# Paleogenomics/IBDGem

Measured on NVIDIA B200. Metric: LD genotype-comparisons/s (site x target x bg x 4), higher is better.
Workload: dtype f64

## Files before the change

### ibdgem_b200/csrc/engine.cu

```cuda
#include <math.h>
#include <stdarg.h>
#include <stdio.h>
#include <string.h>

#include <algorithm>

#include "engine.h"
#include "site_math.cuh"

namespace ibdgem {

static thread_local char g_err[1024] = "";

void set_error(const char *fmt, ...) {
    va_list ap;
    va_start(ap, fmt);
    vsnprintf(g_err, sizeof g_err, fmt, ap);
    va_end(ap);
}

static const char *const kKernelNameList[] = {
    "site_table",     "scan_count",    "scan_offsets",  "scan_rank",    "window_nonld", "counters",
    "expand_sites",   "ld_general",    "ld_finalize",   "ld_compact",   "ld_c0",        "ld_transpose",
    "ld_stage",       "ld_expand_bg",  "ld_expand_tgt", "ld_windows",   "ld_ibd0",
    "ld_mma",         "viterbi",       "viterbi_back",  "viterbi_out",  "fill",
    "v_slots",        "v_wmap",        "v_tw",          "v_sort",       "v_expand_a",  "v_expand_b",   "ld_vmma",
    "window_linear",  "posterior_fwd", "posterior_bwd", "posterior_fwd_log", "posterior_bwd_log",
    "tract_count",    "tract_emit",    "posterior_bwd_moments",
};
static_assert(sizeof(kKernelNameList) / sizeof(kKernelNameList[0]) == K_COUNT, "one name per KernelId, in enum order");
const char *const *const kKernelNames = kKernelNameList;

LaunchScope::LaunchScope(ibdgem_engine *e_, int id_, cudaStream_t s_) : e(e_), id(id_), s(s_ ? s_ : e_->stream) {
    e->k_launches[id]++;
    if (!e->timing) return;
    auto get = [&]() {
        cudaEvent_t ev;
        if (!e->event_pool.empty()) {
            ev = e->event_pool.back();
            e->event_pool.pop_back();
        } else {
            cudaEventCreate(&ev);
        }
        return ev;
    };
    a = get();
    b = get();
    cudaEventRecord(a, s);
}
LaunchScope::~LaunchScope() {
    if (!a) return;
    cudaEventRecord(b, s);
    e->pending.push_back({id, a, b});
}
int settle_timers(ibdgem_engine *e) {
    if (e->t0_set || e->pending.size() > 4096) return resolve_timers(e);
    return 0;
}
int resolve_timers(ibdgem_engine *e) {
    FILE *tl = e->timeline_path && e->t0_set && !e->pending.empty() ? fopen(e->timeline_path, "a") : nullptr;
    for (auto &p : e->pending) {
        float ms = 0;
        cudaEventSynchronize(p.b);
        if (cudaEventElapsedTime(&ms, p.a, p.b) == cudaSuccess) e->k_ms[p.id] += ms;
        if (tl) {
            float t_a = 0, t_b = 0;
            cudaEventElapsedTime(&t_a, e->ev_t0, p.a);
            cudaEventElapsedTime(&t_b, e->ev_t0, p.b);
            fprintf(tl, "%s %.4f %.4f\n", kKernelNames[p.id], t_a, t_b);
        }
        e->event_pool.push_back(p.a);
        e->event_pool.push_back(p.b);
    }
    e->pending.clear();
    if (tl) fclose(tl);
    return 0;
}

int dev_alloc(ibdgem_engine *e, void **p, size_t bytes) {
    *p = nullptr;
    if (bytes == 0) bytes = 16;
    IBD_CUDA(cudaMalloc(p, bytes));
    e->device_bytes += (int64_t)bytes;
    return 0;
}
void dev_free(ibdgem_engine *e, void *p, size_t bytes) {
    if (!p) return;
    cudaFree(p);
    e->device_bytes -= (int64_t)(bytes ? bytes : 16);
}

int pinned_stage(ibdgem_engine *e, size_t bytes, void **out) {
    if (e->h_pin_cap < bytes) {
        if (e->h_pin) cudaFreeHost(e->h_pin);
        e->h_pin = nullptr;
        e->h_pin_cap = 0;
        const size_t want = bytes + bytes / 4 + 4096;
        IBD_CUDA(cudaMallocHost(&e->h_pin, want));
        e->h_pin_cap = want;
    }
    *out = e->h_pin;
    return 0;
}

int scratch(ibdgem_engine *e, int slot, size_t bytes, void **out) {
    if (e->scratch.empty()) e->scratch.assign(SC_SLOTS, nullptr);
    DeviceBuf *&b = e->scratch[slot];
    if (!b) b = new DeviceBuf();
    if (b->cap < bytes) {
        if (b->p) dev_free(e, b->p, b->cap);
        b->p = nullptr;
        b->cap = 0;
        size_t want = bytes + bytes / 8 + 256;
        if (dev_alloc(e, &b->p, want)) return 1;
        b->cap = want;
    }
    *out = b->p;
    return 0;
}

__device__ __forceinline__ int warp_sum_i(int v) {
#pragma unroll
    for (int o = 16; o > 0; o >>= 1) v += __shfl_xor_sync(0xffffffffu, v, o);
    return v;
}
__device__ __forceinline__ double warp_sum_d(double v) {
#pragma unroll
    for (int o = 16; o > 0; o >>= 1) v += __shfl_xor_sync(0xffffffffu, v, o);
    return v;
}
__device__ __forceinline__ double warp_max_d(double v) {
#pragma unroll
    for (int o = 16; o > 0; o >>= 1) v = fmax(v, __shfl_xor_sync(0xffffffffu, v, o));
    return v;
}

__global__ void fill_nan_kernel(double *p, int64_t n) {
    int64_t i = blockIdx.x * (int64_t)blockDim.x + threadIdx.x;
    const double nan = __longlong_as_double(0x7ff8000000000000LL);
    for (; i < n; i += (int64_t)gridDim.x * blockDim.x) p[i] = nan;
}

__global__ void __launch_bounds__(256)
site_table_kernel(int64_t s_begin, int64_t S, int32_t N, int64_t Wh, const uint32_t *__restrict__ bits,
                  const uint8_t *__restrict__ hostkeep, const uint8_t *__restrict__ nref,
                  const uint8_t *__restrict__ nalt, const double *__restrict__ afuser,
                  const double *__restrict__ Ptab, int C, double min_af, double max_af, int max_cov,
                  double *__restrict__ f_out, uint8_t *__restrict__ keep, uint8_t *__restrict__ status,
                  double *__restrict__ lik7, double *__restrict__ lnlik7, const double *__restrict__ lnPtab) {
    __shared__ double stage7[8][32 * 7];
    const int lane = threadIdx.x & 31;
    const int64_t warp0 = (blockIdx.x * (int64_t)blockDim.x + threadIdx.x) >> 5;
    const int64_t nwarps = ((int64_t)gridDim.x * blockDim.x) >> 5;
    const int H = 2 * N;
    const int nfull = H >> 5, rem = H & 31;
    const bool vec4 = ((Wh & 3) == 0);
    const int n4 = vec4 ? (nfull >> 2) : 0;
    for (int64_t s0 = s_begin + warp0 * 32; s0 < S; s0 += nwarps * 32) {
        const int rows = (int)min((int64_t)32, S - s0);
        int mycnt = 0;
        const int j = lane >> 2, q = lane & 3;
#pragma unroll
        for (int it = 0; it < 4; it++) {
            const int r = it * 8 + j;
            int cnt = 0;
            if (r < rows) {
                const uint32_t *row = bits + (s0 + r) * Wh;
                const uint4 *row4 = reinterpret_cast<const uint4 *>(row);
                for (int w = q; w < n4; w += 4) {
                    const uint4 x = __ldg(row4 + w);
                    cnt += __popc(x.x) + __popc(x.y) + __popc(x.z) + __popc(x.w);
                }
                for (int w = (n4 << 2) + q; w < nfull; w += 4) cnt += __popc(__ldg(row + w));
                if (q == 0 && rem) cnt += __popc(__ldg(row + nfull) & ((1u << rem) - 1u));
            }
            cnt += __shfl_xor_sync(0xffffffffu, cnt, 1);
            cnt += __shfl_xor_sync(0xffffffffu, cnt, 2);
            const int got = __shfl_sync(0xffffffffu, cnt, 4 * (lane & 7));
            if ((lane >> 3) == it) mycnt = got;
        }
        const int64_t s = s0 + lane;
        double v[7], lv[7];
        const double nan = __longlong_as_double(0x7ff8000000000000LL);
#pragma unroll
        for (int i = 0; i < 7; i++) v[i] = lv[i] = nan;
        if (lane < rows) {
            double f = __ddiv_rn((double)mycnt, (double)H);
            if (afuser) {
                const double u = afuser[s];
                if (u == u) f = u;
            }
            const int r = nref[s], a = nalt[s];
            const bool k = hostkeep[s] && !(f > max_af || f < min_af) && (r + a <= max_cov);
            if (k) {
                const double *P = Ptab + (size_t)(r * C + a) * 3;
                const double P0 = P[0], P1 = P[1], P2 = P[2];
                v[0] = lik_ibd0(f, P0, P1, P2);
                v[1] = lik_ibd1(0, f, P0, P1, P2);
                v[2] = lik_ibd1(1, f, P0, P1, P2);
                v[3] = lik_ibd1(2, f, P0, P1, P2);
                v[4] = P0; v[5] = P1; v[6] = P2;
            }
            const double *lP = lnPtab + (k ? (size_t)(r * C + a) * 3 : 0);
#pragma unroll
            for (int i = 0; i < 7; i++) lv[i] = k ? (i >= 4 ? lP[i - 4] : log(v[i])) : v[i];
            f_out[s] = f;
            keep[s] = k ? 1 : 0;
            status[s] = k ? ((r + a >= 1) ? 1 : 2) : 0;
        }
        double *stw = stage7[threadIdx.x >> 5];
#pragma unroll
        for (int pass = 0; pass < 2; pass++) {
            __syncwarp();
#pragma unroll
            for (int i = 0; i < 7; i++) stw[lane * 7 + i] = pass ? lv[i] : v[i];
            __syncwarp();
            double *dst = (pass ? lnlik7 : lik7) + s0 * 7;
            for (int i = lane; i < rows * 7; i += 32) dst[i] = stw[i];
        }
    }
}

__global__ void __launch_bounds__(256)
site_status_kernel(int64_t S, const uint8_t *__restrict__ hostkeep, const uint8_t *__restrict__ nref,
                   const uint8_t *__restrict__ nalt, int max_cov, uint8_t *__restrict__ keep, uint8_t *__restrict__ status,
                   int C, unsigned long long *__restrict__ cnt ) {
    extern __shared__ unsigned int shist[];
    for (int i = threadIdx.x; i < C + 3; i += blockDim.x) shist[i] = 0;
    __syncthreads();
    unsigned proc = 0, skip = 0, cov = 0;
    for (int64_t s = blockIdx.x * (int64_t)blockDim.x + threadIdx.x; s < S; s += (int64_t)gridDim.x * blockDim.x) {
        const int r = nref[s], a = nalt[s];
        const bool k = hostkeep[s] && (r + a <= max_cov);
        keep[s] = k ? 1 : 0;
        status[s] = k ? ((r + a >= 1) ? 1 : 2) : 0;
        if (k) {
            proc++;
            cov += (unsigned)(r + a);
            atomicAdd(&shist[3 + min(r + a, C - 1)], 1u);
        } else {
            skip++;
        }
    }
    proc = (unsigned)warp_sum_i((int)proc);
    skip = (unsigned)warp_sum_i((int)skip);
    cov = (unsigned)warp_sum_i((int)cov);
    if ((threadIdx.x & 31) == 0) {
        atomicAdd(&shist[0], proc);
        atomicAdd(&shist[1], skip);
        atomicAdd(&shist[2], cov);
    }
    __syncthreads();
    for (int i = threadIdx.x; i < C + 3; i += blockDim.x)
        if (shist[i]) atomicAdd(&cnt[i], (unsigned long long)shist[i]);
}

constexpr int SCAN_THREADS = 256;
constexpr int SCAN_ITERS = 8;
constexpr int SCAN_CHUNK = SCAN_THREADS * SCAN_ITERS;
constexpr int ROW_SLICE = 32768;

__global__ void __launch_bounds__(SCAN_THREADS)
scan_count_kernel(SiteView v, const int32_t *__restrict__ targets, uint32_t *__restrict__ blockcnt,
                  int nb) {
    const int t = blockIdx.y;
    const int indiv = targets ? targets[t] : 0;
    const int64_t base = (int64_t)blockIdx.x * SCAN_CHUNK;
    int c = 0;
    for (int it = 0; it < SCAN_ITERS; it++) {
        const int64_t s = base + it * SCAN_THREADS + threadIdx.x;
        int r, a, g;
        if (s < v.S && site_eval(v, t, indiv, s, r, a, g) == 1) c++;
    }
    c = warp_sum_i(c);
    __shared__ int ws[SCAN_THREADS / 32];
    if ((threadIdx.x & 31) == 0) ws[threadIdx.x >> 5] = c;
    __syncthreads();
    if (threadIdx.x == 0) {
        int tot = 0;
        for (int i = 0; i < SCAN_THREADS / 32; i++) tot += ws[i];
        blockcnt[(int64_t)t * nb + blockIdx.x] = tot;
    }
}

__global__ void __launch_bounds__(256)
scan_offsets_kernel(uint32_t *__restrict__ blockcnt, int nb, int window, int64_t *__restrict__ ktot,
                    int32_t *__restrict__ nwin) {
    const int t = blockIdx.x;
    uint32_t *row = blockcnt + (int64_t)t * nb;
    __shared__ uint32_t carry;
    __shared__ uint32_t ws[8];
    if (threadIdx.x == 0) carry = 0;
    __syncthreads();
    for (int b0 = 0; b0 < nb; b0 += 256) {
        const int i = b0 + threadIdx.x;
        const uint32_t v = (i < nb) ? row[i] : 0;
        uint32_t x = v;
#pragma unroll
        for (int o = 1; o < 32; o <<= 1) {
            const uint32_t y = __shfl_up_sync(0xffffffffu, x, o);
            if ((threadIdx.x & 31) >= o) x += y;
        }
        if ((threadIdx.x & 31) == 31) ws[threadIdx.x >> 5] = x;
        __syncthreads();
        uint32_t woff = 0;
        for (int w = 0; w < (int)(threadIdx.x >> 5); w++) woff += ws[w];
        const uint32_t excl = carry + woff + x - v;
        if (i < nb) row[i] = excl;
        __syncthreads();
        if (threadIdx.x == 255) carry = excl + v;
        __syncthreads();
    }
    if (threadIdx.x == 0) {
        ktot[t] = carry;
        nwin[t] = (int32_t)((carry + (uint32_t)window - 1) / (uint32_t)window);
    }
}

__global__ void __launch_bounds__(SCAN_THREADS)
scan_rank_kernel(SiteView v, const int32_t *__restrict__ targets, const uint32_t *__restrict__ blockoff,
                 int nb, int window, const int64_t *__restrict__ ktot, int64_t *__restrict__ wfirst,
                 int64_t *__restrict__ wlast, int maxW, uint32_t *__restrict__ rank_out) {
    const int t = blockIdx.y;
    const int indiv = targets ? targets[t] : 0;
    const int64_t base = (int64_t)blockIdx.x * SCAN_CHUNK;
    const int lane = threadIdx.x & 31, wid = threadIdx.x >> 5;
    __shared__ int ws[SCAN_THREADS / 32];
    uint32_t running = blockoff[(int64_t)t * nb + blockIdx.x];
    const int64_t K = ktot[t];
    for (int it = 0; it < SCAN_ITERS; it++) {
        const int64_t s = base + it * SCAN_THREADS + threadIdx.x;
        int r, a, g;
        const bool inf = (s < v.S) && site_eval(v, t, indiv, s, r, a, g) == 1;
        const uint32_t bal = __ballot_sync(0xffffffffu, inf);
        if (lane == 0) ws[wid] = __popc(bal);
        __syncthreads();
        uint32_t off = running;
        int tot = 0;
        for (int w = 0; w < SCAN_THREADS / 32; w++) {
            if (w < wid) off += ws[w];
            tot += ws[w];
        }
        const uint32_t rk = off + __popc(bal & ((1u << lane) - 1u));
        if (rank_out && s < v.S) rank_out[s] = rk;
        if (inf) {
            const uint32_t w = rk / (uint32_t)window, k = rk % (uint32_t)window;
            if ((int)w < maxW) {
                if (k == 0) wfirst[(int64_t)t * maxW + w] = s;
                if (k == (uint32_t)window - 1 || (int64_t)rk == K - 1) wlast[(int64_t)t * maxW + w] = s;
            }
        }
        running += tot;
        __syncthreads();
    }
}

struct WindowMapView {
    const int64_t *wfirst, *wlast;
    const int32_t *nwin;
    int rows;
    int maxW;
};

__global__ void __launch_bounds__(256)
window_nonld_kernel(SiteView v, WindowMapView m, const int32_t *__restrict__ targets, int T,
                    const uint64_t *__restrict__ pos, const double *__restrict__ f,
                    const double *__restrict__ lnlik7, const double *__restrict__ Ptab, int C,
                    int outW, double *__restrict__ wll, int32_t *__restrict__ wn,
                    uint64_t *__restrict__ ws, uint64_t *__restrict__ we, int32_t *__restrict__ nwin_out) {
    const int lane = threadIdx.x & 31;
    const int64_t gw = (blockIdx.x * (int64_t)blockDim.x + threadIdx.x) >> 5;
    const int64_t total = (int64_t)T * outW;
    if (gw >= total) return;
    const int t = (int)(gw / outW), w = (int)(gw % outW);
    const int row = (m.rows == 1) ? 0 : t;
    const int nw = m.nwin[row];
    if (w == 0 && lane == 0) nwin_out[t] = nw;
    if (w >= nw || w >= m.maxW) return;
    const int indiv = targets[t];
    const int64_t s0 = m.wfirst[(int64_t)row * m.maxW + w], s1 = m.wlast[(int64_t)row * m.maxW + w];
    double a0 = 0, a1 = 0, a2 = 0;
    int n = 0;
    for (int64_t s = s0 + lane; s <= s1; s += 32) {
        int r, a, g;
        if (site_eval(v, t, indiv, s, r, a, g) != 1) continue;
        n++;
        if (v.tgt_counts) {
            const double *P = Ptab + (size_t)(r * C + a) * 3;
            const double P0 = P[0], P1 = P[1], P2 = P[2], ff = f[s];
            a0 += log(lik_ibd0(ff, P0, P1, P2));
            a1 += log(lik_ibd1(g, ff, P0, P1, P2));
            a2 += log(P[g]);
        } else {
            const double *L = lnlik7 + s * 7;
            a0 += L[0];
            a1 += L[1 + g];
            a2 += L[4 + g];
        }
    }
    a0 = warp_sum_d(a0);
    a1 = warp_sum_d(a1);
    a2 = warp_sum_d(a2);
    n = warp_sum_i(n);
    if (lane == 0) {
        const int64_t o = (int64_t)t * outW + w;
        wll[o * 3 + 0] = a0;
        wll[o * 3 + 1] = a1;
        wll[o * 3 + 2] = a2;
        wn[o] = n;
        ws[o] = pos[s0];
        we[o] = pos[s1];
    }
}

constexpr int NONLD_TILE = 256;
template <int NONLD_BATCH>
__global__ void __launch_bounds__(128)
window_nonld_shared_kernel(SiteView v, WindowMapView m, const int32_t *__restrict__ targets, int T,
                           const uint64_t *__restrict__ pos, const uint8_t *__restrict__ status,
                           const double *__restrict__ lnlik7, int outW, double *__restrict__ wll,
                           int32_t *__restrict__ wn, uint64_t *__restrict__ ws, uint64_t *__restrict__ we,
                           int32_t *__restrict__ nwin_out) {
    __shared__ double2 sl12[NONLD_TILE][3];
    __shared__ int64_t srow[NONLD_TILE];
    __shared__ int32_t soff[NONLD_TILE];
    __shared__ int segcnt[NONLD_TILE / 32];
    __shared__ double sa0[4];
    constexpr int PASSES = NONLD_TILE / 128;
    const int w = blockIdx.x;
    const int nw = m.nwin[0];
    const int t = blockIdx.y * blockDim.x + threadIdx.x;
    if (w == 0 && t < T) nwin_out[t] = nw;
    if (w >= nw || w >= m.maxW) return;
    const int64_t s0 = m.wfirst[w], s1 = m.wlast[w];
    const int indiv = t < T ? targets[t] : 0;
    const uint32_t *tcol = v.bits + (indiv >> 4);
    const int tsh = (indiv & 15) * 2;
    const int lane = threadIdx.x & 31;
    double a0p = 0, a1 = 0, a2 = 0;
    int n = 0;
    for (int64_t sb = s0; sb <= s1; sb += NONLD_TILE) {
        __syncthreads();
        unsigned bal[PASSES];
#pragma unroll
        for (int q = 0; q < PASSES; q++) {
            const int64_t s = sb + q * 128 + threadIdx.x;
            bal[q] = __ballot_sync(0xffffffffu, s <= s1 && status[s] == 1);
            if (lane == 0) segcnt[(q * 128 + threadIdx.x) >> 5] = __popc(bal[q]);
        }
        __syncthreads();
        int cnt = 0;
#pragma unroll
        for (int q = 0; q < PASSES; q++) {
            const int seg = (q * 128 + (int)threadIdx.x) >> 5;
            int base = 0;
            for (int k = 0; k < seg; k++) base += segcnt[k];
            if ((bal[q] >> lane) & 1u) {
                const int slot = base + __popc(bal[q] & ((1u << lane) - 1u));
                const int64_t site = sb + q * 128 + threadIdx.x;
                srow[slot] = site * v.Wh;
                soff[slot] = (int32_t)(site - s0);
            }
        }
        for (int k = 0; k < NONLD_TILE / 32; k++) cnt += segcnt[k];
        __syncthreads();
        for (int i = threadIdx.x; i < cnt * 7; i += blockDim.x) {
            const int j = i / 7, c = i - j * 7;
            const double x = lnlik7[(s0 + soff[j]) * 7 + c];
            double *dst = reinterpret_cast<double *>(&sl12[j][0]);
            if (c == 0)
                a0p += x;
            else if (c <= 3)
                dst[(c - 1) * 2] = x;
            else
                dst[(c - 4) * 2 + 1] = x;
        }
        __syncthreads();
        if (t < T) {
            for (int j0 = 0; j0 < cnt; j0 += NONLD_BATCH) {
                uint32_t pr[NONLD_BATCH];
#pragma unroll
                for (int q = 0; q < NONLD_BATCH; q++) pr[q] = (j0 + q < cnt) ? __ldg(tcol + srow[j0 + q]) : 0u;
#pragma unroll
                for (int q = 0; q < NONLD_BATCH; q++) {
                    if (j0 + q < cnt) {
                        const int g = __popc((pr[q] >> tsh) & 3u);
                        const double2 l = sl12[j0 + q][g];
                        a1 += l.x;
                        a2 += l.y;
                    }
                }
            }
            n += cnt;
        }
    }
    a0p = warp_sum_d(a0p);
    if (lane == 0) sa0[threadIdx.x >> 5] = a0p;
    __syncthreads();
    if (t < T) {
        const double a0 = (sa0[0] + sa0[1]) + (sa0[2] + sa0[3]);
        const int64_t o = (int64_t)t * outW + w;
        wll[o * 3 + 0] = a0;
        wll[o * 3 + 1] = a1;
        wll[o * 3 + 2] = a2;
        wn[o] = n;
        ws[o] = pos[s0];
        we[o] = pos[s1];
    }
}

__global__ void __launch_bounds__(128)
window_linear_kernel(SiteView v, WindowMapView m, const int32_t *__restrict__ targets, int T, const double *__restrict__ f,
                     const double *__restrict__ lik7, const double *__restrict__ Ptab, int C, int outW, double *__restrict__ wlin) {
    const int64_t i = blockIdx.x * (int64_t)blockDim.x + threadIdx.x;
    if (i >= (int64_t)T * outW) return;
    const int t = (int)(i / outW), w = (int)(i % outW);
    const int row = (m.rows == 1) ? 0 : t;
    if (w >= m.nwin[row] || w >= m.maxW) return;
    const int indiv = targets[t];
    const int64_t s0 = m.wfirst[(int64_t)row * m.maxW + w], s1 = m.wlast[(int64_t)row * m.maxW + w];
    double p0 = 1.0, p1 = 1.0, p2 = 1.0;
    for (int64_t s = s0; s <= s1; s++) {
        int r, a, g;
        if (site_eval(v, t, indiv, s, r, a, g) != 1) continue;
        double l0, l1, l2;
        if (v.tgt_counts) {
            const double *P = Ptab + (size_t)(r * C + a) * 3;
            l0 = lik_ibd0(f[s], P[0], P[1], P[2]);
            l1 = lik_ibd1(g, f[s], P[0], P[1], P[2]);
            l2 = P[g];
        } else {
            const double *L = lik7 + s * 7;
            l0 = L[0];
            l1 = L[1 + g];
            l2 = L[4 + g];
        }
        p0 = __dmul_rn(p0, l0);
        p1 = __dmul_rn(p1, l1);
        p2 = __dmul_rn(p2, l2);
    }
    wlin[i * 3 + 0] = p0;
    wlin[i * 3 + 1] = p1;
    wlin[i * 3 + 2] = p2;
}

constexpr int COUNTERS_CHUNK = 8192;
__global__ void __launch_bounds__(256)
counters_kernel(SiteView v, const int32_t *__restrict__ targets, int C,
                unsigned long long *__restrict__ out ) {
    const int t = blockIdx.y;
    const int indiv = targets ? targets[t] : 0;
    extern __shared__ unsigned long long sh[];
    for (int i = threadIdx.x; i < C + 3; i += blockDim.x) sh[i] = 0;
    __syncthreads();
    unsigned long long proc = 0, skip = 0, cov = 0;
    const int64_t s_begin = (int64_t)blockIdx.x * COUNTERS_CHUNK;
    const int64_t s_end = min(v.S, s_begin + COUNTERS_CHUNK);
    for (int64_t s = s_begin + threadIdx.x; s < s_end; s += blockDim.x) {
        int r = 0, a = 0, g = 0;
        const int st = site_eval(v, t, indiv, s, r, a, g);
        if (st == 0) {
            skip++;
        } else {
            proc++;
            cov += (unsigned)(r + a);
            atomicAdd(&sh[3 + min(r + a, C - 1)], 1ULL);
        }
    }
    atomicAdd(&sh[0], proc);
    atomicAdd(&sh[1], skip);
    atomicAdd(&sh[2], cov);
    __syncthreads();
    for (int i = threadIdx.x; i < C + 3; i += blockDim.x)
        if (sh[i]) atomicAdd(&out[(int64_t)t * (C + 3) + i], sh[i]);
}

__global__ void __launch_bounds__(256)
expand_sites_kernel(SiteView v, const int32_t *__restrict__ targets, int T,
                    const double *__restrict__ f, const double *__restrict__ lik7,
                    const double *__restrict__ Ptab, int C, uint8_t *__restrict__ st_out,
                    double *__restrict__ lik_out) {
    const int64_t i = blockIdx.x * (int64_t)blockDim.x + threadIdx.x;
    if (i >= (int64_t)T * v.S) return;
    const int t = (int)(i / v.S);
    const int64_t s = i % v.S;
    int r = 0, a = 0, g = 0;
    const int st = site_eval(v, t, targets[t], s, r, a, g);
    const double nan = __longlong_as_double(0x7ff8000000000000LL);
    double l0 = nan, l1 = nan, l2 = nan;
    if (st != 0) {
        if (v.tgt_counts) {
            const double *P = Ptab + (size_t)(r * C + a) * 3;
            l0 = lik_ibd0(f[s], P[0], P[1], P[2]);
            l1 = lik_ibd1(g, f[s], P[0], P[1], P[2]);
            l2 = P[g];
        } else {
            const double *L = lik7 + s * 7;
            l0 = L[0];
            l1 = L[1 + g];
            l2 = L[4 + g];
        }
    }
    if (st_out) st_out[i] = (uint8_t)st;
    if (lik_out) {
        lik_out[i * 3 + 0] = l0;
        lik_out[i * 3 + 1] = l1;
        lik_out[i * 3 + 2] = l2;
    }
}

constexpr int LD_THREADS = 256;
constexpr int LD_PER = 2;

struct LdPartial {
    double m0, s0, m1, s1;
};

__global__ void __launch_bounds__(LD_THREADS)
ld_general_kernel(SiteView v, WindowMapView m, const int32_t *__restrict__ targets,
                  const int32_t *__restrict__ bg, int n_bg, int pu_idx,
                  const double *__restrict__ lnPtab, int C, int outW, int nz,
                  LdPartial *__restrict__ part ) {
    const int w = blockIdx.x, t = blockIdx.y, z = blockIdx.z;
    const int row = (m.rows == 1) ? 0 : t;
    if (w >= m.nwin[row] || w >= m.maxW || w >= outW) return;
    const int indiv = targets[t];
    const int64_t s0 = m.wfirst[(int64_t)row * m.maxW + w], s1 = m.wlast[(int64_t)row * m.maxW + w];

    __shared__ double sl[LD_THREADS][3];
    __shared__ int64_t ssite[LD_THREADS];
    __shared__ uint8_t sa[LD_THREADS];
    __shared__ int wcount[LD_THREADS / 32];
    __shared__ double red[LD_THREADS / 32];

    const int lane = threadIdx.x & 31, wid = threadIdx.x >> 5;
    int b[LD_PER];
    bool valid[LD_PER];
    double acc[LD_PER][5];
#pragma unroll
    for (int p = 0; p < LD_PER; p++) {
        const int n = (z * LD_PER + p) * LD_THREADS + threadIdx.x;
        b[p] = (n < n_bg) ? bg[n] : -1;
        valid[p] = (n < n_bg) && b[p] != indiv && b[p] != pu_idx;
        if (!valid[p]) b[p] = 0;
#pragma unroll
        for (int q = 0; q < 5; q++) acc[p][q] = 0.0;
    }

    for (int64_t sb = s0; sb <= s1; sb += LD_THREADS) {
        const int64_t s = sb + threadIdx.x;
        int r = 0, a = 0, g = 0;
        const bool inf = (s <= s1) && site_eval(v, t, indiv, s, r, a, g) == 1;
        const uint32_t bal = __ballot_sync(0xffffffffu, inf);
        if (lane == 0) wcount[wid] = __popc(bal);
        __syncthreads();
        int off = 0, cnt = 0;
        for (int k = 0; k < LD_THREADS / 32; k++) {
            if (k < wid) off += wcount[k];
            cnt += wcount[k];
        }
        if (inf) {
            const int j = off + __popc(bal & ((1u << lane) - 1u));
            const double *L = lnPtab + (size_t)(r * C + a) * 3;
            sl[j][0] = L[0];
            sl[j][1] = L[1];
            sl[j][2] = L[2];
            ssite[j] = s;
            sa[j] = (uint8_t)hap_pair(v.bits + s * v.Wh, indiv);
        }
        __syncthreads();
        for (int j = 0; j < cnt; j++) {
            const double l0 = sl[j][0], l1 = sl[j][1], l2 = sl[j][2];
            const uint32_t ta = sa[j];
            const double u0lo = (ta & 1u) ? l1 : l0, u0hi = (ta & 1u) ? l2 : l1;
            const double u1lo = (ta & 2u) ? l1 : l0, u1hi = (ta & 2u) ? l2 : l1;
            const uint32_t *rowp = v.bits + ssite[j] * v.Wh;
#pragma unroll
            for (int p = 0; p < LD_PER; p++) {
                const uint32_t pr = hap_pair(rowp, b[p]);
                const bool r0 = pr & 1u, r1 = pr & 2u;
                const int gg = (int)r0 + (int)r1;
                acc[p][0] += (gg == 0) ? l0 : (gg == 1 ? l1 : l2);
                acc[p][1] += r0 ? u0hi : u0lo;
                acc[p][2] += r1 ? u0hi : u0lo;
                acc[p][3] += r0 ? u1hi : u1lo;
                acc[p][4] += r1 ? u1hi : u1lo;
            }
        }
        __syncthreads();
    }

    const double NEG = -INFINITY;
    double m0 = NEG, m1 = NEG;
#pragma unroll
    for (int p = 0; p < LD_PER; p++)
        if (valid[p]) {
            m0 = fmax(m0, acc[p][0]);
            m1 = fmax(m1, fmax(fmax(acc[p][1], acc[p][2]), fmax(acc[p][3], acc[p][4])));
        }
    auto block_max = [&](double x) {
        x = warp_max_d(x);
        __syncthreads();
        if (lane == 0) red[wid] = x;
        __syncthreads();
        double y = red[0];
        for (int k = 1; k < LD_THREADS / 32; k++) y = fmax(y, red[k]);
        return y;
    };
    auto block_sum = [&](double x) {
        x = warp_sum_d(x);
        __syncthreads();
        if (lane == 0) red[wid] = x;
        __syncthreads();
        double y = 0;
        for (int k = 0; k < LD_THREADS / 32; k++) y += red[k];
        return y;
    };
    m0 = block_max(m0);
    m1 = block_max(m1);
    double e0 = 0, e1 = 0;
#pragma unroll
    for (int p = 0; p < LD_PER; p++)
        if (valid[p]) {
            e0 += exp(acc[p][0] - m0);
            e1 += exp(acc[p][1] - m1) + exp(acc[p][2] - m1) + exp(acc[p][3] - m1) + exp(acc[p][4] - m1);
        }
    e0 = block_sum(e0);
    e1 = block_sum(e1);
    if (threadIdx.x == 0) {
        LdPartial o;
        o.m0 = m0; o.s0 = e0; o.m1 = m1; o.s1 = e1;
        part[((int64_t)t * outW + w) * nz + z] = o;
    }
}

__global__ void ld_finalize_kernel(const LdPartial *__restrict__ part, int nz, WindowMapView m, int T,
                                   int outW, const int32_t *__restrict__ nrefpanel,
                                   double *__restrict__ wll) {
    const int64_t i = blockIdx.x * (int64_t)blockDim.x + threadIdx.x;
    if (i >= (int64_t)T * outW) return;
    const int t = (int)(i / outW), w = (int)(i % outW);
    const int row = (m.rows == 1) ? 0 : t;
    if (w >= m.nwin[row]) return;
    const double nan = __longlong_as_double(0x7ff8000000000000LL);
    const int nr = nrefpanel[t];
    if (nr <= 0) {
        wll[i * 3 + 0] = nan;
        wll[i * 3 + 1] = nan;
        return;
    }
    double M0 = -INFINITY, M1 = -INFINITY;
    for (int z = 0; z < nz; z++) {
        M0 = fmax(M0, part[i * nz + z].m0);
        M1 = fmax(M1, part[i * nz + z].m1);
    }
    double S0 = 0, S1 = 0;
    for (int z = 0; z < nz; z++) {
        const LdPartial p = part[i * nz + z];
        if (p.s0 > 0) S0 += p.s0 * exp(p.m0 - M0);
        if (p.s1 > 0) S1 += p.s1 * exp(p.m1 - M1);
    }
    wll[i * 3 + 0] = M0 + log(S0) - log((double)nr);
    wll[i * 3 + 1] = M1 + log(S1) - log(4.0 * (double)nr);
}

int wait_panel_upto(ibdgem_engine *e, int64_t s_end) {
    while (e->chunks_waited < (int)e->chunk_end.size() &&
           (e->chunks_waited == 0 || e->chunk_end[(size_t)e->chunks_waited - 1] < s_end)) {
        IBD_CUDA(cudaStreamWaitEvent(e->stream, e->chunk_ev[(size_t)e->chunks_waited], 0));
        e->chunks_waited++;
    }
    if (e->chunk_end.empty() || e->chunk_end.back() < s_end) {
        set_error("[::] ERROR: panel rows up to %lld are needed but only %lld were declared ready "
                  "(ibdgem_engine_panel_rows_ready).", (long long)s_end, (long long)(e->chunk_end.empty() ? 0 : e->chunk_end.back()));
        return 1;
    }
    return 0;
}

int ensure_table(ibdgem_engine *e, int64_t s_end) {
    if (wait_panel_upto(e, s_end)) return 1;
    if (e->table_upto >= s_end) return 0;
    {
        LaunchScope ls(e, K_SITE_TABLE);
        const int64_t n = s_end - e->table_upto;
        site_table_kernel<<<(unsigned)((n + 255) / 256), 256, 0, e->stream>>>(
            e->table_upto, s_end, e->N, e->Wh, e->d_bits, e->d_hostkeep, e->d_nref, e->d_nalt, e->d_afuser, e->d_P, e->C,
            e->prm.min_af, e->prm.max_af, (int)e->prm.max_cov, e->d_f, e->d_keep, e->d_status, e->d_lik7, e->d_lnlik7, e->d_lnP);
    }
    IBD_CUDA(cudaGetLastError());
    e->table_upto = s_end;
    return 0;
}

void window_shard_bounds(const ibdgem_engine *e, int32_t *w_begin, int32_t *w_end, int64_t *s_begin, int64_t *s_end) {
    const int64_t nW = e->nW_shared;
    const int32_t wb = (int32_t)(nW * e->shard_index / e->shard_count), we = (int32_t)(nW * (e->shard_index + 1) / e->shard_count);
    if (w_begin) *w_begin = wb;
    if (w_end) *w_end = we;
    if (s_begin) *s_begin = wb > 0 && wb <= (int32_t)e->h_wlast.size() ? e->h_wlast[(size_t)wb - 1] + 1 : 0;
    if (s_end) *s_end = (e->shard_index + 1 >= e->shard_count || we <= 0 || we > (int32_t)e->h_wlast.size()) ? e->S : e->h_wlast[(size_t)we - 1] + 1;
}

}

using namespace ibdgem;

extern "C" {

const char *ibdgem_last_error(void) { return g_err; }
int ibdgem_abi_version(void) { return IBDGEM_B200_ABI_VERSION; }

static unsigned long host_binom(unsigned int n, unsigned int k) {
    unsigned long v = 1;
    const unsigned int base = n - k;
    for (unsigned int j = 1; j <= k; j++) v = ((unsigned int)(base + j) * v) / j;
    return v;
}

static void host_pdg(double eps, unsigned r, unsigned a, double out[3]) {
    if (r == 0 && a == 0) {
        out[0] = out[1] = out[2] = 1.0;
        return;
    }
    volatile double coef = (double)host_binom(r + a, r);
    volatile double p0 = coef * pow(1 - eps, (double)r);
    p0 = p0 * pow(eps, (double)a);
    volatile double p1 = coef * pow(0.5, (double)r);
    p1 = p1 * pow(0.5, (double)a);
    volatile double p2 = coef * pow(1 - eps, (double)a);
    p2 = p2 * pow(eps, (double)r);
    out[0] = p0 == 0.0 ? DBL_MIN : (double)p0;
    out[1] = p1 == 0.0 ? DBL_MIN : (double)p1;
    out[2] = p2 == 0.0 ? DBL_MIN : (double)p2;
}

int ibdgem_engine_create(const ibdgem_params *params, ibdgem_engine **out) {
    if (!params || !out) {
        set_error("[::] ERROR in ibdgem_engine_create(): NULL argument.");
        return 1;
    }
    *out = nullptr;
    if (params->max_cov < 1 || params->max_cov > IBDGEM_MAX_COV_LIMIT) {
        set_error("[::] ERROR: Invalid maximum estimated coverage (-M) of %u (must be 1..%d).",
                  params->max_cov, IBDGEM_MAX_COV_LIMIT);
        return 1;
    }
    if (params->window_size < 2) {
        set_error("[::] ERROR: Invalid window size (-w) of %d (must be >= 2).", params->window_size);
        return 1;
    }
    int ndev = 0;
    cudaError_t ce = cudaGetDeviceCount(&ndev);
    if (ce != cudaSuccess || ndev <= 0) {
        set_error("[::] ERROR: no usable CUDA device (%s); the engine has no CPU fallback.",
                  ce == cudaSuccess ? "device count is 0" : cudaGetErrorString(ce));
        return 1;
    }
    if (params->device < 0 || params->device >= ndev) {
        set_error("[::] ERROR: CUDA device %d out of range (0..%d).", params->device, ndev - 1);
        return 1;
    }
    IBD_CUDA(cudaSetDevice(params->device));
    ibdgem_engine *e = new ibdgem_engine();
    e->prm = *params;
    e->device = params->device;
    e->C = (int)params->max_cov + 1;
    cudaDeviceProp prop;
    if (cudaGetDeviceProperties(&prop, e->device) == cudaSuccess) e->sm_count = prop.multiProcessorCount;

    const int C = e->C;
    e->h_P.assign((size_t)C * C * 3, 1.0);
    e->h_lnP.assign((size_t)C * C * 3, 0.0);
    for (int r = 0; r < C; r++)
        for (int a = 0; a + r < C; a++) {
            double P[3];
            host_pdg(params->epsilon, (unsigned)r, (unsigned)a, P);
            for (int g = 0; g < 3; g++) {
                e->h_P[((size_t)r * C + a) * 3 + g] = P[g];
                e->h_lnP[((size_t)r * C + a) * 3 + g] = (double)logl((long double)P[g]);
            }
        }
    {
        const long double eps = params->epsilon;
        bool ok = eps > 0 && eps < 1;
        long double kap = 0, al = 0, be = 0;
        if (ok) {
            kap = logl(4 * eps * (1 - eps));
            al = logl(0.5L / (1 - eps));
            be = logl(0.5L / eps);
            for (int r = 0; r < C && ok; r++)
                for (int a = 0; a + r < C && ok; a++) {
                    const double *L = &e->h_lnP[((size_t)r * C + a) * 3];
                    const long double c = (long double)L[2] - 2 * (long double)L[1] + L[0];
                    const long double d = (long double)L[1] - L[0];
                    const long double tol = 1e-12L * (1 + fabsl((long double)L[0]) + fabsl((long double)L[2]));
                    if (fabsl(c - (r + a) * kap) > tol || fabsl(d - (r * al + a * be)) > tol) ok = false;
                }
        }
        e->depth_linear = ok;
        e->kappa = (double)kap;
        e->alpha = (double)al;
        e->beta = (double)be;
    }
    if (dev_alloc(e, (void **)&e->d_P, e->h_P.size() * 8) || dev_alloc(e, (void **)&e->d_lnP, e->h_lnP.size() * 8)) {
        delete e;
        return 1;
    }
    IBD_CUDA(cudaMemcpy(e->d_P, e->h_P.data(), e->h_P.size() * 8, cudaMemcpyHostToDevice));
    IBD_CUDA(cudaMemcpy(e->d_lnP, e->h_lnP.data(), e->h_lnP.size() * 8, cudaMemcpyHostToDevice));
    *out = e;
    return 0;
}

static void free_sites(ibdgem_engine *e) {
    dev_free(e, e->d_pos, (size_t)e->S * 8);
    dev_free(e, e->d_nref, (size_t)e->S);
    dev_free(e, e->d_nalt, (size_t)e->S);
    dev_free(e, e->d_hostkeep, (size_t)e->S);
    if (e->d_afuser) dev_free(e, e->d_afuser, (size_t)e->S * 8);
    e->d_pos = nullptr;
    e->d_nref = e->d_nalt = e->d_hostkeep = nullptr;
    e->d_afuser = nullptr;
    e->have_sites = false;
}
static void free_panel(ibdgem_engine *e, int64_t S) {
    if (e->d_bits && e->owns_bits) dev_free(e, e->d_bits, (size_t)S * e->Wh * 4);
    e->d_bits = nullptr;
    e->owns_bits = true;
    e->have_panel = false;
}
static void free_prepared(ibdgem_engine *e, int64_t S) {
    if (e->d_f) {
        dev_free(e, e->d_f, (size_t)S * 8);
        dev_free(e, e->d_keep, (size_t)S);
        dev_free(e, e->d_status, (size_t)S);
        dev_free(e, e->d_lik7, (size_t)S * 56);
        dev_free(e, e->d_lnlik7, (size_t)S * 56);
        dev_free(e, e->d_rank, (size_t)S * 4);
    }
    if (e->d_wfirst) {
        const size_t cap = (size_t)(S / std::max(e->prm.window_size, 1) + 2) * 8;
        dev_free(e, e->d_wfirst, cap);
        dev_free(e, e->d_wlast, cap);
        dev_free(e, e->d_nwin_shared, 4);
        dev_free(e, e->d_ktot_shared, 8);
    }
    e->d_f = e->d_lik7 = e->d_lnlik7 = nullptr;
    e->d_keep = e->d_status = nullptr;
    e->d_rank = nullptr;
    e->d_wfirst = e->d_wlast = nullptr;
    e->d_nwin_shared = nullptr;
    e->d_ktot_shared = nullptr;
    e->prepared = false;
    ld_tensor_release(e);
    ld_vtensor_release(e);
}

int ibdgem_engine_destroy(ibdgem_engine *e) {
    if (!e) return 0;
    cudaSetDevice(e->device);
    cudaStreamSynchronize(e->stream);
    resolve_timers(e);
    const int64_t S = e->S;
    free_prepared(e, S);
    free_panel(e, S);
    if (e->have_sites) free_sites(e);
    dev_free(e, e->d_P, e->h_P.size() * 8);
    dev_free(e, e->d_lnP, e->h_lnP.size() * 8);
    dev_free(e, e->d_shared_cnt, (size_t)(e->C + 3) * 8);
    for (auto *b : e->scratch)
        if (b) {
            if (b->p) cudaFree(b->p);
            delete b;
        }
    for (auto ev : e->event_pool) cudaEventDestroy(ev);
    for (auto ev : e->chunk_ev) cudaEventDestroy(ev);
    if (e->ev_order) cudaEventDestroy(e->ev_order);
    if (e->ev_book) cudaEventDestroy(e->ev_book);
    if (e->copy_stream) cudaStreamDestroy(e->copy_stream);
    for (auto ev : e->range_ev) cudaEventDestroy(ev);
    if (e->d2h_stream) cudaStreamDestroy(e->d2h_stream);
    if (e->h_pin) cudaFreeHost(e->h_pin);
    delete e;
    return 0;
}

int ibdgem_engine_set_stream(ibdgem_engine *e, void *cuda_stream) {
    if (!e) return 1;
    e->stream = (cudaStream_t)cuda_stream;
    return 0;
}

int ibdgem_engine_upload_sites(ibdgem_engine *e, int64_t n_sites, const uint64_t *pos,
                               const uint8_t *n_ref, const uint8_t *n_alt, const uint8_t *host_keep,
                               const double *af_user) {
    if (!e || n_sites <= 0 || !pos || !n_ref || !n_alt || !host_keep) {
        set_error("[::] ERROR in ibdgem_engine_upload_sites(): bad arguments.");
        return 1;
    }
    IBD_CUDA(cudaSetDevice(e->device));
    if (!e->timeline_path) e->timeline_path = getenv("IBDGEM_TIMELINE");
    if (e->timeline_path && e->timing) {
        if (!e->ev_t0) {
            IBD_CUDA(cudaEventCreate(&e->ev_t0));
            IBD_CUDA(cudaEventCreate(&e->ev_wll));
            IBD_CUDA(cudaEventCreate(&e->ev_bookdone));
        }
        IBD_CUDA(cudaEventRecord(e->ev_t0, e->stream));
        e->t0_set = true;
    }
    if (e->have_panel && e->S != n_sites) {
        set_error("[::] ERROR: site count %lld does not match the uploaded panel (%lld rows).",
                  (long long)n_sites, (long long)e->S);
        return 1;
    }
    if (e->have_sites && (e->S != n_sites || (af_user != nullptr) != (e->d_afuser != nullptr))) {
        const int64_t S_old = e->S;
        free_prepared(e, S_old);
        free_sites(e);
    }
    if (!e->have_sites) {
        if (!e->have_panel) e->S = n_sites;
        if (dev_alloc(e, (void **)&e->d_pos, (size_t)n_sites * 8) || dev_alloc(e, (void **)&e->d_nref, (size_t)n_sites) ||
            dev_alloc(e, (void **)&e->d_nalt, (size_t)n_sites) || dev_alloc(e, (void **)&e->d_hostkeep, (size_t)n_sites))
            return 1;
        if (af_user && dev_alloc(e, (void **)&e->d_afuser, (size_t)n_sites * 8)) return 1;
    }
    IBD_CUDA(cudaMemcpyAsync(e->d_pos, pos, (size_t)n_sites * 8, cudaMemcpyHostToDevice, e->stream));
    IBD_CUDA(cudaMemcpyAsync(e->d_nref, n_ref, (size_t)n_sites, cudaMemcpyHostToDevice, e->stream));
    IBD_CUDA(cudaMemcpyAsync(e->d_nalt, n_alt, (size_t)n_sites, cudaMemcpyHostToDevice, e->stream));
    IBD_CUDA(cudaMemcpyAsync(e->d_hostkeep, host_keep, (size_t)n_sites, cudaMemcpyHostToDevice, e->stream));
    if (af_user)
        IBD_CUDA(cudaMemcpyAsync(e->d_afuser, af_user, (size_t)n_sites * 8, cudaMemcpyHostToDevice, e->stream));
    e->have_sites = true;
    e->prepared = false;
    return 0;
}

int ibdgem_engine_upload_panel(ibdgem_engine *e, int64_t n_sites, int32_t n_indiv,
                               const uint32_t *bits, int64_t words_per_site) {
    if (!e || n_sites <= 0 || n_indiv <= 0 || !bits || words_per_site * 32 < 2 * (int64_t)n_indiv) {
        set_error("[::] ERROR in ibdgem_engine_upload_panel(): bad arguments.");
        return 1;
    }
    IBD_CUDA(cudaSetDevice(e->device));
    if (e->have_sites && e->S != n_sites) {
        set_error("[::] ERROR: panel has %lld rows but %lld sites were uploaded.", (long long)n_sites,
                  (long long)e->S);
        return 1;
    }
    if (e->have_panel && (e->S != n_sites || e->Wh != words_per_site)) {
        free_prepared(e, e->S);
        free_panel(e, e->S);
    }
    if (e->have_panel && !e->owns_bits) free_panel(e, e->S);
    if (!e->have_panel) {
        e->S = n_sites;
        e->Wh = words_per_site;
        if (dev_alloc(e, (void **)&e->d_bits, (size_t)n_sites * words_per_site * 4)) return 1;
    }
    e->N = n_indiv;
    if (!e->copy_stream) {
        IBD_CUDA(cudaStreamCreateWithFlags(&e->copy_stream, cudaStreamNonBlocking));
        IBD_CUDA(cudaEventCreateWithFlags(&e->ev_order, cudaEventDisableTiming));
    }
    static const int want_chunks = [] {
        const char *sc = getenv("IBDGEM_PANEL_CHUNKS");
        return sc ? std::max(1, atoi(sc)) : PANEL_CHUNKS;
    }();
    static const double taper = [] {
        const char *st = getenv("IBDGEM_PANEL_TAPER");
        const double t = st ? atof(st) : PANEL_TAPER;
        return (t > 0.1 && t <= 1.0) ? t : 1.0;
    }();
    const size_t panel_bytes = (size_t)n_sites * (size_t)words_per_site * 4;
    const int nchunk = (int)std::max<size_t>(1, std::min<size_t>((size_t)want_chunks, panel_bytes / PANEL_CHUNK_MIN_BYTES));
    while ((int)e->chunk_ev.size() < nchunk) {
        cudaEvent_t ev;
        IBD_CUDA(cudaEventCreateWithFlags(&ev, e->t0_set ? cudaEventDefault : cudaEventDisableTiming));
        e->chunk_ev.push_back(ev);
    }
    IBD_CUDA(cudaEventRecord(e->ev_order, e->stream));
    IBD_CUDA(cudaStreamWaitEvent(e->copy_stream, e->ev_order, 0));
    e->chunk_end.assign((size_t)nchunk, 0);
    double wsum = 0, wk = 1;
    for (int k = 0; k < nchunk; k++, wk *= taper) wsum += wk;
    int64_t s0 = 0;
    double acc = 0;
    wk = 1;
    for (int k = 0; k < nchunk; k++, wk *= taper) {
        acc += wk / wsum;
        const int64_t s1 = k + 1 == nchunk ? n_sites : std::min<int64_t>(n_sites, std::max<int64_t>(s0 + 1, (int64_t)(acc * (double)n_sites)));
        IBD_CUDA(cudaMemcpyAsync(e->d_bits + (size_t)s0 * words_per_site, bits + (size_t)s0 * words_per_site,
                                 (size_t)(s1 - s0) * words_per_site * 4, cudaMemcpyHostToDevice, e->copy_stream));
        IBD_CUDA(cudaEventRecord(e->chunk_ev[(size_t)k], e->copy_stream));
        e->chunk_end[(size_t)k] = s1;
        s0 = s1;
    }
    e->chunks_waited = 0;
    e->have_panel = true;
    e->prepared = false;
    e->table_from = e->table_upto = 0;
    ld_tensor_invalidate(e);
    ld_vtensor_invalidate(e);
    return 0;
}

int ibdgem_engine_set_panel_device(ibdgem_engine *e, int64_t n_sites, int32_t n_indiv, const uint32_t *d_bits,
                                   int64_t words_per_site) {
    if (!e || n_sites <= 0 || n_indiv <= 0 || !d_bits || words_per_site * 32 < 2 * (int64_t)n_indiv) {
        set_error("[::] ERROR in ibdgem_engine_set_panel_device(): bad arguments.");
        return 1;
    }
    IBD_CUDA(cudaSetDevice(e->device));
    cudaPointerAttributes attr;
    if (cudaPointerGetAttributes(&attr, d_bits) != cudaSuccess || attr.type != cudaMemoryTypeDevice || attr.device != e->device) {
        cudaGetLastError();
        set_error("[::] ERROR in ibdgem_engine_set_panel_device(): d_bits is not device memory of GPU %d.", e->device);
        return 1;
    }
    if (e->have_sites && e->S != n_sites) {
        set_error("[::] ERROR: panel has %lld rows but %lld sites were uploaded.", (long long)n_sites, (long long)e->S);
        return 1;
    }
    IBD_CUDA(cudaStreamSynchronize(e->stream));
    if (e->have_panel && (e->S != n_sites || e->Wh != words_per_site)) free_prepared(e, e->S);
    if (e->have_panel) free_panel(e, e->S);
    e->S = n_sites;
    e->Wh = words_per_site;
    e->N = n_indiv;
    e->d_bits = const_cast<uint32_t *>(d_bits);
    e->owns_bits = false;
    e->chunk_end.clear();
    e->chunks_waited = 0;
    e->have_panel = true;
    e->prepared = false;
    e->table_from = e->table_upto = 0;
    ld_tensor_invalidate(e);
    ld_vtensor_invalidate(e);
    return 0;
}

int ibdgem_engine_clone_panel(ibdgem_engine *e, ibdgem_engine *src) {
    if (!e || !src || e == src || !src->have_panel) {
        set_error("[::] ERROR in ibdgem_engine_clone_panel(): the source engine has no panel.");
        return 1;
    }
    if (e->have_sites && e->S != src->S) {
        set_error("[::] ERROR: panel has %lld rows but %lld sites were uploaded.", (long long)src->S, (long long)e->S);
        return 1;
    }
    IBD_CUDA(cudaSetDevice(e->device));
    if (e->have_panel && (e->S != src->S || e->Wh != src->Wh || !e->owns_bits)) {
        free_prepared(e, e->S);
        free_panel(e, e->S);
    }
    if (!e->have_panel) {
        e->S = src->S;
        e->Wh = src->Wh;
        if (dev_alloc(e, (void **)&e->d_bits, (size_t)e->S * e->Wh * 4)) return 1;
    }
    e->N = src->N;
    if (!e->copy_stream) {
        IBD_CUDA(cudaStreamCreateWithFlags(&e->copy_stream, cudaStreamNonBlocking));
        IBD_CUDA(cudaEventCreateWithFlags(&e->ev_order, cudaEventDisableTiming));
    }
    if (e->device != src->device) {
        int can = 0;
        cudaDeviceCanAccessPeer(&can, e->device, src->device);
        if (can && cudaDeviceEnablePeerAccess(src->device, 0) == cudaErrorPeerAccessAlreadyEnabled) cudaGetLastError();
    }
    IBD_CUDA(cudaEventRecord(e->ev_order, e->stream));
    IBD_CUDA(cudaStreamWaitEvent(e->copy_stream, e->ev_order, 0));
    const size_t nchunk = std::max<size_t>(1, src->chunk_end.size());
    while (e->chunk_ev.size() < nchunk) {
        cudaEvent_t ev;
        IBD_CUDA(cudaEventCreateWithFlags(&ev, e->t0_set ? cudaEventDefault : cudaEventDisableTiming));
        e->chunk_ev.push_back(ev);
    }
    e->chunk_end.assign(nchunk, 0);
    int64_t s0 = 0;
    for (size_t k = 0; k < nchunk; k++) {
        const int64_t s1 = src->chunk_end.empty() ? src->S : src->chunk_end[k];
        if (!src->chunk_end.empty()) IBD_CUDA(cudaStreamWaitEvent(e->copy_stream, src->chunk_ev[k], 0));
        IBD_CUDA(cudaMemcpyPeerAsync(e->d_bits + (size_t)s0 * e->Wh, e->device, src->d_bits + (size_t)s0 * e->Wh, src->device,
                                     (size_t)(s1 - s0) * e->Wh * 4, e->copy_stream));
        IBD_CUDA(cudaEventRecord(e->chunk_ev[k], e->copy_stream));
        e->chunk_end[k] = s1;
        s0 = s1;
    }
    e->chunks_waited = 0;
    e->have_panel = true;
    e->owns_bits = true;
    e->prepared = false;
    e->table_from = e->table_upto = 0;
    ld_tensor_invalidate(e);
    ld_vtensor_invalidate(e);
    return 0;
}

int ibdgem_engine_panel_rows_ready(ibdgem_engine *e, int64_t row_end, void *stream) {
    if (!e || !e->have_panel || e->owns_bits) {
        set_error("[::] ERROR in ibdgem_engine_panel_rows_ready(): no caller-owned device panel is set.");
        return 1;
    }
    if (row_end <= 0 || row_end > e->S || (!e->chunk_end.empty() && row_end < e->chunk_end.back())) {
        set_error("[::] ERROR in ibdgem_engine_panel_rows_ready(): row_end %lld out of order or range.", (long long)row_end);
        return 1;
    }
    IBD_CUDA(cudaSetDevice(e->device));
    const size_t k = e->chunk_end.size();
    while (e->chunk_ev.size() <= k) {
        cudaEvent_t ev;
        IBD_CUDA(cudaEventCreateWithFlags(&ev, e->t0_set ? cudaEventDefault : cudaEventDisableTiming));
        e->chunk_ev.push_back(ev);
    }
    IBD_CUDA(cudaEventRecord(e->chunk_ev[k], stream ? static_cast<cudaStream_t>(stream) : e->stream));
    e->chunk_end.push_back(row_end);
    return 0;
}

int ibdgem_engine_sync_uploads(ibdgem_engine *e) {
    if (!e) return 1;
    IBD_CUDA(cudaSetDevice(e->device));
    if (e->copy_stream) IBD_CUDA(cudaStreamSynchronize(e->copy_stream));
    IBD_CUDA(cudaStreamSynchronize(e->stream));
    return 0;
}

static SiteView make_view(ibdgem_engine *e, const uint8_t *d_tgt_counts, int vflag) {
    SiteView v;
    v.keep = e->d_keep;
    v.nref = e->d_nref;
    v.nalt = e->d_nalt;
    v.bits = e->d_bits;
    v.Wh = e->Wh;
    v.S = e->S;
    v.tgt_counts = d_tgt_counts;
    v.vflag = vflag;
    return v;
}

extern "C++" {
namespace ibdgem {
int build_window_map(ibdgem_engine *e, const SiteView &v, const int32_t *d_targets, int rows,
                     int maxW, int64_t *d_wfirst, int64_t *d_wlast, int32_t *d_nwin,
                     int64_t *d_ktot, uint32_t *d_rank) {
    const int nb = (int)((e->S + SCAN_CHUNK - 1) / SCAN_CHUNK);
    uint32_t *d_cnt;
    if (scratch(e, SC_BLOCKCNT, (size_t)rows * nb * 4, (void **)&d_cnt)) return 1;
    for (int r0 = 0; r0 < rows; r0 += ROW_SLICE) {
        const int rc = std::min(ROW_SLICE, rows - r0);
        SiteView vv = v;
        if (vv.tgt_counts) vv.tgt_counts += (size_t)r0 * e->S * 2;
        const int32_t *tg = d_targets ? d_targets + r0 : nullptr;
        uint32_t *cnt = d_cnt + (size_t)r0 * nb;
        {
            LaunchScope ls(e, K_SCAN_COUNT);
            scan_count_kernel<<<dim3(nb, rc), SCAN_THREADS, 0, e->stream>>>(vv, tg, cnt, nb);
        }
        {
            LaunchScope ls(e, K_SCAN_OFFSETS);
            scan_offsets_kernel<<<rc, 256, 0, e->stream>>>(cnt, nb, e->prm.window_size, d_ktot + r0, d_nwin + r0);
        }
        {
            LaunchScope ls(e, K_SCAN_RANK);
            scan_rank_kernel<<<dim3(nb, rc), SCAN_THREADS, 0, e->stream>>>(
                vv, tg, cnt, nb, e->prm.window_size, d_ktot + r0, d_wfirst + (size_t)r0 * maxW, d_wlast + (size_t)r0 * maxW, maxW,
                d_rank);
        }
    }
    IBD_CUDA(cudaGetLastError());
    return 0;
}
}
}

int ibdgem_engine_prepare(ibdgem_engine *e) {
    if (!e) return 1;
    if (e->prepared) return 0;
    if (!e->have_sites || !e->have_panel) {
        set_error("[::] ERROR in ibdgem_engine_prepare(): sites and panel must both be uploaded.");
        return 1;
    }
    IBD_CUDA(cudaSetDevice(e->device));
    const int64_t S = e->S;
    const int maxW = (int)(S / e->prm.window_size + 2);
    if (!e->d_f) {
        if (dev_alloc(e, (void **)&e->d_f, (size_t)S * 8) || dev_alloc(e, (void **)&e->d_keep, (size_t)S) ||
            dev_alloc(e, (void **)&e->d_status, (size_t)S) || dev_alloc(e, (void **)&e->d_lik7, (size_t)S * 56) ||
            dev_alloc(e, (void **)&e->d_lnlik7, (size_t)S * 56) || dev_alloc(e, (void **)&e->d_rank, (size_t)S * 4) ||
            dev_alloc(e, (void **)&e->d_wfirst, (size_t)maxW * 8) || dev_alloc(e, (void **)&e->d_wlast, (size_t)maxW * 8) ||
            dev_alloc(e, (void **)&e->d_nwin_shared, 4) || dev_alloc(e, (void **)&e->d_ktot_shared, 8))
            return 1;
    }
    e->table_from = e->table_upto = 0;
    e->lazy_table = !e->d_afuser && e->prm.min_af <= 0.0 && e->prm.max_af >= 1.0;
    e->shared_cnt_valid = false;
    if (e->lazy_table) {
        if (!e->d_shared_cnt && dev_alloc(e, (void **)&e->d_shared_cnt, (size_t)(e->C + 3) * 8)) return 1;
        IBD_CUDA(cudaMemsetAsync(e->d_shared_cnt, 0, (size_t)(e->C + 3) * 8, e->stream));
        LaunchScope ls(e, K_SITE_TABLE);
        const unsigned nblk = (unsigned)std::min<int64_t>((S + 255) / 256, (int64_t)e->sm_count * 8);
        site_status_kernel<<<nblk, 256, (size_t)(e->C + 3) * 4, e->stream>>>(S, e->d_hostkeep, e->d_nref, e->d_nalt, (int)e->prm.max_cov,
                                                                           e->d_keep, e->d_status, e->C, e->d_shared_cnt);
        e->shared_cnt_valid = true;
    } else if (ensure_table(e, S)) {
        return 1;
    }
    IBD_CUDA(cudaGetLastError());
    int32_t *d_nwin = e->d_nwin_shared;
    int64_t *d_ktot = e->d_ktot_shared;
    SiteView v = make_view(e, nullptr, 0);
    v.bits = nullptr;
    if (build_window_map(e, v, nullptr, 1, maxW, e->d_wfirst, e->d_wlast, d_nwin, d_ktot, e->d_rank)) return 1;
    int64_t *h_map;
    if (pinned_stage(e, (size_t)(maxW + 2) * 8, (void **)&h_map)) return 1;
    IBD_CUDA(cudaMemcpyAsync(h_map, d_nwin, 4, cudaMemcpyDeviceToHost, e->stream));
    IBD_CUDA(cudaMemcpyAsync(h_map + 1, d_ktot, 8, cudaMemcpyDeviceToHost, e->stream));
    IBD_CUDA(cudaMemcpyAsync(h_map + 2, e->d_wlast, (size_t)maxW * 8, cudaMemcpyDeviceToHost, e->stream));
    IBD_CUDA(cudaStreamSynchronize(e->stream));
    const int32_t nwin = *reinterpret_cast<const int32_t *>(h_map);
    const int64_t ktot = h_map[1];
    e->nW_shared = nwin;
    e->K_shared = ktot;
    e->h_wlast.assign(h_map + 2, h_map + 2 + std::max(nwin, 0));
    e->table_from = 0;
    if (e->shard_count > 1 && e->lazy_table) {
        int64_t sb = 0;
        window_shard_bounds(e, nullptr, nullptr, &sb, nullptr);
        e->table_from = e->table_upto = sb;
    }
    e->prepared = true;
    ld_tensor_invalidate(e);
    ld_vtensor_invalidate(e);
    settle_timers(e);
    return 0;
}

int ibdgem_engine_invalidate(ibdgem_engine *e) {
    if (!e) return 1;
    e->prepared = false;
    e->table_from = e->table_upto = 0;
    ld_tensor_invalidate(e);
    ld_vtensor_invalidate(e);
    return 0;
}

int ibdgem_engine_get_site_table(ibdgem_engine *e, double *f, uint8_t *status, double *lik7) {
    if (!e) return 1;
    if (ibdgem_engine_prepare(e)) return 1;
    if (e->table_from > 0) {
        e->table_from = 0;
        e->table_from = e->table_upto = 0;
    }
    if (ensure_table(e, e->S)) return 1;
    IBD_CUDA(cudaSetDevice(e->device));
    if (f) IBD_CUDA(cudaMemcpyAsync(f, e->d_f, (size_t)e->S * 8, cudaMemcpyDeviceToHost, e->stream));
    if (status) IBD_CUDA(cudaMemcpyAsync(status, e->d_status, (size_t)e->S, cudaMemcpyDeviceToHost, e->stream));
    if (lik7) IBD_CUDA(cudaMemcpyAsync(lik7, e->d_lik7, (size_t)e->S * 56, cudaMemcpyDeviceToHost, e->stream));
    IBD_CUDA(cudaStreamSynchronize(e->stream));
    return 0;
}

static int score_common(ibdgem_engine *e, int32_t T, const int32_t *targets, int32_t n_bg,
                        const int32_t *bg, int32_t pu_idx, const uint8_t *tgt_counts,
                        ibdgem_scores *out, bool ld) {
    if (!e || T <= 0 || !targets || !out || (ld && (n_bg < 0 || (n_bg > 0 && !bg)))) {
        set_error("[::] ERROR in ibdgem_engine_score_%s(): bad arguments.", ld ? "ld" : "nonld");
        return 1;
    }
    if (ibdgem_engine_prepare(e)) return 1;
    IBD_CUDA(cudaSetDevice(e->device));
    for (int t = 0; t < T; t++)
        if (targets[t] < 0 || targets[t] >= e->N) {
            set_error("[::] ERROR: target ordinal %d out of range (panel has %d individuals).", targets[t], e->N);
            return 1;
        }
    for (int n = 0; ld && n < n_bg; n++)
        if (bg[n] < 0 || bg[n] >= e->N) {
            set_error("[::] ERROR: background ordinal %d out of range (panel has %d individuals).", bg[n], e->N);
            return 1;
        }
    const int64_t S = e->S;
    const int C = e->C;
    const int vflag = e->prm.variable_sites_only ? 1 : 0;
    const bool shared = !vflag && !tgt_counts;
    const int mapW = shared ? std::max(e->nW_shared, 1) : (int)(S / e->prm.window_size + 2);
    const bool want_windows = out->n_windows || out->w_start || out->w_end || out->w_nsites || out->w_loglik ||
                              out->w_loglik_device || out->w_lik_linear;
    const int outW = want_windows ? out->max_windows : mapW;
    if (want_windows && outW <= 0) {
        set_error("[::] ERROR: ibdgem_scores.max_windows must be positive.");
        return 1;
    }
    if (shared && want_windows && e->nW_shared > outW) {
        set_error("[::] ERROR: %d windows do not fit max_windows = %d.", e->nW_shared, outW);
        return 1;
    }

    int32_t *d_targets;
    if (scratch(e, SC_TARGETS, (size_t)T * 4, (void **)&d_targets)) return 1;
    IBD_CUDA(cudaMemcpyAsync(d_targets, targets, (size_t)T * 4, cudaMemcpyHostToDevice, e->stream));
    uint8_t *d_tc = nullptr;
    if (tgt_counts) {
        if (scratch(e, SC_TGT_COUNTS, (size_t)T * S * 2, (void **)&d_tc)) return 1;
        IBD_CUDA(cudaMemcpyAsync(d_tc, tgt_counts, (size_t)T * S * 2, cudaMemcpyHostToDevice, e->stream));
    }
    SiteView v = make_view(e, d_tc, vflag);

    bool vtensor = false;
    WindowMapView m;
    int32_t *d_nwin;
    int64_t *d_ktot;
    if (shared) {
        d_nwin = e->d_nwin_shared;
        m.wfirst = e->d_wfirst;
        m.wlast = e->d_wlast;
        m.nwin = d_nwin;
        m.rows = 1;
        m.maxW = (int)(S / e->prm.window_size + 2);
    } else if (ld && !e->force_general && ld_vtensor_eligible(e, T, n_bg)) {
        vtensor = true;
        d_nwin = nullptr;
        m.wfirst = m.wlast = nullptr;
        m.nwin = nullptr;
        m.rows = T;
        m.maxW = mapW;
    } else {
        int64_t *d_wf, *d_wl;
        if (scratch(e, SC_WFIRST, (size_t)T * mapW * 8, (void **)&d_wf) ||
            scratch(e, SC_WLAST, (size_t)T * mapW * 8, (void **)&d_wl) ||
            scratch(e, SC_NWIN, (size_t)std::max(T, 1) * 4, (void **)&d_nwin) ||
            scratch(e, SC_KTOT, (size_t)std::max(T, 1) * 8, (void **)&d_ktot))
            return 1;
        if (ensure_table(e, S)) return 1;
        if (build_window_map(e, v, d_targets, T, mapW, d_wf, d_wl, d_nwin, d_ktot, nullptr)) return 1;
        m.wfirst = d_wf;
        m.wlast = d_wl;
        m.nwin = d_nwin;
        m.rows = T;
        m.maxW = mapW;
    }

    double *d_wll;
    int32_t *d_wn, *d_nwout;
    uint64_t *d_ws, *d_we;
    const size_t nWT = (size_t)T * outW;
    if (scratch(e, SC_WLL, nWT * 24, (void **)&d_wll) || scratch(e, SC_WN, nWT * 4 + (size_t)T * 4, (void **)&d_wn) ||
        scratch(e, SC_WS, nWT * 8, (void **)&d_ws) || scratch(e, SC_WE, nWT * 8, (void **)&d_we))
        return 1;
    d_nwout = d_wn + nWT;
    {
        LaunchScope ls(e, K_FILL);
        fill_nan_kernel<<<(unsigned)std::min<int64_t>((int64_t)(nWT * 3 + 255) / 256, 4096), 256, 0, e->stream>>>(d_wll, (int64_t)nWT * 3);
    }
    IBD_CUDA(cudaMemsetAsync(d_wn, 0, nWT * 4 + (size_t)T * 4, e->stream));
    IBD_CUDA(cudaMemsetAsync(d_ws, 0, nWT * 8, e->stream));
    IBD_CUDA(cudaMemsetAsync(d_we, 0, nWT * 8, e->stream));
    const bool tensor = ld && !e->force_general && shared && ld_tensor_eligible(e, T, n_bg, tgt_counts);
    e->book_ready = false;
    if ((tensor || vtensor) && !e->copy_stream) {
        IBD_CUDA(cudaStreamCreateWithFlags(&e->copy_stream, cudaStreamNonBlocking));
        IBD_CUDA(cudaEventCreateWithFlags(&e->ev_order, cudaEventDisableTiming));
    }
    if ((tensor || vtensor) && !e->ev_book) IBD_CUDA(cudaEventCreateWithFlags(&e->ev_book, cudaEventDisableTiming));
    if (!tensor) {
        if (e->shard_count > 1) {
            set_error("[::] ERROR: a window shard (ibdgem_engine_set_window_shard) needs the shared-window tensor --LD path; "
                      "shard the target list instead for non-LD, -v and -D runs.");
            return 1;
        }
        if (ensure_table(e, S)) return 1;
    }
    e->wll_streamed = false;
    e->wll_dev_streamed = false;
    e->h_wll_out = out->w_loglik;
    e->d_wll_out_device = static_cast<double *>(out->w_loglik_device);
    if (vtensor) {
        const int rc = ld_vtensor_score(e, T, targets, d_targets, n_bg, bg, pu_idx, d_tc, outW, d_wll, d_wn, d_ws, d_we, d_nwout);
        if (rc == 1) return 1;
        if (rc == 2) {
            vtensor = false;
            int64_t *d_wf, *d_wl;
            if (scratch(e, SC_WFIRST, (size_t)T * mapW * 8, (void **)&d_wf) ||
                scratch(e, SC_WLAST, (size_t)T * mapW * 8, (void **)&d_wl) ||
                scratch(e, SC_NWIN, (size_t)std::max(T, 1) * 4, (void **)&d_nwin) ||
                scratch(e, SC_KTOT, (size_t)std::max(T, 1) * 8, (void **)&d_ktot))
                return 1;
            if (build_window_map(e, v, d_targets, T, mapW, d_wf, d_wl, d_nwin, d_ktot, nullptr)) return 1;
            m.wfirst = d_wf;
            m.wlast = d_wl;
            m.nwin = d_nwin;
        } else {
            e->last_ld_path = 2;
        }
    }
    if (vtensor) {
    } else if (tensor) {
        if (ld_tensor_score(e, T, targets, d_targets, n_bg, bg, pu_idx, outW, d_wll, d_wn, d_ws, d_we, d_nwout)) return 1;
        e->last_ld_path = 1;
    } else {
        {
            LaunchScope ls(e, K_WINDOW_NONLD);
            if (shared) {
                static const int batch = [] { const char *sb = getenv("IBDGEM_NONLD_BATCH"); return sb ? atoi(sb) : 8; }();
                const dim3 grid((unsigned)std::max(e->nW_shared, 1), (unsigned)((T + 127) / 128));
                auto kern = batch >= 32 ? window_nonld_shared_kernel<32> : (batch >= 16 ? window_nonld_shared_kernel<16> : window_nonld_shared_kernel<8>);
                kern<<<grid, 128, 0, e->stream>>>(v, m, d_targets, T, e->d_pos, e->d_status, e->d_lnlik7, outW, d_wll, d_wn, d_ws, d_we, d_nwout);
            } else {
                const int64_t warps = (int64_t)nWT;
                window_nonld_kernel<<<(unsigned)((warps * 32 + 255) / 256), 256, 0, e->stream>>>(
                    v, m, d_targets, T, e->d_pos, e->d_f, e->d_lnlik7, e->d_P, C, outW, d_wll, d_wn, d_ws, d_we, d_nwout);
            }
        }
        IBD_CUDA(cudaGetLastError());
    }

    if (ld && !tensor && !vtensor) {
        std::vector<int32_t> h_nref(T);
        for (int t = 0; t < T; t++) {
            int c = 0;
            for (int n = 0; n < n_bg; n++)
                if (bg[n] != targets[t] && bg[n] != pu_idx) c++;
            h_nref[t] = c;
        }
        {
            int32_t *d_bg, *d_nrp;
            LdPartial *d_part;
            const int nz = std::max(1, (n_bg + LD_THREADS * LD_PER - 1) / (LD_THREADS * LD_PER));
            if (scratch(e, SC_BG, (size_t)std::max(n_bg, 1) * 4, (void **)&d_bg) ||
                scratch(e, SC_NREFPANEL, (size_t)T * 4, (void **)&d_nrp) ||
                scratch(e, SC_LD_PART, nWT * nz * sizeof(LdPartial), (void **)&d_part))
                return 1;
            if (n_bg > 0) IBD_CUDA(cudaMemcpyAsync(d_bg, bg, (size_t)n_bg * 4, cudaMemcpyHostToDevice, e->stream));
            IBD_CUDA(cudaMemcpyAsync(d_nrp, h_nref.data(), (size_t)T * 4, cudaMemcpyHostToDevice, e->stream));
            for (int t0 = 0; t0 < T; t0 += 32768) {
                const int tc = std::min(32768, T - t0);
                SiteView vv = v;
                if (vv.tgt_counts) vv.tgt_counts += (size_t)t0 * S * 2;
                WindowMapView mm = m;
                if (mm.rows != 1) {
                    mm.wfirst += (size_t)t0 * m.maxW;
                    mm.wlast += (size_t)t0 * m.maxW;
                    mm.nwin += t0;
                }
                LaunchScope ls(e, K_LD_GENERAL);
                ld_general_kernel<<<dim3(outW, tc, nz), LD_THREADS, 0, e->stream>>>(
                    vv, mm, d_targets + t0, d_bg, n_bg, pu_idx, e->d_lnP, C, outW, nz, d_part + (size_t)t0 * outW * nz);
            }
            {
                LaunchScope ls(e, K_LD_FINALIZE);
                ld_finalize_kernel<<<(unsigned)((nWT + 255) / 256), 256, 0, e->stream>>>(d_part, nz, m, T, outW, d_nrp, d_wll);
            }
            IBD_CUDA(cudaGetLastError());
            e->last_ld_path = 0;
        }
    }

    if (e->shard_count == 1 && ensure_table(e, S)) return 1;
    double *d_wlin = nullptr;
    if (out->w_lik_linear && e->shard_count == 1) {
        if (scratch(e, SC_WLIN, nWT * 24, (void **)&d_wlin)) return 1;
        {
            LaunchScope ls(e, K_FILL);
            fill_nan_kernel<<<(unsigned)std::min<int64_t>((int64_t)(nWT * 3 + 255) / 256, 4096), 256, 0, e->stream>>>(d_wlin, (int64_t)nWT * 3);
        }
        if (!vtensor) {
            LaunchScope ls(e, K_WINDOW_LINEAR);
            window_linear_kernel<<<(unsigned)((nWT + 127) / 128), 128, 0, e->stream>>>(v, m, d_targets, T, e->d_f, e->d_lik7, e->d_P, C, outW, d_wlin);
        }
        IBD_CUDA(cudaGetLastError());
    }
    const bool want_counters = out->processed || out->skipped || out->final_total_cov || out->final_dist;
    unsigned long long *d_cnt = nullptr;
    const int crow = C + 3;
    const int crows = shared ? 1 : T;
    if (want_counters && shared && e->shared_cnt_valid) {
        d_cnt = e->d_shared_cnt;
    } else if (want_counters) {
        if (scratch(e, SC_COUNTERS, (size_t)crows * crow * 8, (void **)&d_cnt)) return 1;
        IBD_CUDA(cudaMemsetAsync(d_cnt, 0, (size_t)crows * crow * 8, e->stream));
        LaunchScope ls(e, K_COUNTERS);
        for (int r0 = 0; r0 < crows; r0 += ROW_SLICE) {
            const int rc = std::min(ROW_SLICE, crows - r0);
            SiteView vv = v;
            if (vv.tgt_counts) vv.tgt_counts += (size_t)r0 * S * 2;
            counters_kernel<<<dim3((unsigned)((S + COUNTERS_CHUNK - 1) / COUNTERS_CHUNK), rc), 256, (size_t)crow * 8, e->stream>>>(
                vv, shared ? nullptr : d_targets + r0, C, d_cnt + (size_t)r0 * crow);
        }
    }
    uint8_t *d_st = nullptr;
    double *d_sl = nullptr;
    if (out->site_status || out->site_lik) {
        if (out->site_status && scratch(e, SC_SITE_STATUS, (size_t)T * S, (void **)&d_st)) return 1;
        if (out->site_lik && scratch(e, SC_SITE_LIK, (size_t)T * S * 24, (void **)&d_sl)) return 1;
        LaunchScope ls(e, K_EXPAND_SITES);
        const int64_t n = (int64_t)T * S;
        expand_sites_kernel<<<(unsigned)((n + 255) / 256), 256, 0, e->stream>>>(v, d_targets, T, e->d_f, e->d_lik7, e->d_P, C, d_st, d_sl);
    }
    IBD_CUDA(cudaGetLastError());

    if (out->w_loglik_device && !e->wll_dev_streamed)
        IBD_CUDA(cudaMemcpyAsync(out->w_loglik_device, d_wll, nWT * 24, cudaMemcpyDefault, e->stream));
    if (out->w_loglik && !e->wll_streamed)
        IBD_CUDA(cudaMemcpyAsync(out->w_loglik, d_wll, nWT * 24, cudaMemcpyDeviceToHost, e->stream));
    if (d_wlin) IBD_CUDA(cudaMemcpyAsync(out->w_lik_linear, d_wlin, nWT * 24, cudaMemcpyDeviceToHost, e->stream));
    if (e->t0_set) IBD_CUDA(cudaEventRecord(e->ev_wll, e->wll_streamed ? e->d2h_stream : e->stream));
    cudaStream_t bs = e->stream;
    if (e->book_ready) {
        IBD_CUDA(cudaStreamWaitEvent(e->copy_stream, e->ev_book, 0));
        bs = e->copy_stream;
    }
    if (out->w_nsites) IBD_CUDA(cudaMemcpyAsync(out->w_nsites, d_wn, nWT * 4, cudaMemcpyDeviceToHost, bs));
    if (out->w_start) IBD_CUDA(cudaMemcpyAsync(out->w_start, d_ws, nWT * 8, cudaMemcpyDeviceToHost, bs));
    if (out->w_end) IBD_CUDA(cudaMemcpyAsync(out->w_end, d_we, nWT * 8, cudaMemcpyDeviceToHost, bs));
    if (e->t0_set) IBD_CUDA(cudaEventRecord(e->ev_bookdone, bs));
    std::vector<int32_t> h_nw(T);
    IBD_CUDA(cudaMemcpyAsync(h_nw.data(), d_nwout, (size_t)T * 4, cudaMemcpyDeviceToHost, e->stream));
    std::vector<unsigned long long> h_cnt;
    if (want_counters) {
        h_cnt.resize((size_t)crows * crow);
        IBD_CUDA(cudaMemcpyAsync(h_cnt.data(), d_cnt, h_cnt.size() * 8, cudaMemcpyDeviceToHost, e->stream));
    }
    if (out->site_status) IBD_CUDA(cudaMemcpyAsync(out->site_status, d_st, (size_t)T * S, cudaMemcpyDeviceToHost, e->stream));
    if (out->site_lik) IBD_CUDA(cudaMemcpyAsync(out->site_lik, d_sl, (size_t)T * S * 24, cudaMemcpyDeviceToHost, e->stream));
    IBD_CUDA(cudaStreamSynchronize(e->stream));
    if (e->book_ready) IBD_CUDA(cudaStreamSynchronize(e->copy_stream));
    if (e->wll_streamed || e->wll_dev_streamed) IBD_CUDA(cudaStreamSynchronize(e->d2h_stream));
    e->book_ready = false;
    settle_timers(e);
    if (e->t0_set) {
        if (FILE *tl = fopen(e->timeline_path, "a")) {
            float ms = 0;
            for (size_t k = 0; k < e->chunk_end.size(); k++)
                if (cudaEventElapsedTime(&ms, e->ev_t0, e->chunk_ev[k]) == cudaSuccess) fprintf(tl, "chunk%d_arrived %.4f %.4f\n", (int)k, ms, ms);
            if (cudaEventElapsedTime(&ms, e->ev_t0, e->ev_wll) == cudaSuccess) fprintf(tl, "wll_on_host %.4f %.4f\n", ms, ms);
            if (cudaEventElapsedTime(&ms, e->ev_t0, e->ev_bookdone) == cudaSuccess) fprintf(tl, "bookkeeping_on_host %.4f %.4f\n", ms, ms);
            fprintf(tl, "---\n");
            fclose(tl);
            cudaGetLastError();
        }
    }

    for (int t = 0; t < T; t++) {
        if (want_windows && h_nw[t] > outW) {
            set_error("[::] ERROR: target %d has %d windows but max_windows = %d.", t, h_nw[t], outW);
            return 1;
        }
        if (out->n_windows) out->n_windows[t] = h_nw[t];
        if (want_counters) {
            const unsigned long long *c = &h_cnt[(size_t)(shared ? 0 : t) * crow];
            if (out->processed) out->processed[t] = c[0];
            if (out->skipped) out->skipped[t] = c[1];
            if (out->final_total_cov) out->final_total_cov[t] = c[2];
            if (out->final_dist)
                for (int k = 0; k < C; k++) out->final_dist[(size_t)t * C + k] = c[3 + k];
        }
    }
    return 0;
}

int ibdgem_engine_score_nonld(ibdgem_engine *e, int32_t n_targets, const int32_t *targets,
                              const uint8_t *tgt_counts, ibdgem_scores *out) {
    return score_common(e, n_targets, targets, 0, nullptr, -1, tgt_counts, out, false);
}

int ibdgem_engine_score_ld(ibdgem_engine *e, int32_t n_targets, const int32_t *targets, int32_t n_bg,
                           const int32_t *bg, int32_t pu_idx, const uint8_t *tgt_counts,
                           ibdgem_scores *out) {
    return score_common(e, n_targets, targets, n_bg, bg, pu_idx, tgt_counts, out, true);
}

int ibdgem_engine_set_window_shard(ibdgem_engine *e, int32_t index, int32_t count) {
    if (!e || count < 1 || index < 0 || index >= count) {
        set_error("[::] ERROR in ibdgem_engine_set_window_shard(): need 0 <= index < count.");
        return 1;
    }
    if (e->shard_index != index || e->shard_count != count) {
        e->shard_index = index;
        e->shard_count = count;
        e->prepared = false;
        e->table_from = e->table_upto = 0;
        ld_tensor_invalidate(e);
        ld_vtensor_invalidate(e);
    }
    return 0;
}

int ibdgem_engine_set_shard_compact_output(ibdgem_engine *e, int32_t on) {
    if (!e) return 1;
    e->shard_compact = on != 0;
    return 0;
}

int ibdgem_engine_window_shard(ibdgem_engine *e, int32_t *w_begin, int32_t *w_end, int64_t *site_begin, int64_t *site_end) {
    if (!e) return 1;
    if (ibdgem_engine_prepare(e)) return 1;
    window_shard_bounds(e, w_begin, w_end, site_begin, site_end);
    return 0;
}

int ibdgem_peer_alloc(int32_t device, int64_t bytes, void **dptr, unsigned char *handle64) {
    if (!dptr || !handle64 || bytes <= 0) {
        set_error("[::] ERROR in ibdgem_peer_alloc(): bad arguments.");
        return 1;
    }
    static_assert(sizeof(cudaIpcMemHandle_t) == 64, "the ABI passes IPC handles as 64 opaque bytes");
    IBD_CUDA(cudaSetDevice(device));
    IBD_CUDA(cudaMalloc(dptr, (size_t)bytes));
    cudaIpcMemHandle_t h;
    const cudaError_t ce = cudaIpcGetMemHandle(&h, *dptr);
    if (ce != cudaSuccess) {
        cudaFree(*dptr);
        *dptr = nullptr;
        set_error("[::] ERROR in ibdgem_peer_alloc(): cudaIpcGetMemHandle: %s", cudaGetErrorString(ce));
        return 1;
    }
    memcpy(handle64, &h, 64);
    return 0;
}
int ibdgem_peer_open(int32_t device, const unsigned char *handle64, void **dptr) {
    if (!dptr || !handle64) {
        set_error("[::] ERROR in ibdgem_peer_open(): bad arguments.");
        return 1;
    }
    IBD_CUDA(cudaSetDevice(device));
    cudaIpcMemHandle_t h;
    memcpy(&h, handle64, 64);
    IBD_CUDA(cudaIpcOpenMemHandle(dptr, h, cudaIpcMemLazyEnablePeerAccess));
    return 0;
}
int ibdgem_peer_close(int32_t device, void *dptr, int32_t owner) {
    if (!dptr) return 0;
    IBD_CUDA(cudaSetDevice(device));
    if (owner)
        IBD_CUDA(cudaFree(dptr));
    else
        IBD_CUDA(cudaIpcCloseMemHandle(dptr));
    return 0;
}

int ibdgem_engine_last_ld_path(ibdgem_engine *e) { return e ? e->last_ld_path : -1; }
int ibdgem_engine_force_general_ld(ibdgem_engine *e, int on) {
    if (!e) return 1;
    e->force_general = on;
    return 0;
}

int ibdgem_engine_enable_timing(ibdgem_engine *e, int on) {
    if (!e) return 1;
    e->timing = on != 0;
    return 0;
}
int ibdgem_engine_reset_stats(ibdgem_engine *e) {
    if (!e) return 1;
    resolve_timers(e);
    for (int k = 0; k < K_COUNT; k++) {
        e->k_ms[k] = 0;
        e->k_launches[k] = 0;
    }
    return 0;
}
int ibdgem_engine_num_kernels(ibdgem_engine *e) { return e ? (int)K_COUNT : 0; }
int ibdgem_engine_kernel_stats(ibdgem_engine *e, int32_t k, char *name_out, int32_t name_cap,
                               double *ms_total, int64_t *launches) {
    if (!e || k < 0 || k >= K_COUNT) return 1;
    resolve_timers(e);
    if (name_out && name_cap > 0) {
        strncpy(name_out, kKernelNames[k], (size_t)name_cap - 1);
        name_out[name_cap - 1] = 0;
    }
    if (ms_total) *ms_total = e->k_ms[k];
    if (launches) *launches = e->k_launches[k];
    return 0;
}
int64_t ibdgem_engine_device_bytes(ibdgem_engine *e) { return e ? e->device_bytes : 0; }

}
```

### ibdgem_b200/csrc/engine.h

```cpp
#pragma once

#include <cuda_runtime.h>
#include <stdint.h>

#include <functional>
#include <string>
#include <vector>

#include "../../include/ibdgem_b200.h"

namespace ibdgem {

void set_error(const char *fmt, ...);

#define IBD_CUDA(expr)                                                                          \
    do {                                                                                        \
        cudaError_t _e = (expr);                                                                \
        if (_e != cudaSuccess) {                                                                \
            ::ibdgem::set_error("[::] ERROR in %s (%s:%d): %s", #expr, __FILE__, __LINE__,      \
                                cudaGetErrorString(_e));                                        \
            return 1;                                                                           \
        }                                                                                       \
    } while (0)

enum KernelId {
    K_SITE_TABLE = 0,
    K_SCAN_COUNT,
    K_SCAN_OFFSETS,
    K_SCAN_RANK,
    K_WINDOW_NONLD,
    K_COUNTERS,
    K_EXPAND_SITES,
    K_LD_GENERAL,
    K_LD_FINALIZE,
    K_LD_COMPACT,
    K_LD_C0,
    K_LD_TRANSPOSE,
    K_LD_STAGE,
    K_LD_EXPAND_BG,
    K_LD_EXPAND_TGT,
    K_LD_WINDOWS,
    K_LD_IBD0,
    K_LD_MMA,
    K_VITERBI,
    K_VITERBI_BACK,
    K_VITERBI_OUT,
    K_FILL,
    K_V_SLOTS,
    K_V_WMAP,
    K_V_TW,
    K_V_SORT,
    K_V_EXPAND_A,
    K_V_EXPAND_B,
    K_LD_VMMA,
    K_WINDOW_LINEAR,
    K_POSTERIOR_FWD,
    K_POSTERIOR_BWD,
    K_POSTERIOR_FWD_LOG,
    K_POSTERIOR_BWD_LOG,
    K_TRACT_COUNT,
    K_TRACT_EMIT,
    K_POSTERIOR_BWD_MOMENTS,
    K_COUNT
};

extern const char *const *const kKernelNames;

struct LdCache;
struct VCache;
struct SiteView;

struct PendingTimer {
    int id;
    cudaEvent_t a, b;
};

struct DeviceBuf {
    void *p = nullptr;
    size_t cap = 0;
};

}

struct ibdgem_engine {
    ibdgem_params prm{};
    int device = 0;
    int sm_count = 148;
    cudaStream_t stream = nullptr;
    int C = 21;

    std::vector<double> h_P;
    std::vector<double> h_lnP;
    double *d_P = nullptr, *d_lnP = nullptr;
    bool depth_linear = false;
    double kappa = 0, alpha = 0, beta = 0;

    int64_t S = 0;
    int32_t N = 0;
    int64_t Wh = 0;
    uint64_t *d_pos = nullptr;
    uint8_t *d_nref = nullptr, *d_nalt = nullptr, *d_hostkeep = nullptr;
    double *d_afuser = nullptr;
    uint32_t *d_bits = nullptr;
    bool owns_bits = true;
    bool have_sites = false, have_panel = false, prepared = false;

    cudaStream_t copy_stream = nullptr;
    cudaEvent_t ev_order = nullptr;
    cudaEvent_t ev_book = nullptr;
    bool book_ready = false;
    cudaStream_t d2h_stream = nullptr;
    std::vector<cudaEvent_t> range_ev;
    double *h_wll_out = nullptr;
    bool wll_streamed = false;
    std::vector<cudaEvent_t> chunk_ev;
    std::vector<int64_t> chunk_end;
    int chunks_waited = 0;
    int64_t table_from = 0, table_upto = 0;
    int32_t shard_index = 0, shard_count = 1;
    bool shard_compact = false;
    double *d_wll_out_device = nullptr;
    bool wll_dev_streamed = false;
    bool lazy_table = false;
    std::vector<int64_t> h_wlast;

    double *d_f = nullptr;
    uint8_t *d_keep = nullptr;
    uint8_t *d_status = nullptr;
    double *d_lik7 = nullptr, *d_lnlik7 = nullptr;
    uint32_t *d_rank = nullptr;
    int64_t *d_wfirst = nullptr, *d_wlast = nullptr;
    int32_t *d_nwin_shared = nullptr;
    int64_t *d_ktot_shared = nullptr;
    int32_t nW_shared = 0;
    int64_t K_shared = 0;
    unsigned long long *d_shared_cnt = nullptr;
    bool shared_cnt_valid = false;

    ibdgem::LdCache *ld = nullptr;
    ibdgem::VCache *vc = nullptr;

    void *h_pin = nullptr;
    size_t h_pin_cap = 0;
    std::vector<ibdgem::DeviceBuf *> scratch;
    int64_t device_bytes = 0;

    bool timing = false;
    double k_ms[ibdgem::K_COUNT] = {0};
    int64_t k_launches[ibdgem::K_COUNT] = {0};
    std::vector<ibdgem::PendingTimer> pending;
    std::vector<cudaEvent_t> event_pool;
    const char *timeline_path = nullptr;
    cudaEvent_t ev_t0 = nullptr, ev_wll = nullptr, ev_bookdone = nullptr;
    bool t0_set = false;

    int64_t hg_flagged = 0;
    int64_t hg_tracts = -1;
    int last_ld_path = -1;
    int force_general = 0;
};

namespace ibdgem {

struct LaunchScope {
    ibdgem_engine *e;
    int id;
    cudaEvent_t a = nullptr, b = nullptr;
    cudaStream_t s = nullptr;
    LaunchScope(ibdgem_engine *e_, int id_, cudaStream_t s_ = nullptr);
    ~LaunchScope();
};
int resolve_timers(ibdgem_engine *e);
int settle_timers(ibdgem_engine *e);
int pinned_stage(ibdgem_engine *e, size_t bytes, void **out);

enum ScratchSlot {
    SC_TARGETS = 0, SC_BG, SC_TGT_COUNTS, SC_BLOCKCNT, SC_WFIRST, SC_WLAST, SC_NWIN, SC_KTOT, SC_WLL,
    SC_WN, SC_WS, SC_WE, SC_COUNTERS, SC_SITE_STATUS, SC_SITE_LIK, SC_LD_PART, SC_NREFPANEL,
    SC_HG_LIK, SC_HG_OFF, SC_HG_STATE, SC_HG_SCORE, SC_HG_COUNTS, SC_HG_FROMT, SC_HG_LAST,
    SC_MMA_TGT, SC_MMA_BG, SC_MMA_ROWLSE, SC_MMA_BGIDX, SC_MMA_MISC, SC_MMA_UNIT,
    SC_WLIN, SC_WLL_PACK, SC_V_KS, SC_V_KE, SC_V_TWBASE, SC_V_TWI, SC_V_TWD, SC_V_ORDER, SC_V_HIST, SC_V_TILES, SC_V_MISC, SC_HG_CKPT,
    SC_HG_TRACTS,
    SC_HG_TOFF, SC_SLOTS
};
int scratch(ibdgem_engine *e, int slot, size_t bytes, void **out);
int table_layout(const char *fn, int n_tables, const int64_t *bin_offsets, int64_t table_stride, std::vector<int64_t> *sl, int64_t *maxbins,
                 int64_t *total);
int viterbi_on_device(ibdgem_engine *e, int n_tables, int64_t maxbins, int64_t total_bins, const int64_t *d_start, const int64_t *d_len,
                      const double *d_lik, int is_log, double p01, double p02, double p12, uint8_t *d_state, double *d_score,
                      long long *d_counts, uint8_t *d_flag);
void viterbi_redo_flagged(const std::vector<int> &flagged, const int64_t *bin_offsets, const double *lik, int is_log, double p01,
                          double p02, double p12,
                          const std::function<void(size_t, int, const uint8_t *, const double *, const int64_t *)> &sink);
bool bad_penalties(const char *fn, double p01, double p02, double p12);
int posterior_on_device(ibdgem_engine *e, int n_tables, int64_t maxbins, const int64_t *d_start, const int64_t *d_len, const double *d_lik,
                        int is_log, double p01, double p02, double p12, double *d_post, double *d_expected, double *d_cov = nullptr);

int wait_panel_upto(ibdgem_engine *e, int64_t s_end);
int ensure_table(ibdgem_engine *e, int64_t s_end);

int dev_alloc(ibdgem_engine *e, void **p, size_t bytes);
void dev_free(ibdgem_engine *e, void *p, size_t bytes);

bool ld_tensor_eligible(ibdgem_engine *e, int32_t n_targets, int32_t n_bg, const uint8_t *tgt_counts);
int ld_tensor_prepare(ibdgem_engine *e);
int ld_tensor_score(ibdgem_engine *e, int32_t T, const int32_t *h_targets, const int32_t *d_targets, int32_t n_bg,
                    const int32_t *h_bg, int32_t pu_idx, int32_t outW, double *d_wll , int32_t *d_wn,
                    uint64_t *d_ws, uint64_t *d_we, int32_t *d_nwout);
void ld_tensor_release(ibdgem_engine *e);
constexpr int PANEL_CHUNKS = 16;
constexpr double PANEL_TAPER = 1.0;
constexpr size_t PANEL_CHUNK_MIN_BYTES = (size_t)16 << 20;
void ld_tensor_invalidate(ibdgem_engine *e);
int ld_transpose_launch(ibdgem_engine *e, int w_begin, int w_end, const int32_t *infsite, int Wpad, int WP32, int H, uint32_t *tbits);
bool ld_vtensor_eligible(ibdgem_engine *e, int32_t n_targets, int32_t n_bg);
int ld_vtensor_score(ibdgem_engine *e, int32_t T, const int32_t *h_targets, const int32_t *d_targets, int32_t n_bg, const int32_t *h_bg,
                     int32_t pu_idx, const uint8_t *d_tgt_counts, int32_t outW, double *d_wll, int32_t *d_wn, uint64_t *d_ws,
                     uint64_t *d_we, int32_t *d_nwout);
void ld_vtensor_release(ibdgem_engine *e);
void ld_vtensor_invalidate(ibdgem_engine *e);
int build_window_map(ibdgem_engine *e, const SiteView &v, const int32_t *d_targets, int rows, int maxW, int64_t *d_wfirst,
                     int64_t *d_wlast, int32_t *d_nwin, int64_t *d_ktot, uint32_t *d_rank);
void window_shard_bounds(const ibdgem_engine *e, int32_t *w_begin, int32_t *w_end, int64_t *s_begin, int64_t *s_end);

}
```

### ibdgem_b200/csrc/ld_mma.cu

```cuda
#include <cuda.h>
#include <math.h>
#include <stdio.h>
#include <stdlib.h>
#include <string.h>

#include <algorithm>
#include <vector>

#include "engine.h"
#include "tc_common.cuh"

namespace ibdgem {

struct LdCache {
    bool valid = false;
    int tw_upto = 0;
    int32_t nW = 0;
    int64_t K = 0;
    int W = 0, Wpad = 0, WP32 = 0, KB = 0;
    int H = 0, N = 0;
    int32_t *d_infsite = nullptr;
    uint8_t *d_nk = nullptr;
    uint8_t *d_nr = nullptr;
    double *d_l0 = nullptr;
    double *d_C0 = nullptr;
    uint32_t *d_tbits = nullptr;
    size_t b_infsite = 0, b_nk = 0, b_nr = 0, b_l0 = 0, b_C0 = 0, b_tbits = 0;
};

constexpr int KEY_PAD = -(1 << 30);
constexpr int KEY_INIT = -(1 << 29);
constexpr double SCREEN_NATS = 32.0;
constexpr int MAX_GRID_Y = 65535;
constexpr size_t LD_OPERAND_BUDGET = (size_t)12 << 30;


__global__ void __launch_bounds__(256)
ld_compact_kernel(int64_t S, const uint8_t *__restrict__ status, const uint32_t *__restrict__ rank,
                  const uint8_t *__restrict__ nref, const uint8_t *__restrict__ nalt,
                  const double *__restrict__ lnP, int C, int W, int Wpad, int32_t *__restrict__ infsite,
                  uint8_t *__restrict__ nk, uint8_t *__restrict__ nr, double *__restrict__ l0) {
    const int64_t s = blockIdx.x * (int64_t)blockDim.x + threadIdx.x;
    if (s >= S || status[s] != 1) return;
    const uint32_t r = rank[s];
    const int64_t slot = (int64_t)(r / (uint32_t)W) * Wpad + (r % (uint32_t)W);
    const int a = nref[s], b = nalt[s];
    infsite[slot] = (int32_t)s;
    nk[slot] = (uint8_t)(a + b);
    nr[slot] = (uint8_t)a;
    l0[slot] = lnP[(size_t)(a * C + b) * 3];
}

__global__ void __launch_bounds__(256) ld_c0_kernel(const double *__restrict__ l0, int Wpad, double *__restrict__ C0) {
    __shared__ double sh[256];
    const double *p = l0 + (size_t)blockIdx.x * Wpad;
    double a = 0;
    for (int k = threadIdx.x; k < Wpad; k += 256) a += p[k];
    sh[threadIdx.x] = a;
    __syncthreads();
    for (int o = 128; o > 0; o >>= 1) {
        if ((int)threadIdx.x < o) sh[threadIdx.x] += sh[threadIdx.x + o];
        __syncthreads();
    }
    if (threadIdx.x == 0) C0[blockIdx.x] = sh[0];
}

__device__ __forceinline__ uint32_t transpose32(uint32_t x, int lane) {
#pragma unroll
    for (int k = 0; k < 5; k++) {
        const int j = 16 >> k;
        const uint32_t m = k == 0 ? 0x0000FFFFu : k == 1 ? 0x00FF00FFu : k == 2 ? 0x0F0F0F0Fu : k == 3 ? 0x33333333u : 0x55555555u;
        const bool hi = (lane & j) != 0;
        const uint32_t keep = hi ? ~m : m;
        const uint32_t y = __shfl_xor_sync(0xffffffffu, x, j);
        const uint32_t t = __funnelshift_l(y, y, hi ? 32 - j : j);
        x = (x & keep) | (t & ~keep);
    }
    return x;
}

__global__ void __launch_bounds__(1024)
ld_transpose_kernel(int w_off, const uint32_t *__restrict__ bits, int64_t Wh, int H, const int32_t *__restrict__ infsite,
                    int Wpad, int WP32, uint32_t *__restrict__ tbits) {
    __shared__ uint32_t tile[256 * 33];
    const int w = w_off + blockIdx.y, j0 = blockIdx.x * 8;
    const int lane = threadIdx.x & 31, g = threadIdx.x >> 5;
    if (g < WP32) {
        const int32_t s = infsite[(size_t)w * Wpad + g * 32 + lane];
        const uint32_t *row = bits + (size_t)(s < 0 ? 0 : s) * Wh;
        uint32_t word[8];
        if ((Wh & 3) == 0) {
            uint4 lo = make_uint4(0u, 0u, 0u, 0u), hi = lo;
            if (s >= 0 && j0 < Wh) lo = __ldg(reinterpret_cast<const uint4 *>(row + j0));
            if (s >= 0 && j0 + 4 < Wh) hi = __ldg(reinterpret_cast<const uint4 *>(row + j0 + 4));
            word[0] = lo.x; word[1] = lo.y; word[2] = lo.z; word[3] = lo.w;
            word[4] = hi.x; word[5] = hi.y; word[6] = hi.z; word[7] = hi.w;
        } else {
#pragma unroll
            for (int jj = 0; jj < 8; jj++) word[jj] = (s >= 0 && j0 + jj < Wh) ? __ldg(row + j0 + jj) : 0u;
        }
#pragma unroll
        for (int jj = 0; jj < 8; jj++) tile[(jj * 32 + lane) * 33 + g] = transpose32(word[jj], lane);
    }
    __syncthreads();
    if (lane < WP32)
        for (int hl = g; hl < 256; hl += 32) {
            const int hap = j0 * 32 + hl;
            if (hap < H) tbits[((size_t)w * H + hap) * WP32 + lane] = tile[hl * 33 + lane];
        }
}


__device__ __forceinline__ uint32_t spread4(uint32_t nib) { return (nib * 0x00204081u) & 0x01010101u; }
__device__ __forceinline__ void spread32(uint32_t x, uint32_t (&e)[8]) {
#pragma unroll
    for (int k = 0; k < 8; k++) e[k] = spread4((x >> (4 * k)) & 15u);
}
__device__ __forceinline__ unsigned warp_sum(unsigned v) {
#pragma unroll
    for (int o = 16; o > 0; o >>= 1) v += __shfl_xor_sync(0xffffffffu, v, o);
    return v;
}

__global__ void __launch_bounds__(256) ld_stage_kernel(uint32_t *__restrict__ dst, const uint32_t *__restrict__ src, int n) {
    const int i = blockIdx.x * blockDim.x + threadIdx.x;
    if (i < n) dst[i] = src[i];
}

__global__ void __launch_bounds__(256)
ld_expand_bg_kernel(int w0, int nU, int npadU, int ncols, int ncolpad, int H, int Wpad, int WP32,
                    const int32_t *__restrict__ bgU, const double *__restrict__ lnc, const uint32_t *__restrict__ tbits,
                    const uint8_t *__restrict__ nr, const uint8_t *__restrict__ nk, const double *__restrict__ C0,
                    double alpha, double beta, double kappa, double inv_abs_kappa, unsigned char *__restrict__ out,
                    int32_t *__restrict__ akey, double *__restrict__ Rp, double *__restrict__ Qp, double *__restrict__ Fp) {
    const int lane = threadIdx.x & 31;
    const int u = blockIdx.x * 8 + (threadIdx.x >> 5);
    const int wl = blockIdx.y, w = w0 + wl;
    if (u >= npadU) return;
    if (u >= nU) {
        if (lane < 2 && 2 * u + lane < ncolpad) {
            akey[(size_t)w * ncolpad + 2 * u + lane] = KEY_PAD;
            Rp[(size_t)w * ncolpad + 2 * u + lane] = -INFINITY;
            Fp[(size_t)w * ncolpad + 2 * u + lane] = 0.0;
        }
        return;
    }
    const int ind = __ldg(bgU + u);
    unsigned A0 = 0, N0 = 0, A1 = 0, N1 = 0, M = 0;
    if (lane < WP32) {
        const uint32_t x0 = __ldg(tbits + ((size_t)w * H + 2 * ind) * WP32 + lane);
        const uint32_t x1 = __ldg(tbits + ((size_t)w * H + 2 * ind + 1) * WP32 + lane);
        const uint4 *cr = reinterpret_cast<const uint4 *>(nr + (size_t)w * Wpad + lane * 32);
        const uint4 *cn = reinterpret_cast<const uint4 *>(nk + (size_t)w * Wpad + lane * 32);
        const uint4 r0 = __ldg(cr), r1 = __ldg(cr + 1), n0 = __ldg(cn), n1 = __ldg(cn + 1);
        const uint32_t rr[8] = {r0.x, r0.y, r0.z, r0.w, r1.x, r1.y, r1.z, r1.w};
        const uint32_t nn[8] = {n0.x, n0.y, n0.z, n0.w, n1.x, n1.y, n1.z, n1.w};
        uint32_t e0[8], e1[8];
        spread32(x0, e0);
        spread32(x1, e1);
#pragma unroll
        for (int k = 0; k < 8; k++) {
            A0 = __dp4a(e0[k], rr[k], A0);
            N0 = __dp4a(e0[k], nn[k], N0);
            A1 = __dp4a(e1[k], rr[k], A1);
            N1 = __dp4a(e1[k], nn[k], N1);
            M = __dp4a(e0[k] & e1[k], nn[k], M);
        }
        uint4 *o0 = reinterpret_cast<uint4 *>(out + ((size_t)wl * ncols + 2 * u) * Wpad) + lane * 2;
        uint4 *o1 = reinterpret_cast<uint4 *>(out + ((size_t)wl * ncols + 2 * u + 1) * Wpad) + lane * 2;
        __stcs(o0, make_uint4(e0[0], e0[1], e0[2], e0[3]));
        __stcs(o0 + 1, make_uint4(e0[4], e0[5], e0[6], e0[7]));
        __stcs(o1, make_uint4(e1[0], e1[1], e1[2], e1[3]));
        __stcs(o1 + 1, make_uint4(e1[4], e1[5], e1[6], e1[7]));
    }
    A0 = warp_sum(A0); N0 = warp_sum(N0); A1 = warp_sum(A1); N1 = warp_sum(N1); M = warp_sum(M);
    if (lane == 0) {
        const double R0 = fma(alpha, (double)A0, beta * (double)(N0 - A0));
        const double R1 = fma(alpha, (double)A1, beta * (double)(N1 - A1));
        const double lc = lnc[u];
        const double p0 = R0 + lc, p1 = R1 + lc;
        Rp[(size_t)w * ncolpad + 2 * u] = p0;
        Rp[(size_t)w * ncolpad + 2 * u + 1] = p1;
        const double k0 = rint(p0 * inv_abs_kappa), k1 = rint(p1 * inv_abs_kappa);
        akey[(size_t)w * ncolpad + 2 * u] = (int32_t)k0;
        akey[(size_t)w * ncolpad + 2 * u + 1] = (int32_t)k1;
        Fp[(size_t)w * ncolpad + 2 * u] = p0 == -INFINITY ? 0.0 : exp(fma(k0, kappa, p0));
        Fp[(size_t)w * ncolpad + 2 * u + 1] = p1 == -INFINITY ? 0.0 : exp(fma(k1, kappa, p1));
        Qp[(size_t)w * nU + u] = (((C0[w] + R0) + R1) + kappa * (double)M) + lc;
    }
}

__global__ void __launch_bounds__(256)
ld_expand_tgt_kernel(int w0, int T, int H, int Wpad, int WP32, int outW, const int32_t *__restrict__ targets,
                     const uint32_t *__restrict__ tbits, const uint8_t *__restrict__ nr, const uint8_t *__restrict__ nk,
                     const double *__restrict__ C0, double alpha, double beta, double kappa,
                     unsigned char *__restrict__ out, double *__restrict__ Rt, double *__restrict__ wll) {
    const int lane = threadIdx.x & 31;
    const int t = blockIdx.x * 8 + (threadIdx.x >> 5);
    const int wl = blockIdx.y, w = w0 + wl;
    if (t >= T) return;
    const int ind = __ldg(targets + t);
    unsigned A0 = 0, N0 = 0, A1 = 0, N1 = 0, M = 0;
    if (lane < WP32) {
        const uint32_t x0 = __ldg(tbits + ((size_t)w * H + 2 * ind) * WP32 + lane);
        const uint32_t x1 = __ldg(tbits + ((size_t)w * H + 2 * ind + 1) * WP32 + lane);
        const uint4 *cr = reinterpret_cast<const uint4 *>(nr + (size_t)w * Wpad + lane * 32);
        const uint4 *cn = reinterpret_cast<const uint4 *>(nk + (size_t)w * Wpad + lane * 32);
        const uint4 r0 = __ldg(cr), r1 = __ldg(cr + 1), n0 = __ldg(cn), n1 = __ldg(cn + 1);
        const uint32_t rr[8] = {r0.x, r0.y, r0.z, r0.w, r1.x, r1.y, r1.z, r1.w};
        const uint32_t nn[8] = {n0.x, n0.y, n0.z, n0.w, n1.x, n1.y, n1.z, n1.w};
        uint32_t e0[8], e1[8];
        spread32(x0, e0);
        spread32(x1, e1);
#pragma unroll
        for (int k = 0; k < 8; k++) {
            A0 = __dp4a(e0[k], rr[k], A0);
            N0 = __dp4a(e0[k], nn[k], N0);
            A1 = __dp4a(e1[k], rr[k], A1);
            N1 = __dp4a(e1[k], nn[k], N1);
            M = __dp4a(e0[k] & e1[k], nn[k], M);
        }
        if (out) {
#pragma unroll
            for (int k = 0; k < 8; k++) {
                e0[k] = (e0[k] * 0xFFu) & nn[k];
                e1[k] = (e1[k] * 0xFFu) & nn[k];
            }
            uint4 *o0 = reinterpret_cast<uint4 *>(out + ((size_t)wl * 2 * T + 2 * t) * Wpad) + lane * 2;
            uint4 *o1 = reinterpret_cast<uint4 *>(out + ((size_t)wl * 2 * T + 2 * t + 1) * Wpad) + lane * 2;
            __stcs(o0, make_uint4(e0[0], e0[1], e0[2], e0[3]));
            __stcs(o0 + 1, make_uint4(e0[4], e0[5], e0[6], e0[7]));
            __stcs(o1, make_uint4(e1[0], e1[1], e1[2], e1[3]));
            __stcs(o1 + 1, make_uint4(e1[4], e1[5], e1[6], e1[7]));
        }
    }
    A0 = warp_sum(A0); N0 = warp_sum(N0); A1 = warp_sum(A1); N1 = warp_sum(N1); M = warp_sum(M);
    if (lane == 0) {
        const double R0 = fma(alpha, (double)A0, beta * (double)(N0 - A0));
        const double R1 = fma(alpha, (double)A1, beta * (double)(N1 - A1));
        Rt[((size_t)w * T + t) * 2] = R0;
        Rt[((size_t)w * T + t) * 2 + 1] = R1;
        wll[((size_t)t * outW + w) * 3 + 2] = ((C0[w] + R0) + R1) + kappa * (double)M;
    }
}

__global__ void __launch_bounds__(256)
ld_store_cols_kernel(const double *__restrict__ src, double *__restrict__ dst, int T, int outW, int w_lo, int ncols) {
    const int64_t per = (int64_t)ncols * 3;
    const int64_t i = blockIdx.x * (int64_t)blockDim.x + threadIdx.x;
    if (i >= (int64_t)T * per) return;
    const int64_t t = i / per, c = i % per;
    const int64_t o = (t * outW + w_lo) * 3 + c;
    dst[o] = src[o];
}

__global__ void __launch_bounds__(256)
ld_pack_cols_kernel(const double *__restrict__ src, double *__restrict__ dst, int T, int outW, int w_lo, int ncols) {
    const int64_t i = blockIdx.x * (int64_t)blockDim.x + threadIdx.x;
    if (i >= (int64_t)T * ncols * 3) return;
    const int64_t c = i % 3, t = (i / 3) % T, w = i / ((int64_t)3 * T);
    dst[i] = src[(t * outW + w_lo + w) * 3 + c];
}

__global__ void __launch_bounds__(256)
ld_windows_kernel(int w_lo, int w_hi, int T, int nW, int outW, int W, int64_t K, const int64_t *__restrict__ wfirst,
                  const int64_t *__restrict__ wlast, const uint64_t *__restrict__ pos, int32_t *__restrict__ wn,
                  uint64_t *__restrict__ ws, uint64_t *__restrict__ we, int32_t *__restrict__ nwout) {
    const int64_t j = blockIdx.x * (int64_t)blockDim.x + threadIdx.x;
    const int span = w_hi - w_lo;
    if (j >= (int64_t)T * span) return;
    const int t = (int)(j / span), w = w_lo + (int)(j % span);
    const int64_t i = (int64_t)t * outW + w;
    if (w == w_lo) nwout[t] = nW;
    if (w >= nW) return;
    const int64_t left = K - (int64_t)w * W;
    wn[i] = (int32_t)(left < W ? left : W);
    ws[i] = pos[wfirst[w]];
    we[i] = pos[wlast[w]];
}

constexpr int IBD0_CHUNKS = 64;
__global__ void __launch_bounds__(256, 4)
ld_ibd0_kernel(int w_off, int T, int nU, int outW, const double *__restrict__ Qp, const int32_t *__restrict__ ownU,
               const double *__restrict__ lognb, double *__restrict__ wll, int stage) {
    extern __shared__ double qs[];
    __shared__ double cm[IBD0_CHUNKS], cs[IBD0_CHUNKS];
    __shared__ double tot_m, tot_s;
    const int w = w_off + blockIdx.x;
    const double *q = Qp + (size_t)w * nU;
    if (stage) {
        for (int u = threadIdx.x; u < nU; u += blockDim.x) qs[u] = __ldg(q + u);
        __syncthreads();
        q = qs;
    }
    const int clen = (nU + IBD0_CHUNKS - 1) / IBD0_CHUNKS;
    const int lane = threadIdx.x & 31, wid = threadIdx.x >> 5;
    for (int c = wid; c < IBD0_CHUNKS; c += 8) {
        const int u0 = c * clen, u1 = min(nU, u0 + clen);
        double m = -INFINITY;
        for (int u = u0 + lane; u < u1; u += 32) m = fmax(m, q[u]);
        for (int o = 16; o > 0; o >>= 1) m = fmax(m, __shfl_xor_sync(0xffffffffu, m, o));
        double s = 0;
        if (m > -INFINITY)
            for (int u = u0 + lane; u < u1; u += 32) s += exp_nonpos(q[u] - m);
        for (int o = 16; o > 0; o >>= 1) s += __shfl_xor_sync(0xffffffffu, s, o);
        if (lane == 0) { cm[c] = m; cs[c] = s; }
    }
    __syncthreads();
    if (wid == 0) {
        double m = fmax(cm[lane], cm[lane + 32]);
        for (int o = 16; o > 0; o >>= 1) m = fmax(m, __shfl_xor_sync(0xffffffffu, m, o));
        double s = 0;
        if (cs[lane] > 0) s += cs[lane] * exp_nonpos(cm[lane] - m);
        if (cs[lane + 32] > 0) s += cs[lane + 32] * exp_nonpos(cm[lane + 32] - m);
        for (int o = 16; o > 0; o >>= 1) s += __shfl_xor_sync(0xffffffffu, s, o);
        if (lane == 0) { tot_m = m; tot_s = s; }
    }
    __syncthreads();
    const double nan = __longlong_as_double(0x7ff8000000000000LL);
    for (int t = threadIdx.x; t < T; t += blockDim.x) {
        const double lnb = lognb[t];
        double r;
        if (!(lnb == lnb)) {
            r = nan;
        } else {
            const int own = ownU[t];
            double x = 0;
            if (own >= 0 && q[own] >= tot_m - 60.0) x = exp_nonpos(q[own] - tot_m);
            if (x + x <= tot_s) {
                r = tot_m + log(tot_s - x) - lnb;
            } else {
                const int oc = own / clen;
                double m = -INFINITY;
                for (int c = 0; c < IBD0_CHUNKS; c++)
                    if (c != oc) m = fmax(m, cm[c]);
                const int u0 = oc * clen, u1 = min(nU, u0 + clen);
                for (int u = u0; u < u1; u++)
                    if (u != own) m = fmax(m, q[u]);
                double s = 0;
                for (int c = 0; c < IBD0_CHUNKS; c++)
                    if (c != oc && cs[c] > 0) s += cs[c] * exp_nonpos(cm[c] - m);
                for (int u = u0; u < u1; u++)
                    if (u != own) s += exp_nonpos(q[u] - m);
                r = m + log(s) - lnb;
            }
        }
        wll[((size_t)t * outW + w) * 3 + 0] = r;
    }
}

namespace mma {
using namespace tcx;
constexpr int BM = 128, BN = 128, KBYTES = 128, UK = 32;
constexpr int MAXKB = 8;
constexpr int A_SLAB = BM * KBYTES;
constexpr int B_SLAB = BN * KBYTES;
constexpr int EPI_WARP0 = 4;
constexpr int NSETS = 4;
constexpr int ETAB_N = 512;

template <int CG_, int NSTAGE_>
struct Cfg {
    static constexpr int CG = CG_, NSTAGE = NSTAGE_;
    static constexpr int TILE_N = BN * CG;
    static constexpr int NACC = 512 / TILE_N;
    static constexpr int SETCOLS = TILE_N / NSETS;
    static constexpr int THREADS = 128 + NSETS * 128;
    static constexpr int OFF_A = 0;
    static constexpr int OFF_B = OFF_A + MAXKB * A_SLAB;
    static constexpr int OFF_KEYS = OFF_B + NSTAGE * B_SLAB;
    static constexpr int OFF_MERGE = OFF_KEYS + NSETS * 4 * SETCOLS * 4;
    static constexpr int OFF_KMAX = OFF_MERGE + NSETS * BM * 16;
    static constexpr int OFF_BAR = OFF_KMAX + 2 * BM * 4;
    static constexpr int NBAR = 2 * MAXKB + 2 * NSTAGE + 2 * NACC + URING;
    static constexpr int OFF_TMEM = OFF_BAR + NBAR * 8;
    static constexpr int OFF_URING = OFF_TMEM + 16;
    static constexpr int OFF_ETAB = OFF_URING + URING * 4;
    static constexpr int SMEM_BYTES = OFF_ETAB + ETAB_N * 8 + 1024;
    static constexpr uint32_t IDESC = (2u << 4)  | (0u << 7)  | (0u << 10)  |
                                      ((uint32_t)(TILE_N >> 3) << 17) | ((uint32_t)((BM * CG) >> 4) << 24);
    static_assert(SMEM_BYTES <= 232448, "over the 227 KB shared memory limit");
    static_assert(SETCOLS % 32 == 0 && SETCOLS <= BN, "epilogue sets split the tile into 32-column chunks");
};

struct Params {
    int w0;
    int nW, MB, NT, KB;
    int n_units;
    int nrows, ncolpad;
    int H, outW;
    int delta;
    double kappa;
    const int32_t *akey;
    const double *Rp;
    const double *Fp;
    int tab_n, dpos;
    const double *Rt;
    const int32_t *row_own;
    const double *C0;
    const double *lognb4;
    double *wll;
    double *wll_host;
    int debug;
    int warm_tiles;
    int *unit_counter;
    int pf_tiles;
    unsigned long long *trace;
};
#define IBD_TRACE(role, ev, tile)                                                                          \
    do {                                                                                                   \
        if (p.trace && blockIdx.x == 0 && lane == 0 && tr_n < 1024 && (p.debug != 9 || (ev) == 5))        \
            p.trace[(role) * 1024 + tr_n++] = ((unsigned long long)clock64() << 16) | ((ev) << 12) | ((tile) & 0xfff); \
    } while (0)

template <class CF>
__global__ void __launch_bounds__(CF::THREADS, 1)
ld_mma_kernel(const __grid_constant__ CUtensorMap tmapA, const __grid_constant__ CUtensorMap tmapB, const Params p) {
    constexpr int CG = CF::CG, NSTAGE = CF::NSTAGE, NACC = CF::NACC, TILE_N = CF::TILE_N;
    constexpr int OFF_A = CF::OFF_A, OFF_B = CF::OFF_B, OFF_KEYS = CF::OFF_KEYS, OFF_MERGE = CF::OFF_MERGE;
    constexpr int OFF_BAR = CF::OFF_BAR, OFF_TMEM = CF::OFF_TMEM, OFF_KMAX = CF::OFF_KMAX;
    extern __shared__ unsigned char smem_raw[];
    unsigned char *smem = reinterpret_cast<unsigned char *>((reinterpret_cast<uintptr_t>(smem_raw) + 1023) & ~(uintptr_t)1023);
    uint64_t *bars = reinterpret_cast<uint64_t *>(smem + OFF_BAR);
    uint64_t *a_full = bars, *a_empty = bars + MAXKB;
    uint64_t *b_full = bars + 2 * MAXKB, *b_empty = b_full + NSTAGE;
    uint64_t *acc_full = b_empty + NSTAGE, *acc_empty = acc_full + NACC;
    uint64_t *ufull = acc_empty + NACC;
    int *uring = reinterpret_cast<int *>(smem + CF::OFF_URING);
    uint32_t *tmem_slot = reinterpret_cast<uint32_t *>(smem + OFF_TMEM);

    const int warp = threadIdx.x >> 5, lane = threadIdx.x & 31;
    uint32_t rank = 0;
    if constexpr (CG == 2) asm volatile("mov.u32 %0, %%cluster_ctarank;" : "=r"(rank));

    if (p.trace && warp == 1 && lane == 0 && blockIdx.x < 256) {
        unsigned long long t;
        asm volatile("mov.u64 %0, %%globaltimer;" : "=l"(t));
        p.trace[3 * 1024 + blockIdx.x * 4] = t;
        unsigned smid;
        asm volatile("mov.u32 %0, %%smid;" : "=r"(smid));
        p.trace[3 * 1024 + blockIdx.x * 4 + 2] = smid;
    }
    if (warp == 0 && lane == 0) {
        asm volatile("prefetch.tensormap [%0];" ::"l"(&tmapA) : "memory");
        asm volatile("prefetch.tensormap [%0];" ::"l"(&tmapB) : "memory");
    }
    if (warp == 1 && lane == 0) {
        for (int i = 0; i < MAXKB; i++) { mbar_init(a_full + i, 1); mbar_init(a_empty + i, 1); }
        for (int i = 0; i < URING; i++) mbar_init(ufull + i, 1);
        for (int i = 0; i < NSTAGE; i++) { mbar_init(b_full + i, 1); mbar_init(b_empty + i, 1); }
        for (int i = 0; i < NACC; i++) { mbar_init(acc_full + i, 1); mbar_init(acc_empty + i, 4 * NSETS * CG); }
        asm volatile("fence.mbarrier_init.release.cluster;" ::: "memory");
    }
    if (warp == 3)
        for (int i = lane; i < 2 * BM; i += 32) reinterpret_cast<int *>(smem + OFF_KMAX)[i] = KEY_INIT;
    for (int i = threadIdx.x; i < p.tab_n; i += CF::THREADS)
        reinterpret_cast<double *>(smem + CF::OFF_ETAB)[i] = exp(-p.kappa * (double)(i - p.delta));
    if (warp == 2) {
        if constexpr (CG == 1) {
            asm volatile("tcgen05.alloc.cta_group::1.sync.aligned.shared::cta.b32 [%0], %1;" ::"r"(smem_u32(tmem_slot)), "r"(512u) : "memory");
            asm volatile("tcgen05.relinquish_alloc_permit.cta_group::1.sync.aligned;" ::: "memory");
        } else {
            asm volatile("tcgen05.alloc.cta_group::2.sync.aligned.shared::cta.b32 [%0], %1;" ::"r"(smem_u32(tmem_slot)), "r"(512u) : "memory");
            asm volatile("tcgen05.relinquish_alloc_permit.cta_group::2.sync.aligned;" ::: "memory");
        }
    }
    tc_fence_before();
    __syncthreads();
    if constexpr (CG == 2) cluster_sync_all();
    tc_fence_after();
    const uint32_t tmem_base = *tmem_slot;

    if (warp < EPI_WARP0) {
    if (warp == 0) {
        if (lane == 0) {
            int st = 0;
            uint32_t ph = 0;
            int u_next = -1;
            auto fetch_unit = [&]() {
                const int v = atomicAdd(p.unit_counter, 1);
                return v < p.n_units ? v : -1;
            };
            int pending = -1;
            if (rank == 0) {
                u_next = fetch_unit();
                unit_publish<CG>(uring, ufull, 0, u_next);
                pending = atomicAdd(p.unit_counter, 1);
            }
            for (int it = 0;; it++) {
                int u;
                if (rank == 0) {
                    u = u_next;
                    if (u < 0) break;
                } else {
                    u = unit_of(uring, ufull, it);
                    if (u < 0) break;
                }
                const int w = u / p.MB, mb = u % p.MB;
                auto load_a = [&](int kb) {
                    mbar_wait(a_empty + kb, (uint32_t)((it & 1) ^ 1));
                    if (rank == 0) mbar_expect_tx(a_full + kb, (uint32_t)(CG * A_SLAB));
                    tma_load_3d_cg<CG>(smem + OFF_A + kb * A_SLAB, &tmapA, a_full + kb, kb * KBYTES, (mb * CG + (int)rank) * BM, w);
                };
                for (int n = 0; n < p.NT; n++)
                    for (int kb = 0; kb < p.KB; kb++) {
                        if (n == 0) load_a(kb);
                        if (n + p.pf_tiles < p.NT)
                            tma_prefetch_3d(&tmapB, kb * KBYTES, ((n + p.pf_tiles) * CG + (int)rank) * BN, w);
                        mbar_wait(b_empty + st, ph ^ 1u);
                        if (rank == 0) mbar_expect_tx(b_full + st, (uint32_t)(CG * B_SLAB));
                        tma_load_3d_cg<CG>(smem + OFF_B + st * B_SLAB, &tmapB, b_full + st, kb * KBYTES,
                                           (n * CG + (int)rank) * BN, w);
                        if (++st == NSTAGE) { st = 0; ph ^= 1u; }
                    }
                if (rank == 0) {
                    u_next = pending < p.n_units ? pending : -1;
                    unit_publish<CG>(uring, ufull, it + 1, u_next);
                    if (u_next >= 0) pending = atomicAdd(p.unit_counter, 1);
                }
            }
        }
    } else if (warp == 1) {
        if (rank == 0) {
            int st = 0;
            uint32_t ph = 0;
            int it = 0;
            uint32_t g = 0;
            int tr_n = 0;
            const uint64_t adesc0 = umma_desc_sw128(smem_u32(smem + OFF_A));
            const uint64_t bdesc0 = umma_desc_sw128(smem_u32(smem + OFF_B));
            for (;; it++) {
                const int u_cur = unit_of(uring, ufull, it);
                if (u_cur < 0) break;
                for (int n = 0; n < p.NT; n++, g++) {
                    const bool first = n == 0, last = n == p.NT - 1;
                    const uint32_t acc = g % NACC, use = g / NACC;
                    IBD_TRACE(0, 1, g);
                    mbar_wait(acc_empty + acc, (use & 1u) ^ 1u);
                    IBD_TRACE(0, 2, g);
                    const uint32_t d_tmem = tmem_base + acc * TILE_N;
                    for (int kb = 0; kb < p.KB; kb += 2) {
                        const bool two = kb + 1 < p.KB;
                        int st2 = st + 1;
                        uint32_t ph2 = ph;
                        if (st2 == NSTAGE) { st2 = 0; ph2 ^= 1u; }
                        const bool r1 = mbar_test(b_full + st, ph);
                        const bool r2 = two ? mbar_test(b_full + st2, ph2) : true;
                        if (!r1 || !r2) IBD_TRACE(0, 3, g);
                        if (!r1) mbar_wait(b_full + st, ph);
                        if (!r2) mbar_wait(b_full + st2, ph2);
                        if (!r1 || !r2) IBD_TRACE(0, 4, g);
                        if (first) {
                            IBD_TRACE(0, 6, kb);
                            mbar_wait(a_full + kb, (uint32_t)(it & 1));
                            if (two) mbar_wait(a_full + kb + 1, (uint32_t)(it & 1));
                            IBD_TRACE(0, 7, kb);
                        }
                        tc_fence_after();
                        if (elect_one()) {
                            const uint64_t ad = adesc0 + (uint64_t)((kb * A_SLAB) >> 4);
                            const uint64_t bd = bdesc0 + (uint64_t)((st * B_SLAB) >> 4);
#pragma unroll
                            for (int k = 0; k < KBYTES / UK; k++)
                                umma_i8_cg<CG>(d_tmem, ad + (uint64_t)(k * (UK >> 4)), bd + (uint64_t)(k * (UK >> 4)), CF::IDESC,
                                               (uint32_t)((kb | k) != 0));
                            tc_commit_cg<CG>(b_empty + st);
                            if (last) tc_commit_cg<CG>(a_empty + kb);
                            if (two) {
                                const uint64_t ad2 = ad + (uint64_t)(A_SLAB >> 4);
                                const uint64_t bd2 = bdesc0 + (uint64_t)((st2 * B_SLAB) >> 4);
#pragma unroll
                                for (int k = 0; k < KBYTES / UK; k++)
                                    umma_i8_cg<CG>(d_tmem, ad2 + (uint64_t)(k * (UK >> 4)), bd2 + (uint64_t)(k * (UK >> 4)), CF::IDESC, 1u);
                                tc_commit_cg<CG>(b_empty + st2);
                                if (last) tc_commit_cg<CG>(a_empty + kb + 1);
                            }
                            if (kb + 2 >= p.KB) tc_commit_cg<CG>(acc_full + acc);
                        }
                        __syncwarp();
                        if (two) { st = st2; ph = ph2; }
                        if (++st == NSTAGE) { st = 0; ph ^= 1u; }
                    }
                }
                IBD_TRACE(0, 5, (u_cur % p.MB) | (((u_cur / p.MB) & 0x1ff) << 3));
            }
            if (p.trace && lane == 0 && blockIdx.x < 256) p.trace[3 * 1024 + blockIdx.x * 4 + 3] = (unsigned long long)it;
        }
    } else {
        const double2 *mb_buf = reinterpret_cast<const double2 *>(smem + OFF_MERGE);
        const int r0 = (warp - 2) * 64 + lane * 2;
        asm volatile("bar.arrive 2, %0;" ::"n"(NSETS * 128 + 64) : "memory");
        for (int it = 0;; it++) {
            const int u = unit_of(uring, ufull, it);
            if (u < 0) break;
            const int w = p.w0 + u / p.MB, mb = u % p.MB;
            const int row = (mb * CG + (int)rank) * BM + r0;
            const bool ok = row < p.nrows;
            double rw0 = 0.0, rw1 = 0.0, lnb = 0.0;
            if (ok) {
                rw0 = __ldg(p.Rt + (size_t)w * p.nrows + row);
                rw1 = __ldg(p.Rt + (size_t)w * p.nrows + row + 1);
                lnb = __ldg(p.lognb4 + (row >> 1));
            }
            const double c0w = __ldg(p.C0 + w);
            asm volatile("bar.sync 1, %0;" ::"n"(NSETS * 128 + 64) : "memory");
            double A[2], S[2];
#pragma unroll
            for (int h = 0; h < 2; h++) {
                double2 o[NSETS];
#pragma unroll
                for (int q = 0; q < NSETS; q++) o[q] = mb_buf[q * BM + r0 + h];
                double M2 = o[0].x;
#pragma unroll
                for (int q = 1; q < NSETS; q++) M2 = fmax(M2, o[q].x);
                double S2 = 0.0;
#pragma unroll
                for (int q = 0; q < NSETS; q++) S2 = fma(o[q].y, exp_nonpos(o[q].x - M2), S2);
                S[h] = S2;
                A[h] = (S2 > 0.0) ? M2 + (h ? rw1 : rw0) : -INFINITY;
            }
            asm volatile("bar.arrive 2, %0;" ::"n"(NSETS * 128 + 64) : "memory");
            const double mm = fmax(A[0], A[1]);
            double r = mm + log(fma(S[0], exp_nonpos(A[0] - mm), S[1] * exp_nonpos(A[1] - mm)));
            if (mm == -INFINITY) r = -INFINITY;
            r = (c0w + r) - lnb;
            if (!(lnb == lnb)) r = __longlong_as_double(0x7ff8000000000000LL);
            if (ok) {
                double *o = p.wll + ((size_t)(row >> 1) * p.outW + w) * 3;
                o[1] = r;
                if (p.wll_host) {
                    double *h = p.wll_host + ((size_t)(row >> 1) * p.outW + w) * 3;
                    const double l0 = o[0], l2 = o[2];
                    h[0] = l0;
                    h[1] = r;
                    h[2] = l2;
                }
            }
        }
    }
    } else {
        constexpr int SETCOLS = CF::SETCOLS;
        const int ew = warp - EPI_WARP0, set = ew >> 2, quarter = warp & 3;
        const int rloc = quarter * 32 + lane;
        int *skeys = reinterpret_cast<int *>(smem + OFF_KEYS) + ew * SETCOLS;
        double2 *merge = reinterpret_cast<double2 *>(smem + OFF_MERGE);
        int *skmax_all = reinterpret_cast<int *>(smem + OFF_KMAX);
        uint32_t g0 = 0;
        int it = 0;
        int tr_n = 0;
        const int tr_role = ew == 0 ? 1 : (ew == 15 ? 2 : 3);
        for (;; it++, g0 += (uint32_t)p.NT) {
            const int u = unit_of(uring, ufull, it);
            if (u < 0) break;
            const int w = p.w0 + u / p.MB, mb = u % p.MB;
            const int row = (mb * CG + (int)rank) * BM + rloc;
            const bool row_ok = row < p.nrows;
            const int own0 = row_ok ? p.row_own[row] : -1;
            const int32_t *akw = p.akey + (size_t)w * p.ncolpad;
            const bool tab = p.tab_n > 0;
            const double *etab = reinterpret_cast<const double *>(smem + CF::OFF_ETAB);
            const double *rpw = (tab ? p.Fp : p.Rp) + (size_t)w * p.ncolpad;
            int vref = KEY_INIT;
            int kmax = row_ok ? KEY_INIT : (1 << 30);
            int *skmax = skmax_all + (it & 1) * BM + rloc;
            double m = -INFINITY, s = 0.0;
            constexpr int NCH = SETCOLS / 32;
            int4 kv_next = make_int4(0, 0, 0, 0);
            double rp_next[NCH];
            auto fetch = [&](int n) {
                const int col = n * TILE_N + set * SETCOLS;
                if (lane < SETCOLS / 4) kv_next = __ldg(reinterpret_cast<const int4 *>(akw + col) + lane);
#pragma unroll
                for (int c = 0; c < NCH; c++) rp_next[c] = __ldg(rpw + col + c * 32 + lane);
            };
            fetch(0);
            for (int n = 0; n < p.NT; n++) {
                const uint32_t g = g0 + (uint32_t)n;
                const int slot = (int)(g % NACC);
                const uint32_t use = g / NACC;
                const int col0 = n * TILE_N + set * SETCOLS;
                double rp_cur[NCH];
#pragma unroll
                for (int c = 0; c < NCH; c++) rp_cur[c] = rp_next[c];
                __syncwarp();
                if (lane < SETCOLS / 4) reinterpret_cast<int4 *>(skeys)[lane] = kv_next;
                __syncwarp();
                if (n + 1 < p.NT) fetch(n + 1);
                const bool own_here = own0 >= col0 && own0 < col0 + SETCOLS;
                const bool any_own = __any_sync(0xffffffffu, own_here);
                kmax = max(kmax, *skmax);
                if (tr_role < 3) IBD_TRACE(tr_role, 1, g);
                mbar_wait_relaxed(acc_full + slot, use & 1u);
                if (tr_role < 3) IBD_TRACE(tr_role, 2, g);
                tc_fence_after();
                const uint32_t taddr = tmem_base + slot * TILE_N + set * SETCOLS + ((uint32_t)(quarter * 32) << 16);
                auto load_chunk = [&](int c, int (&v)[32]) -> int {
                    __syncwarp();
                    tmem_ld32(taddr + c * 32, v);
                    tmem_ld_wait();
#pragma unroll
                    for (int j = 0; j < 32; j += 4) {
                        const int4 a4 = *reinterpret_cast<const int4 *>(skeys + c * 32 + j);
                        v[j] = a4.x - v[j];
                        v[j + 1] = a4.y - v[j + 1];
                        v[j + 2] = a4.z - v[j + 2];
                        v[j + 3] = a4.w - v[j + 3];
                    }
                    if (any_own) {
                        const int jo = own0 - (col0 + c * 32);
#pragma unroll
                        for (int j = 0; j < 32; j++)
                            if ((j & ~1) == jo) v[j] = KEY_PAD;
                    }
                    int c0 = __vimax3_s32(v[0], v[1], v[2]), c1 = __vimax3_s32(v[8], v[9], v[10]);
                    int c2 = __vimax3_s32(v[16], v[17], v[18]), c3 = __vimax3_s32(v[24], v[25], v[26]);
                    c0 = __vimax3_s32(c0, v[3], v[4]); c1 = __vimax3_s32(c1, v[11], v[12]);
                    c2 = __vimax3_s32(c2, v[19], v[20]); c3 = __vimax3_s32(c3, v[27], v[28]);
                    c0 = __vimax3_s32(c0, v[5], v[6]); c1 = __vimax3_s32(c1, v[13], v[14]);
                    c2 = __vimax3_s32(c2, v[21], v[22]); c3 = __vimax3_s32(c3, v[29], v[30]);
                    c0 = __vimax3_s32(c0, v[7], c1); c2 = __vimax3_s32(c2, v[15], c3);
                    return __vimax3_s32(c0, c2, max(v[23], v[31]));
                };
                if (n < p.warm_tiles && p.debug != 1) {
                    int tm = KEY_PAD;
#pragma unroll
                    for (int c = 0; c < NCH; c++) {
                        int v[32];
                        tm = max(tm, load_chunk(c, v));
                    }
                    if (tm > kmax) {
                        kmax = tm;
                        if (row_ok) atomicMax(skmax, tm);
                    }
                    asm volatile("bar.sync 3, %0;" ::"n"(NSETS * 128) : "memory");
                    kmax = max(kmax, *skmax);
                }
#pragma unroll
                for (int c = 0; c < NCH; c++) {
                    if (p.debug == 1) break;
                    int v[32];
                    const int cm = load_chunk(c, v);
                    if (cm > kmax) {
                        kmax = cm;
                        if (row_ok) atomicMax(skmax, cm);
                    }
                    const int thr = kmax - p.delta;
                    if (tab && row_ok && cm > vref + p.dpos) {
                        s *= exp(p.kappa * (double)(kmax - vref));
                        vref = kmax;
                    }
                    uint32_t mask = 0;
                    if (__any_sync(0xffffffffu, cm > thr)) {
#pragma unroll
                        for (int j = 0; j < 32; j++)
                            if (v[j] > thr) mask |= 1u << j;
                    }
                    uint32_t mk = mask;
                    const int trips = __reduce_max_sync(0xffffffffu, (unsigned)__popc(mk));
                    for (int q = 0; q < trips; q++) {
                        const bool act = mk != 0u;
                        const int j = act ? __ffs((int)mk) - 1 : 0;
                        mk &= mk - 1u;
                        const int vj = pick32(v, j);
                        const double rp = __shfl_sync(0xffffffffu, rp_cur[c], j);
                        if (tab) {
                            if (act) s = fma(etab[vj - vref + p.delta], rp, s);
                        } else {
                            const int M = skeys[c * 32 + j] - vj;
                            if (act) lse_add_fast(m, s, fma(p.kappa, (double)M, rp));
                        }
                    }
                }
                tc_fence_before();
                __syncwarp();
                if (lane == 0) mbar_arrive_leader<CG>(acc_empty + slot);
                if (tr_role < 3) IBD_TRACE(tr_role, 3, g);
            }
            if (set == 0) skmax_all[((it + 1) & 1) * BM + rloc] = KEY_INIT;
            if (tr_role < 3) IBD_TRACE(tr_role, 4, g0);
            asm volatile("bar.sync 2, %0;" ::"n"(NSETS * 128 + 64) : "memory");
            merge[set * BM + rloc] = tab ? make_double2(-p.kappa * (double)vref, s) : make_double2(m, s);
            asm volatile("bar.arrive 1, %0;" ::"n"(NSETS * 128 + 64) : "memory");
            if (tr_role < 3) IBD_TRACE(tr_role, 7, g0);
        }
    }

    tc_fence_before();
    __syncthreads();
    if (p.trace && warp == 1 && lane == 0 && blockIdx.x < 256) {
        unsigned long long t;
        asm volatile("mov.u64 %0, %%globaltimer;" : "=l"(t));
        p.trace[3 * 1024 + blockIdx.x * 4 + 1] = t;
    }
    if constexpr (CG == 2) cluster_sync_all();
    if (warp == 2) {
        tc_fence_after();
        if constexpr (CG == 1)
            asm volatile("tcgen05.dealloc.cta_group::1.sync.aligned.b32 %0, %1;" ::"r"(tmem_base), "r"(512u) : "memory");
        else
            asm volatile("tcgen05.dealloc.cta_group::2.sync.aligned.b32 %0, %1;" ::"r"(tmem_base), "r"(512u) : "memory");
    }
}
}

typedef CUresult (*EncodeTiledFn)(CUtensorMap *, CUtensorMapDataType, cuuint32_t, void *, const cuuint64_t *,
                                  const cuuint64_t *, const cuuint32_t *, const cuuint32_t *, CUtensorMapInterleave,
                                  CUtensorMapSwizzle, CUtensorMapL2promotion, CUtensorMapFloatOOBfill);

static EncodeTiledFn get_encode_fn() {
    static const EncodeTiledFn fn = [] {
        void *p = nullptr;
        cudaDriverEntryPointQueryResult q;
        if (cudaGetDriverEntryPoint("cuTensorMapEncodeTiled", &p, cudaEnableDefault, &q) != cudaSuccess || !p)
            return (EncodeTiledFn) nullptr;
        return reinterpret_cast<EncodeTiledFn>(p);
    }();
    return fn;
}

static int make_operand_map(CUtensorMap *m, void *base, int Wpad, int rows, int nW) {
    EncodeTiledFn fn = get_encode_fn();
    if (!fn) {
        set_error("[::] ERROR: cuTensorMapEncodeTiled is not available from the CUDA driver.");
        return 1;
    }
    const cuuint64_t dims[3] = {(cuuint64_t)Wpad, (cuuint64_t)rows, (cuuint64_t)nW};
    const cuuint64_t strides[2] = {(cuuint64_t)Wpad, (cuuint64_t)Wpad * (cuuint64_t)rows};
    const cuuint32_t box[3] = {(cuuint32_t)mma::KBYTES, (cuuint32_t)mma::BM, 1};
    const cuuint32_t estr[3] = {1, 1, 1};
    const CUresult r = fn(m, CU_TENSOR_MAP_DATA_TYPE_UINT8, 3, base, dims, strides, box, estr, CU_TENSOR_MAP_INTERLEAVE_NONE,
                          CU_TENSOR_MAP_SWIZZLE_128B, CU_TENSOR_MAP_L2_PROMOTION_L2_256B, CU_TENSOR_MAP_FLOAT_OOB_FILL_NONE);
    if (r != CUDA_SUCCESS) {
        set_error("[::] ERROR: cuTensorMapEncodeTiled failed (%d) for a %d x %d x %d operand.", (int)r, Wpad, rows, nW);
        return 1;
    }
    return 0;
}

template <class CF>
static int launch_mma_cfg(int n_units, int sm_count, cudaStream_t st, const CUtensorMap &a, const CUtensorMap &b,
                          const mma::Params &p) {
    IBD_CUDA(cudaFuncSetAttribute(mma::ld_mma_kernel<CF>, cudaFuncAttributeMaxDynamicSharedMemorySize, CF::SMEM_BYTES));
    const int groups = std::max(1, std::min(n_units, sm_count / CF::CG));
    cudaLaunchConfig_t cfg = {};
    cfg.gridDim = dim3((unsigned)(groups * CF::CG));
    cfg.blockDim = dim3((unsigned)CF::THREADS);
    cfg.dynamicSmemBytes = CF::SMEM_BYTES;
    cfg.stream = st;
    cudaLaunchAttribute at[1];
    at[0].id = cudaLaunchAttributeClusterDimension;
    at[0].val.clusterDim.x = CF::CG;
    at[0].val.clusterDim.y = 1;
    at[0].val.clusterDim.z = 1;
    cfg.attrs = at;
    cfg.numAttrs = 1;
    IBD_CUDA(cudaLaunchKernelEx(&cfg, mma::ld_mma_kernel<CF>, a, b, p));
    return 0;
}
static int mma_variant() {
    static const int v = [] {
        const char *s = getenv("IBDGEM_MMA_VARIANT");
        return s ? atoi(s) : 2;
    }();
    return v;
}
static int mma_cg(int variant) { return variant == 1 ? 1 : 2; }
static int launch_mma(int variant, int n_units, int sm_count, cudaStream_t st, const CUtensorMap &a, const CUtensorMap &b,
                      const mma::Params &p) {
    if (variant == 1) return launch_mma_cfg<mma::Cfg<1, 5>>(n_units, sm_count, st, a, b, p);
    return launch_mma_cfg<mma::Cfg<2, 5>>(n_units, sm_count, st, a, b, p);
}
static double screen_nats(int ncols) {
    static const double forced = [] {
        const char *s = getenv("IBDGEM_SCREEN_NATS");
        const double f = s ? atof(s) : 0.0;
        return (f >= 8.0 && f <= 700.0) ? f : 0.0;
    }();
    if (forced > 0.0) return forced;
    return std::min(SCREEN_NATS, log((double)std::max(ncols, 2)) + 16.2);
}

bool ld_tensor_eligible(ibdgem_engine *e, int32_t n_targets, int32_t n_bg, const uint8_t *tgt_counts) {
    if (tgt_counts || e->prm.variable_sites_only) return false;
    if (!e->depth_linear || !(e->kappa < -1e-3)) return false;
    if (e->nW_shared <= 0 || e->K_shared <= 0) return false;
    const int Wpad = (e->prm.window_size + 127) / 128 * 128;
    if (Wpad > mma::MAXKB * mma::KBYTES) return false;
    if ((int64_t)e->prm.max_cov * Wpad >= (1 << 24)) return false;
    if (n_targets <= 0 || n_bg <= 0) return false;
    if (ceil(SCREEN_NATS / -e->kappa) > 1e6) return false;
    return true;
}

void ld_tensor_release(ibdgem_engine *e) {
    LdCache *c = e->ld;
    if (!c) return;
    dev_free(e, c->d_infsite, c->b_infsite);
    dev_free(e, c->d_nk, c->b_nk);
    dev_free(e, c->d_nr, c->b_nr);
    dev_free(e, c->d_l0, c->b_l0);
    dev_free(e, c->d_C0, c->b_C0);
    dev_free(e, c->d_tbits, c->b_tbits);
    delete c;
    e->ld = nullptr;
}

void ld_tensor_invalidate(ibdgem_engine *e) {
    if (e->ld) e->ld->valid = false;
}

static int build_cache(ibdgem_engine *e) {
    if (e->ld && e->ld->valid) return 0;
    const int Wpad = (e->prm.window_size + 127) / 128 * 128;
    if (e->ld && (e->ld->nW != e->nW_shared || e->ld->N != e->N || e->ld->Wpad != Wpad)) ld_tensor_release(e);
    LdCache *c = e->ld;
    if (!c) {
        c = new LdCache();
        e->ld = c;
        c->nW = e->nW_shared;
        c->W = e->prm.window_size;
        c->Wpad = Wpad;
        c->WP32 = c->Wpad / 32;
        c->KB = c->Wpad / 128;
        c->N = e->N;
        c->H = 2 * e->N;
        const size_t slots = (size_t)c->nW * c->Wpad;
        c->b_infsite = slots * 4; c->b_nk = slots; c->b_nr = slots; c->b_l0 = slots * 8; c->b_C0 = (size_t)c->nW * 8;
        c->b_tbits = (size_t)c->nW * c->H * c->WP32 * 4;
        if (dev_alloc(e, (void **)&c->d_infsite, c->b_infsite) || dev_alloc(e, (void **)&c->d_nk, c->b_nk) ||
            dev_alloc(e, (void **)&c->d_nr, c->b_nr) || dev_alloc(e, (void **)&c->d_l0, c->b_l0) ||
            dev_alloc(e, (void **)&c->d_C0, c->b_C0) || dev_alloc(e, (void **)&c->d_tbits, c->b_tbits))
            return 1;
    }
    c->K = e->K_shared;
    IBD_CUDA(cudaMemsetAsync(c->d_infsite, 0xFF, c->b_infsite, e->stream));
    IBD_CUDA(cudaMemsetAsync(c->d_nk, 0, c->b_nk, e->stream));
    IBD_CUDA(cudaMemsetAsync(c->d_nr, 0, c->b_nr, e->stream));
    IBD_CUDA(cudaMemsetAsync(c->d_l0, 0, c->b_l0, e->stream));
    {
        LaunchScope ls(e, K_LD_COMPACT);
        ld_compact_kernel<<<(unsigned)((e->S + 255) / 256), 256, 0, e->stream>>>(
            e->S, e->d_status, e->d_rank, e->d_nref, e->d_nalt, e->d_lnP, e->C, c->W, c->Wpad, c->d_infsite, c->d_nk,
            c->d_nr, c->d_l0);
    }
    {
        LaunchScope ls(e, K_LD_C0);
        ld_c0_kernel<<<c->nW, 256, 0, e->stream>>>(c->d_l0, c->Wpad, c->d_C0);
    }
    IBD_CUDA(cudaGetLastError());
    c->valid = true;
    c->tw_upto = 0;
    return 0;
}

int ld_transpose_launch(ibdgem_engine *e, int w_begin, int w_end, const int32_t *infsite, int Wpad, int WP32, int H, uint32_t *tbits) {
    LaunchScope ls(e, K_LD_TRANSPOSE);
    const int words = (H + 31) / 32;
    for (int w0 = w_begin; w0 < w_end; w0 += MAX_GRID_Y)
        ld_transpose_kernel<<<dim3((words + 7) / 8, std::min(MAX_GRID_Y, w_end - w0)), 1024, 0, e->stream>>>(
            w0, e->d_bits, e->Wh, H, infsite, Wpad, WP32, tbits);
    IBD_CUDA(cudaGetLastError());
    return 0;
}

static int cache_windows(ibdgem_engine *e, int w_hi) {
    LdCache *c = e->ld;
    if (e->shard_count > 1 && c->tw_upto == 0) {
        int32_t wb = 0;
        window_shard_bounds(e, &wb, nullptr, nullptr, nullptr);
        c->tw_upto = wb;
    }
    if (c->tw_upto >= w_hi) return 0;
    if (ld_transpose_launch(e, c->tw_upto, w_hi, c->d_infsite, c->Wpad, c->WP32, c->H, c->d_tbits)) return 1;
    c->tw_upto = w_hi;
    return 0;
}

int ld_tensor_prepare(ibdgem_engine *e) {
    if (build_cache(e) || ensure_table(e, e->S)) return 1;
    return cache_windows(e, e->ld->nW);
}

int ld_tensor_score(ibdgem_engine *e, int32_t T, const int32_t *h_targets, const int32_t *d_targets, int32_t n_bg,
                    const int32_t *h_bg, int32_t pu_idx, int32_t outW, double *d_wll, int32_t *d_wn, uint64_t *d_ws,
                    uint64_t *d_we, int32_t *d_nwout) {
    if (build_cache(e)) return 1;
    LdCache *c = e->ld;
    std::vector<int32_t> mult((size_t)c->N, 0), where((size_t)c->N, -1);
    int64_t total_bg = 0;
    for (int n = 0; n < n_bg; n++)
        if (h_bg[n] != pu_idx) { mult[h_bg[n]]++; total_bg++; }
    std::vector<int32_t> bgU;
    std::vector<double> lnc;
    bgU.reserve((size_t)c->N);
    lnc.reserve((size_t)c->N);
    for (int32_t b = 0; b < c->N; b++)
        if (mult[b]) {
            where[b] = (int32_t)bgU.size();
            bgU.push_back(b);
            lnc.push_back(mult[b] == 1 ? 0.0 : log((double)mult[b]));
        }
    const int nU = (int)bgU.size();
    const double nan = (double)NAN;
    std::vector<int32_t> ownU(T), row_own(2 * (size_t)T);
    std::vector<double> lognb(T), lognb4(T);
    for (int t = 0; t < T; t++) {
        const int own = where[h_targets[t]];
        const int64_t nb = total_bg - (own >= 0 ? mult[h_targets[t]] : 0);
        ownU[t] = own;
        lognb[t] = nb > 0 ? log((double)nb) : nan;
        lognb4[t] = nb > 0 ? log(4.0 * (double)nb) : nan;
        row_own[2 * t] = row_own[2 * t + 1] = own >= 0 ? 2 * own : -1;
    }
    const int nW = c->nW;
    std::vector<int> range_end;
    const bool in_flight = e->chunks_waited < (int)e->chunk_end.size() && e->chunk_end.size() > 1 &&
                           cudaEventQuery(e->chunk_ev[e->chunk_end.size() - 1]) == cudaErrorNotReady;
    if (in_flight && c->tw_upto == 0) {
        int w = 0;
        for (size_t k = 0; k < e->chunk_end.size(); k++) {
            while (w < nW && e->h_wlast[(size_t)w] < e->chunk_end[k]) w++;
            range_end.push_back(k + 1 == e->chunk_end.size() ? nW : w);
        }
    } else {
        static const int tail_div = [] { const char *st = getenv("IBDGEM_LD_TAIL_DIV"); return st ? atoi(st) : 0; }();
        if (e->h_wll_out && tail_div > 1 && nW >= 8 * tail_div) range_end.push_back(nW - nW / tail_div);
        range_end.push_back(nW);
    }
    bool by_chunk = in_flight && c->tw_upto == 0;
    int32_t shard_wb = 0, shard_we = nW;
    int64_t shard_se = e->S;
    const bool sharded = e->shard_count > 1;
    if (sharded) {
        window_shard_bounds(e, &shard_wb, &shard_we, nullptr, &shard_se);
        range_end.clear();
        const int span = shard_we - shard_wb;
        static const int parts_env = [] { const char *sp = getenv("IBDGEM_SHARD_PARTS"); return sp ? atoi(sp) : 3; }();
        const int64_t units = (int64_t)span * ((2 * T + 255) / 256);
        int parts = 1;
        if (parts_env < 0) parts = std::min(span, -parts_env);
        else if (e->h_wll_out && parts_env > 1 && (size_t)T * span * 24 >= ((size_t)20 << 20))
            parts = (int)std::max<int64_t>(1, std::min<int64_t>(parts_env, units / (8 * std::max(1, e->sm_count / 2))));
        const int64_t wsum = (int64_t)parts * (parts + 1) / 2;
        int64_t acc = 0;
        for (int k = 0; k < parts; k++) {
            acc += parts - k;
            range_end.push_back(shard_wb + (int)((int64_t)span * acc / wsum));
        }
        by_chunk = false;
    }
    auto range_sites = [&](size_t k) { return by_chunk ? e->chunk_end[k] : shard_se; };
    const int nrows = 2 * T;
    if (nU == 0) {
        double *d_Rt;
        if (ensure_table(e, e->S) || cache_windows(e, nW) || scratch(e, SC_MMA_ROWLSE, (size_t)nW * nrows * 8, (void **)&d_Rt))
            return 1;
        {
            LaunchScope ls(e, K_LD_WINDOWS);
            const int64_t n = (int64_t)T * nW;
            ld_windows_kernel<<<(unsigned)((n + 255) / 256), 256, 0, e->stream>>>(
                0, nW, T, nW, outW, c->W, c->K, e->d_wfirst, e->d_wlast, e->d_pos, d_wn, d_ws, d_we, d_nwout);
        }
        {
            LaunchScope ls(e, K_LD_EXPAND_TGT);
            for (int w0 = 0; w0 < nW; w0 += MAX_GRID_Y)
                ld_expand_tgt_kernel<<<dim3((unsigned)((T + 7) / 8), (unsigned)std::min(MAX_GRID_Y, nW - w0)), 256, 0, e->stream>>>(
                    w0, T, c->H, c->Wpad, c->WP32, outW, d_targets, c->d_tbits, c->d_nr, c->d_nk, c->d_C0, e->alpha, e->beta,
                    e->kappa, nullptr, d_Rt, d_wll);
        }
        IBD_CUDA(cudaGetLastError());
        return 0;
    }
    const int ncols = 2 * nU;
    const int variant = mma_variant();
    const int CG = mma_cg(variant);
    const int NT = (ncols + mma::BN * CG - 1) / (mma::BN * CG);
    const int ncolpad = NT * mma::BN * CG;
    const int MB = (nrows + mma::BM * CG - 1) / (mma::BM * CG);

    const size_t per_window = (size_t)(ncols + nrows) * c->Wpad;
    static const size_t budget = [] {
        const char *sb = getenv("IBDGEM_LD_BUDGET_MB");
        return sb && atol(sb) > 0 ? (size_t)atol(sb) << 20 : LD_OPERAND_BUDGET;
    }();
    const int nWb = (int)std::max<size_t>(1, std::min<size_t>({(size_t)nW, budget / per_window, (size_t)MAX_GRID_Y}));
    int32_t *d_bgU, *d_ownU, *d_rowown, *d_akey;
    double *d_lnc, *d_lognb, *d_lognb4, *d_Rp, *d_Qp, *d_Rt, *d_Fp;
    unsigned char *d_A, *d_B;
    const size_t misc_i = (size_t)nU + T + 2 * (size_t)T;
    const size_t misc_d = (size_t)nU + 2 * (size_t)T;
    if (scratch(e, SC_MMA_MISC, misc_i * 4 + misc_d * 8 + 64, (void **)&d_lnc) ||
        scratch(e, SC_MMA_BGIDX, (size_t)nW * ncolpad * 4, (void **)&d_akey) ||
        scratch(e, SC_MMA_ROWLSE, (2 * (size_t)nW * ncolpad + (size_t)nW * nU + (size_t)nW * nrows) * 8, (void **)&d_Rp) ||
        scratch(e, SC_MMA_TGT, (size_t)nWb * nrows * c->Wpad, (void **)&d_A) ||
        scratch(e, SC_MMA_BG, (size_t)nWb * ncols * c->Wpad, (void **)&d_B))
        return 1;
    d_lognb = d_lnc + nU;
    d_lognb4 = d_lognb + T;
    d_bgU = reinterpret_cast<int32_t *>(d_lognb4 + T);
    d_ownU = d_bgU + nU;
    d_rowown = d_ownU + T;
    d_Fp = d_Rp + (size_t)nW * ncolpad;
    d_Qp = d_Fp + (size_t)nW * ncolpad;
    d_Rt = d_Qp + (size_t)nW * nU;
    {
        void *h_misc;
        if (pinned_stage(e, misc_d * 8 + misc_i * 4, &h_misc)) return 1;
        double *hd = static_cast<double *>(h_misc);
        memcpy(hd, lnc.data(), (size_t)nU * 8);
        memcpy(hd + nU, lognb.data(), (size_t)T * 8);
        memcpy(hd + nU + T, lognb4.data(), (size_t)T * 8);
        int32_t *hi = reinterpret_cast<int32_t *>(hd + misc_d);
        memcpy(hi, bgU.data(), (size_t)nU * 4);
        memcpy(hi + nU, ownU.data(), (size_t)T * 4);
        memcpy(hi + nU + T, row_own.data(), (size_t)T * 8);
        LaunchScope ls(e, K_LD_STAGE);
        const int n = (int)((misc_d * 8 + misc_i * 4) / 4);
        ld_stage_kernel<<<(n + 255) / 256, 256, 0, e->stream>>>(reinterpret_cast<uint32_t *>(d_lnc),
                                                               static_cast<const uint32_t *>(h_misc), n);
    }

    const bool stream_out = (range_end.size() > 1 || sharded) && e->h_wll_out != nullptr;
    const bool stream_dev = e->d_wll_out_device != nullptr;
    double *h_wll_mapped = nullptr;
    if (e->h_wll_out) {
        cudaPointerAttributes attr;
        if (cudaPointerGetAttributes(&attr, e->h_wll_out) == cudaSuccess && attr.type == cudaMemoryTypeHost && attr.devicePointer)
            h_wll_mapped = static_cast<double *>(attr.devicePointer);
        else
            cudaGetLastError();
    }
    static const int direct_env = [] { const char *sd = getenv("IBDGEM_LD_DIRECT_STORE"); return sd ? atoi(sd) : 1; }();
    const bool direct = direct_env && h_wll_mapped != nullptr && !by_chunk && !sharded;
    if (stream_out || stream_dev || direct) {
        if (!e->d2h_stream) IBD_CUDA(cudaStreamCreateWithFlags(&e->d2h_stream, cudaStreamNonBlocking));
        e->wll_streamed = stream_out || direct;
        e->wll_dev_streamed = stream_dev;
    }
    auto launch_ibd0 = [&](int wa, int wb_) -> int {
        LaunchScope ls(e, K_LD_IBD0);
        const size_t q_smem = (size_t)nU * 8 <= 160 * 1024 ? (size_t)nU * 8 : 0;
        IBD_CUDA(cudaFuncSetAttribute(ld_ibd0_kernel, cudaFuncAttributeMaxDynamicSharedMemorySize, 160 * 1024));
        ld_ibd0_kernel<<<wb_ - wa, 256, q_smem, e->stream>>>(wa, T, nU, outW, d_Qp, d_ownU, d_lognb, d_wll, q_smem ? 1 : 0);
        return 0;
    };
    int w_lo = shard_wb;
    for (size_t rk = 0; rk < range_end.size(); rk++) {
    const int w_hi = range_end[rk];
    if (ensure_table(e, range_sites(rk))) return 1;
    if (w_hi == w_lo && !(sharded && rk == 0)) continue;
    if (w_hi > w_lo && cache_windows(e, w_hi)) return 1;
    if (!sharded || rk == 0) {
        LaunchScope ls(e, K_LD_WINDOWS);
        const int b_lo = sharded ? 0 : w_lo, b_hi = sharded ? nW : w_hi;
        const int64_t n = (int64_t)T * (b_hi - b_lo);
        ld_windows_kernel<<<(unsigned)((n + 255) / 256), 256, 0, e->stream>>>(
            b_lo, b_hi, T, nW, outW, c->W, c->K, e->d_wfirst, e->d_wlast, e->d_pos, d_wn, d_ws, d_we, d_nwout);
    }
    if (e->ev_book && !e->book_ready && (sharded ? rk == 0 : w_hi == nW)) {
        IBD_CUDA(cudaEventRecord(e->ev_book, e->stream));
        e->book_ready = true;
    }
    IBD_CUDA(cudaGetLastError());
    if (w_hi == w_lo) continue;
    for (int w0 = w_lo; w0 < w_hi; w0 += nWb) {
        const int nw = std::min(nWb, w_hi - w0);
        {
            LaunchScope ls(e, K_LD_EXPAND_BG);
            const int npadU = ncolpad / 2;
            ld_expand_bg_kernel<<<dim3((unsigned)((npadU + 7) / 8), (unsigned)nw), 256, 0, e->stream>>>(
                w0, nU, npadU, ncols, ncolpad, c->H, c->Wpad, c->WP32, d_bgU, d_lnc, c->d_tbits, c->d_nr, c->d_nk, c->d_C0,
                e->alpha, e->beta, e->kappa, 1.0 / -e->kappa, d_B, d_akey, d_Rp, d_Qp, d_Fp);
        }
        {
            LaunchScope ls(e, K_LD_EXPAND_TGT);
            ld_expand_tgt_kernel<<<dim3((unsigned)((T + 7) / 8), (unsigned)nw), 256, 0, e->stream>>>(
                w0, T, c->H, c->Wpad, c->WP32, outW, d_targets, c->d_tbits, c->d_nr, c->d_nk, c->d_C0, e->alpha, e->beta,
                e->kappa, d_A, d_Rt, d_wll);
        }
        IBD_CUDA(cudaGetLastError());
        CUtensorMap mapA, mapB;
        if (make_operand_map(&mapA, d_A, c->Wpad, nrows, nw)) return 1;
        if (make_operand_map(&mapB, d_B, c->Wpad, ncols, nw)) return 1;
        mma::Params p;
        p.w0 = w0;
        p.nW = nw; p.MB = MB; p.NT = NT; p.KB = c->KB;
        p.n_units = nw * MB;
        p.nrows = nrows; p.ncolpad = ncolpad;
        p.H = c->H; p.outW = outW;
        p.delta = (int)ceil(screen_nats(ncols) / -e->kappa) + 2;
        p.kappa = e->kappa;
        p.akey = d_akey; p.Rp = d_Rp; p.Rt = d_Rt;
        p.Fp = d_Fp;
        {
            static const int tab_env = [] { const char *st = getenv("IBDGEM_MMA_TABLE"); return st ? atoi(st) : 1; }();
            const int dpos = (int)std::min(256.0, floor(600.0 / -e->kappa));
            const int tab_n = p.delta + dpos + 1;
            const bool tab = tab_env && dpos >= 8 && tab_n <= mma::ETAB_N;
            p.tab_n = tab ? tab_n : 0;
            p.dpos = dpos;
        }
        p.row_own = d_rowown;
        p.C0 = c->d_C0; p.lognb4 = d_lognb4; p.wll = d_wll;
        p.wll_host = direct ? h_wll_mapped : nullptr;
        if (direct && launch_ibd0(w0, w0 + nw)) return 1;
        {
            static const int dbg = [] { const char *sdbg = getenv("IBDGEM_MMA_DEBUG"); return sdbg ? atoi(sdbg) : 0; }();
            p.debug = dbg;
        }
        {
            static const int wt = [] { const char *sw = getenv("IBDGEM_MMA_WARM_TILES"); return sw ? atoi(sw) : 1; }();
            p.warm_tiles = wt;
        }
        {
            int *d_unit;
            if (scratch(e, SC_MMA_UNIT, 64, (void **)&d_unit)) return 1;
            IBD_CUDA(cudaMemsetAsync(d_unit, 0, 4, e->stream));
            p.unit_counter = d_unit;
            static const int pf = [] { const char *spf = getenv("IBDGEM_MMA_PF"); return spf ? atoi(spf) : mma::PF_TILES; }();
            p.pf_tiles = pf;
        }
        p.trace = nullptr;
        const char *trace_path = getenv("IBDGEM_MMA_TRACE");
        unsigned long long *d_trace = nullptr;
        if (trace_path) {
            IBD_CUDA(cudaMalloc(&d_trace, 4 * 1024 * 8));
            IBD_CUDA(cudaMemsetAsync(d_trace, 0, 4 * 1024 * 8, e->stream));
            p.trace = d_trace;
        }
        {
            LaunchScope ls(e, K_LD_MMA);
            if (launch_mma(variant, p.n_units, e->sm_count, e->stream, mapA, mapB, p)) return 1;
        }
        IBD_CUDA(cudaGetLastError());
        if (d_trace) {
            std::vector<unsigned long long> h(4 * 1024);
            IBD_CUDA(cudaMemcpyAsync(h.data(), d_trace, h.size() * 8, cudaMemcpyDeviceToHost, e->stream));
            IBD_CUDA(cudaStreamSynchronize(e->stream));
            if (FILE *fh = fopen(trace_path, "wb")) {
                fwrite(h.data(), 8, h.size(), fh);
                fclose(fh);
            }
            cudaFree(d_trace);
        }
    }
    if (!direct && launch_ibd0(w_lo, w_hi)) return 1;
    if (stream_out || stream_dev) {
        while (e->range_ev.size() <= rk) {
            cudaEvent_t ev;
            IBD_CUDA(cudaEventCreateWithFlags(&ev, cudaEventDisableTiming));
            e->range_ev.push_back(ev);
        }
        IBD_CUDA(cudaEventRecord(e->range_ev[rk], e->stream));
        IBD_CUDA(cudaStreamWaitEvent(e->d2h_stream, e->range_ev[rk], 0));
        if (stream_dev) {
            if (T >= 256) {
                const int64_t n = (int64_t)T * (w_hi - w_lo) * 3;
                ld_store_cols_kernel<<<(unsigned)((n + 255) / 256), 256, 0, e->d2h_stream>>>(d_wll, e->d_wll_out_device, T, outW, w_lo, w_hi - w_lo);
                e->k_launches[K_LD_WINDOWS]++;
            } else {
                IBD_CUDA(cudaMemcpy2DAsync(e->d_wll_out_device + (size_t)w_lo * 3, (size_t)outW * 24, d_wll + (size_t)w_lo * 3,
                                           (size_t)outW * 24, (size_t)(w_hi - w_lo) * 24, (size_t)T, cudaMemcpyDefault, e->d2h_stream));
            }
        }
        if (stream_out && sharded && e->shard_compact) {
            double *d_pack;
            const int64_t n = (int64_t)T * (w_hi - w_lo) * 3, off = (int64_t)T * (w_lo - shard_wb) * 3;
            if (scratch(e, SC_WLL_PACK, (size_t)T * (shard_we - shard_wb) * 24, (void **)&d_pack)) return 1;
            ld_pack_cols_kernel<<<(unsigned)((n + 255) / 256), 256, 0, e->d2h_stream>>>(d_wll, d_pack + off, T, outW, w_lo, w_hi - w_lo);
            e->k_launches[K_LD_WINDOWS]++;
            IBD_CUDA(cudaMemcpyAsync(e->h_wll_out + off, d_pack + off, (size_t)n * 8, cudaMemcpyDeviceToHost, e->d2h_stream));
        } else if (stream_out && !direct) {
            if (h_wll_mapped && T >= 256) {
                const int64_t n = (int64_t)T * (w_hi - w_lo) * 3;
                ld_store_cols_kernel<<<(unsigned)((n + 255) / 256), 256, 0, e->d2h_stream>>>(d_wll, h_wll_mapped, T, outW, w_lo, w_hi - w_lo);
                e->k_launches[K_LD_WINDOWS]++;
            } else {
                IBD_CUDA(cudaMemcpy2DAsync(e->h_wll_out + (size_t)w_lo * 3, (size_t)outW * 24, d_wll + (size_t)w_lo * 3, (size_t)outW * 24,
                                           (size_t)(w_hi - w_lo) * 24, (size_t)T, cudaMemcpyDeviceToHost, e->d2h_stream));
            }
        }
    }
    w_lo = w_hi;
    }
    if ((stream_out || direct) && outW > nW && !sharded) {
        const size_t rk = range_end.size();
        while (e->range_ev.size() <= rk) {
            cudaEvent_t ev;
            IBD_CUDA(cudaEventCreateWithFlags(&ev, cudaEventDisableTiming));
            e->range_ev.push_back(ev);
        }
        IBD_CUDA(cudaEventRecord(e->range_ev[rk], e->stream));
        IBD_CUDA(cudaStreamWaitEvent(e->d2h_stream, e->range_ev[rk], 0));
        if (h_wll_mapped && T >= 256) {
            const int64_t n = (int64_t)T * (outW - nW) * 3;
            ld_store_cols_kernel<<<(unsigned)((n + 255) / 256), 256, 0, e->d2h_stream>>>(d_wll, h_wll_mapped, T, outW, nW, outW - nW);
            e->k_launches[K_LD_WINDOWS]++;
        } else {
            IBD_CUDA(cudaMemcpy2DAsync(e->h_wll_out + (size_t)nW * 3, (size_t)outW * 24, d_wll + (size_t)nW * 3, (size_t)outW * 24,
                                       (size_t)(outW - nW) * 24, (size_t)T, cudaMemcpyDeviceToHost, e->d2h_stream));
        }
    }
    IBD_CUDA(cudaGetLastError());
    return 0;
}

}
```

Before: 1251000 billion.

## Fuse haplotype transpose and bg/target operand expansion into one build kernel

Drops the separate transpose-to-tbits cache and the two expand kernels for background and targets. A single ld_build kernel now transposes the panel bits into shared memory per window and individual group. From that tile it computes the dot-product counts and writes the B operand, the A operand (through a per-individual target list), and the per-column scalars. This removes the tbits global buffer, its caching pass, and a second read of bit data per window, at the cost of more index staging and shared memory per block.

```diff
diff --git a/ibdgem_b200/csrc/engine.cu b/ibdgem_b200/csrc/engine.cu
--- a/ibdgem_b200/csrc/engine.cu
+++ b/ibdgem_b200/csrc/engine.cu
@@ -22,7 +22,7 @@
 static const char *const kKernelNameList[] = {
     "site_table",     "scan_count",    "scan_offsets",  "scan_rank",    "window_nonld", "counters",
     "expand_sites",   "ld_general",    "ld_finalize",   "ld_compact",   "ld_c0",        "ld_transpose",
-    "ld_stage",       "ld_expand_bg",  "ld_expand_tgt", "ld_windows",   "ld_ibd0",
+    "ld_stage",       "ld_build",      "ld_windows",    "ld_ibd0",
     "ld_mma",         "viterbi",       "viterbi_back",  "viterbi_out",  "fill",
     "v_slots",        "v_wmap",        "v_tw",          "v_sort",       "v_expand_a",  "v_expand_b",   "ld_vmma",
     "window_linear",  "posterior_fwd", "posterior_bwd", "posterior_fwd_log", "posterior_bwd_log",
@@ -1499,7 +1499,7 @@
     }
     if (vtensor) {
     } else if (tensor) {
-        if (ld_tensor_score(e, T, targets, d_targets, n_bg, bg, pu_idx, outW, d_wll, d_wn, d_ws, d_we, d_nwout)) return 1;
+        if (ld_tensor_score(e, T, targets, n_bg, bg, pu_idx, outW, d_wll, d_wn, d_ws, d_we, d_nwout)) return 1;
         e->last_ld_path = 1;
     } else {
         {
diff --git a/ibdgem_b200/csrc/engine.h b/ibdgem_b200/csrc/engine.h
--- a/ibdgem_b200/csrc/engine.h
+++ b/ibdgem_b200/csrc/engine.h
@@ -37,8 +37,7 @@
     K_LD_C0,
     K_LD_TRANSPOSE,
     K_LD_STAGE,
-    K_LD_EXPAND_BG,
-    K_LD_EXPAND_TGT,
+    K_LD_BUILD,
     K_LD_WINDOWS,
     K_LD_IBD0,
     K_LD_MMA,
@@ -204,7 +203,7 @@
 
 bool ld_tensor_eligible(ibdgem_engine *e, int32_t n_targets, int32_t n_bg, const uint8_t *tgt_counts);
 int ld_tensor_prepare(ibdgem_engine *e);
-int ld_tensor_score(ibdgem_engine *e, int32_t T, const int32_t *h_targets, const int32_t *d_targets, int32_t n_bg,
+int ld_tensor_score(ibdgem_engine *e, int32_t T, const int32_t *h_targets, int32_t n_bg,
                     const int32_t *h_bg, int32_t pu_idx, int32_t outW, double *d_wll , int32_t *d_wn,
                     uint64_t *d_ws, uint64_t *d_we, int32_t *d_nwout);
 void ld_tensor_release(ibdgem_engine *e);
diff --git a/ibdgem_b200/csrc/ld_mma.cu b/ibdgem_b200/csrc/ld_mma.cu
--- a/ibdgem_b200/csrc/ld_mma.cu
+++ b/ibdgem_b200/csrc/ld_mma.cu
@@ -14,7 +14,6 @@
 
 struct LdCache {
     bool valid = false;
-    int tw_upto = 0;
     int32_t nW = 0;
     int64_t K = 0;
     int W = 0, Wpad = 0, WP32 = 0, KB = 0;
@@ -24,8 +23,7 @@
     uint8_t *d_nr = nullptr;
     double *d_l0 = nullptr;
     double *d_C0 = nullptr;
-    uint32_t *d_tbits = nullptr;
-    size_t b_infsite = 0, b_nk = 0, b_nr = 0, b_l0 = 0, b_C0 = 0, b_tbits = 0;
+    size_t b_infsite = 0, b_nk = 0, b_nr = 0, b_l0 = 0, b_C0 = 0;
 };
 
 constexpr int KEY_PAD = -(1 << 30);
@@ -79,13 +77,11 @@
     return x;
 }
 
-__global__ void __launch_bounds__(1024)
-ld_transpose_kernel(int w_off, const uint32_t *__restrict__ bits, int64_t Wh, int H, const int32_t *__restrict__ infsite,
-                    int Wpad, int WP32, uint32_t *__restrict__ tbits) {
-    __shared__ uint32_t tile[256 * 33];
-    const int w = w_off + blockIdx.y, j0 = blockIdx.x * 8;
-    const int lane = threadIdx.x & 31, g = threadIdx.x >> 5;
-    if (g < WP32) {
+constexpr int TILE_LD = 33;
+__device__ __forceinline__ void load_window_tile(int w, int j0, const uint32_t *__restrict__ bits, int64_t Wh,
+                                                 const int32_t *__restrict__ infsite, int Wpad, int WP32,
+                                                 uint32_t *__restrict__ tile, int lane, int warp, int nwarps) {
+    for (int g = warp; g < WP32; g += nwarps) {
         const int32_t s = infsite[(size_t)w * Wpad + g * 32 + lane];
         const uint32_t *row = bits + (size_t)(s < 0 ? 0 : s) * Wh;
         uint32_t word[8];
@@ -100,22 +96,27 @@
             for (int jj = 0; jj < 8; jj++) word[jj] = (s >= 0 && j0 + jj < Wh) ? __ldg(row + j0 + jj) : 0u;
         }
 #pragma unroll
-        for (int jj = 0; jj < 8; jj++) tile[(jj * 32 + lane) * 33 + g] = transpose32(word[jj], lane);
-    }
+        for (int jj = 0; jj < 8; jj++) tile[(jj * 32 + lane) * TILE_LD + g] = transpose32(word[jj], lane);
+    }
+}
+
+__global__ void __launch_bounds__(1024)
+ld_transpose_kernel(int w_off, const uint32_t *__restrict__ bits, int64_t Wh, int H, const int32_t *__restrict__ infsite,
+                    int Wpad, int WP32, uint32_t *__restrict__ tbits) {
+    __shared__ uint32_t tile[256 * TILE_LD];
+    const int w = w_off + blockIdx.y, j0 = blockIdx.x * 8;
+    const int lane = threadIdx.x & 31, g = threadIdx.x >> 5;
+    load_window_tile(w, j0, bits, Wh, infsite, Wpad, WP32, tile, lane, g, 32);
     __syncthreads();
     if (lane < WP32)
         for (int hl = g; hl < 256; hl += 32) {
             const int hap = j0 * 32 + hl;
-            if (hap < H) tbits[((size_t)w * H + hap) * WP32 + lane] = tile[hl * 33 + lane];
+            if (hap < H) tbits[((size_t)w * H + hap) * WP32 + lane] = tile[hl * TILE_LD + lane];
         }
 }
 
 
 __device__ __forceinline__ uint32_t spread4(uint32_t nib) { return (nib * 0x00204081u) & 0x01010101u; }
-__device__ __forceinline__ void spread32(uint32_t x, uint32_t (&e)[8]) {
-#pragma unroll
-    for (int k = 0; k < 8; k++) e[k] = spread4((x >> (4 * k)) & 15u);
-}
 __device__ __forceinline__ unsigned warp_sum(unsigned v) {
 #pragma unroll
     for (int o = 16; o > 0; o >>= 1) v += __shfl_xor_sync(0xffffffffu, v, o);
@@ -127,120 +128,112 @@
     if (i < n) dst[i] = src[i];
 }
 
-__global__ void __launch_bounds__(256)
-ld_expand_bg_kernel(int w0, int nU, int npadU, int ncols, int ncolpad, int H, int Wpad, int WP32,
-                    const int32_t *__restrict__ bgU, const double *__restrict__ lnc, const uint32_t *__restrict__ tbits,
-                    const uint8_t *__restrict__ nr, const uint8_t *__restrict__ nk, const double *__restrict__ C0,
-                    double alpha, double beta, double kappa, double inv_abs_kappa, unsigned char *__restrict__ out,
-                    int32_t *__restrict__ akey, double *__restrict__ Rp, double *__restrict__ Qp, double *__restrict__ Fp) {
-    const int lane = threadIdx.x & 31;
-    const int u = blockIdx.x * 8 + (threadIdx.x >> 5);
-    const int wl = blockIdx.y, w = w0 + wl;
-    if (u >= npadU) return;
-    if (u >= nU) {
-        if (lane < 2 && 2 * u + lane < ncolpad) {
-            akey[(size_t)w * ncolpad + 2 * u + lane] = KEY_PAD;
-            Rp[(size_t)w * ncolpad + 2 * u + lane] = -INFINITY;
-            Fp[(size_t)w * ncolpad + 2 * u + lane] = 0.0;
-        }
-        return;
-    }
-    const int ind = __ldg(bgU + u);
-    unsigned A0 = 0, N0 = 0, A1 = 0, N1 = 0, M = 0;
-    if (lane < WP32) {
-        const uint32_t x0 = __ldg(tbits + ((size_t)w * H + 2 * ind) * WP32 + lane);
-        const uint32_t x1 = __ldg(tbits + ((size_t)w * H + 2 * ind + 1) * WP32 + lane);
-        const uint4 *cr = reinterpret_cast<const uint4 *>(nr + (size_t)w * Wpad + lane * 32);
-        const uint4 *cn = reinterpret_cast<const uint4 *>(nk + (size_t)w * Wpad + lane * 32);
-        const uint4 r0 = __ldg(cr), r1 = __ldg(cr + 1), n0 = __ldg(cn), n1 = __ldg(cn + 1);
-        const uint32_t rr[8] = {r0.x, r0.y, r0.z, r0.w, r1.x, r1.y, r1.z, r1.w};
-        const uint32_t nn[8] = {n0.x, n0.y, n0.z, n0.w, n1.x, n1.y, n1.z, n1.w};
-        uint32_t e0[8], e1[8];
-        spread32(x0, e0);
-        spread32(x1, e1);
-#pragma unroll
-        for (int k = 0; k < 8; k++) {
-            A0 = __dp4a(e0[k], rr[k], A0);
-            N0 = __dp4a(e0[k], nn[k], N0);
-            A1 = __dp4a(e1[k], rr[k], A1);
-            N1 = __dp4a(e1[k], nn[k], N1);
-            M = __dp4a(e0[k] & e1[k], nn[k], M);
-        }
-        uint4 *o0 = reinterpret_cast<uint4 *>(out + ((size_t)wl * ncols + 2 * u) * Wpad) + lane * 2;
-        uint4 *o1 = reinterpret_cast<uint4 *>(out + ((size_t)wl * ncols + 2 * u + 1) * Wpad) + lane * 2;
-        __stcs(o0, make_uint4(e0[0], e0[1], e0[2], e0[3]));
-        __stcs(o0 + 1, make_uint4(e0[4], e0[5], e0[6], e0[7]));
-        __stcs(o1, make_uint4(e1[0], e1[1], e1[2], e1[3]));
-        __stcs(o1 + 1, make_uint4(e1[4], e1[5], e1[6], e1[7]));
-    }
-    A0 = warp_sum(A0); N0 = warp_sum(N0); A1 = warp_sum(A1); N1 = warp_sum(N1); M = warp_sum(M);
-    if (lane == 0) {
-        const double R0 = fma(alpha, (double)A0, beta * (double)(N0 - A0));
-        const double R1 = fma(alpha, (double)A1, beta * (double)(N1 - A1));
-        const double lc = lnc[u];
-        const double p0 = R0 + lc, p1 = R1 + lc;
-        Rp[(size_t)w * ncolpad + 2 * u] = p0;
-        Rp[(size_t)w * ncolpad + 2 * u + 1] = p1;
-        const double k0 = rint(p0 * inv_abs_kappa), k1 = rint(p1 * inv_abs_kappa);
-        akey[(size_t)w * ncolpad + 2 * u] = (int32_t)k0;
-        akey[(size_t)w * ncolpad + 2 * u + 1] = (int32_t)k1;
-        Fp[(size_t)w * ncolpad + 2 * u] = p0 == -INFINITY ? 0.0 : exp(fma(k0, kappa, p0));
-        Fp[(size_t)w * ncolpad + 2 * u + 1] = p1 == -INFINITY ? 0.0 : exp(fma(k1, kappa, p1));
-        Qp[(size_t)w * nU + u] = (((C0[w] + R0) + R1) + kappa * (double)M) + lc;
-    }
-}
-
-__global__ void __launch_bounds__(256)
-ld_expand_tgt_kernel(int w0, int T, int H, int Wpad, int WP32, int outW, const int32_t *__restrict__ targets,
-                     const uint32_t *__restrict__ tbits, const uint8_t *__restrict__ nr, const uint8_t *__restrict__ nk,
-                     const double *__restrict__ C0, double alpha, double beta, double kappa,
-                     unsigned char *__restrict__ out, double *__restrict__ Rt, double *__restrict__ wll) {
-    const int lane = threadIdx.x & 31;
-    const int t = blockIdx.x * 8 + (threadIdx.x >> 5);
-    const int wl = blockIdx.y, w = w0 + wl;
-    if (t >= T) return;
-    const int ind = __ldg(targets + t);
-    unsigned A0 = 0, N0 = 0, A1 = 0, N1 = 0, M = 0;
-    if (lane < WP32) {
-        const uint32_t x0 = __ldg(tbits + ((size_t)w * H + 2 * ind) * WP32 + lane);
-        const uint32_t x1 = __ldg(tbits + ((size_t)w * H + 2 * ind + 1) * WP32 + lane);
-        const uint4 *cr = reinterpret_cast<const uint4 *>(nr + (size_t)w * Wpad + lane * 32);
-        const uint4 *cn = reinterpret_cast<const uint4 *>(nk + (size_t)w * Wpad + lane * 32);
-        const uint4 r0 = __ldg(cr), r1 = __ldg(cr + 1), n0 = __ldg(cn), n1 = __ldg(cn + 1);
-        const uint32_t rr[8] = {r0.x, r0.y, r0.z, r0.w, r1.x, r1.y, r1.z, r1.w};
-        const uint32_t nn[8] = {n0.x, n0.y, n0.z, n0.w, n1.x, n1.y, n1.z, n1.w};
-        uint32_t e0[8], e1[8];
-        spread32(x0, e0);
-        spread32(x1, e1);
-#pragma unroll
-        for (int k = 0; k < 8; k++) {
-            A0 = __dp4a(e0[k], rr[k], A0);
-            N0 = __dp4a(e0[k], nn[k], N0);
-            A1 = __dp4a(e1[k], rr[k], A1);
-            N1 = __dp4a(e1[k], nn[k], N1);
-            M = __dp4a(e0[k] & e1[k], nn[k], M);
-        }
-        if (out) {
-#pragma unroll
-            for (int k = 0; k < 8; k++) {
-                e0[k] = (e0[k] * 0xFFu) & nn[k];
-                e1[k] = (e1[k] * 0xFFu) & nn[k];
-            }
-            uint4 *o0 = reinterpret_cast<uint4 *>(out + ((size_t)wl * 2 * T + 2 * t) * Wpad) + lane * 2;
-            uint4 *o1 = reinterpret_cast<uint4 *>(out + ((size_t)wl * 2 * T + 2 * t + 1) * Wpad) + lane * 2;
-            __stcs(o0, make_uint4(e0[0], e0[1], e0[2], e0[3]));
-            __stcs(o0 + 1, make_uint4(e0[4], e0[5], e0[6], e0[7]));
-            __stcs(o1, make_uint4(e1[0], e1[1], e1[2], e1[3]));
-            __stcs(o1 + 1, make_uint4(e1[4], e1[5], e1[6], e1[7]));
-        }
-    }
-    A0 = warp_sum(A0); N0 = warp_sum(N0); A1 = warp_sum(A1); N1 = warp_sum(N1); M = warp_sum(M);
-    if (lane == 0) {
-        const double R0 = fma(alpha, (double)A0, beta * (double)(N0 - A0));
-        const double R1 = fma(alpha, (double)A1, beta * (double)(N1 - A1));
-        Rt[((size_t)w * T + t) * 2] = R0;
-        Rt[((size_t)w * T + t) * 2 + 1] = R1;
-        wll[((size_t)t * outW + w) * 3 + 2] = ((C0[w] + R0) + R1) + kappa * (double)M;
+constexpr int BUILD_THREADS = 256;
+constexpr int BUILD_TSLOTS = 512;
+__global__ void __launch_bounds__(BUILD_THREADS, 4)
+ld_build_kernel(int w0, int N, int T, int ncols, int ncolpad, int nU, int Wpad, int WP32, int outW,
+                const uint32_t *__restrict__ bits, int64_t Wh, const int32_t *__restrict__ infsite,
+                const uint8_t *__restrict__ nr, const uint8_t *__restrict__ nk, const double *__restrict__ C0,
+                const int32_t *__restrict__ where, const int32_t *__restrict__ tptr, const int32_t *__restrict__ tlist,
+                const double *__restrict__ lnc, double alpha, double beta, double kappa, double inv_abs_kappa,
+                unsigned char *__restrict__ A, unsigned char *__restrict__ B, int32_t *__restrict__ akey,
+                double *__restrict__ Rp, double *__restrict__ Qp, double *__restrict__ Fp, double *__restrict__ Rt,
+                double *__restrict__ wll) {
+    constexpr int NWARPS = BUILD_THREADS / 32;
+    __shared__ uint32_t tile[256 * TILE_LD];
+    __shared__ uint4 cnt_r[64], cnt_n[64];
+    __shared__ int32_t s_u[128], s_tp[129], s_tl[BUILD_TSLOTS];
+    __shared__ double s_lnc[128];
+    const int wl = blockIdx.y, w = w0 + wl, j0 = blockIdx.x * 8;
+    const int lane = threadIdx.x & 31, warp = threadIdx.x >> 5;
+    const int nchunk = Wpad / 16;
+    const int ind0 = j0 * 16, nind = min(128, N - ind0);
+    const int tbase = tptr[ind0], nslot = tptr[ind0 + nind] - tbase;
+    const double c0 = C0[w];
+    for (int i = threadIdx.x; i <= nind; i += BUILD_THREADS) {
+        s_tp[i] = tptr[ind0 + i];
+        if (i < nind) {
+            const int u = where[ind0 + i];
+            s_u[i] = u;
+            s_lnc[i] = u >= 0 ? lnc[u] : 0.0;
+        }
+    }
+    for (int k = threadIdx.x; k < min(nslot, BUILD_TSLOTS); k += BUILD_THREADS) s_tl[k] = tlist[tbase + k];
+    load_window_tile(w, j0, bits, Wh, infsite, Wpad, WP32, tile, lane, warp, NWARPS);
+    for (int c = threadIdx.x; c < nchunk; c += BUILD_THREADS) {
+        cnt_r[c] = __ldg(reinterpret_cast<const uint4 *>(nr + (size_t)w * Wpad) + c);
+        cnt_n[c] = __ldg(reinterpret_cast<const uint4 *>(nk + (size_t)w * Wpad) + c);
+    }
+    if (B && blockIdx.x == 0)
+        for (int k = ncols + threadIdx.x; k < ncolpad; k += BUILD_THREADS) {
+            akey[(size_t)w * ncolpad + k] = KEY_PAD;
+            Rp[(size_t)w * ncolpad + k] = -INFINITY;
+            Fp[(size_t)w * ncolpad + k] = 0.0;
+        }
+    __syncthreads();
+    auto slot_target = [&](int k) { return k - tbase < BUILD_TSLOTS ? s_tl[k - tbase] : tlist[k]; };
+    for (int i = warp; i < nind; i += NWARPS) {
+        const int u = s_u[i], k0 = s_tp[i], k1 = s_tp[i + 1];
+        if (u < 0 && k0 == k1) continue;
+        const uint32_t *x0w = tile + 2 * i * TILE_LD, *x1w = x0w + TILE_LD;
+        unsigned A0 = 0, N0 = 0, A1 = 0, N1 = 0, M = 0;
+        for (int c = lane; c < nchunk; c += 32) {
+            const int sh = (c & 1) * 16;
+            const uint32_t x0 = x0w[c >> 1] >> sh, x1 = x1w[c >> 1] >> sh;
+            const uint4 r4 = cnt_r[c], n4 = cnt_n[c];
+            const uint32_t rr[4] = {r4.x, r4.y, r4.z, r4.w}, nn[4] = {n4.x, n4.y, n4.z, n4.w};
+            uint32_t e0[4], e1[4];
+#pragma unroll
+            for (int k = 0; k < 4; k++) {
+                e0[k] = spread4((x0 >> (4 * k)) & 15u);
+                e1[k] = spread4((x1 >> (4 * k)) & 15u);
+                A0 = __dp4a(e0[k], rr[k], A0);
+                N0 = __dp4a(e0[k], nn[k], N0);
+                A1 = __dp4a(e1[k], rr[k], A1);
+                N1 = __dp4a(e1[k], nn[k], N1);
+                M = __dp4a(e0[k] & e1[k], nn[k], M);
+            }
+            if (u >= 0) {
+                unsigned char *o = B + ((size_t)wl * ncols + 2 * u) * Wpad + c * 16;
+                __stcs(reinterpret_cast<uint4 *>(o), make_uint4(e0[0], e0[1], e0[2], e0[3]));
+                __stcs(reinterpret_cast<uint4 *>(o + Wpad), make_uint4(e1[0], e1[1], e1[2], e1[3]));
+            }
+            if (A && k0 < k1) {
+#pragma unroll
+                for (int k = 0; k < 4; k++) {
+                    e0[k] = (e0[k] * 0xFFu) & nn[k];
+                    e1[k] = (e1[k] * 0xFFu) & nn[k];
+                }
+                for (int k = k0; k < k1; k++) {
+                    unsigned char *o = A + ((size_t)wl * 2 * T + 2 * slot_target(k)) * Wpad + c * 16;
+                    __stcs(reinterpret_cast<uint4 *>(o), make_uint4(e0[0], e0[1], e0[2], e0[3]));
+                    __stcs(reinterpret_cast<uint4 *>(o + Wpad), make_uint4(e1[0], e1[1], e1[2], e1[3]));
+                }
+            }
+        }
+        A0 = warp_sum(A0); N0 = warp_sum(N0); A1 = warp_sum(A1); N1 = warp_sum(N1); M = warp_sum(M);
+        if (lane == 0) {
+            const double R0 = fma(alpha, (double)A0, beta * (double)(N0 - A0));
+            const double R1 = fma(alpha, (double)A1, beta * (double)(N1 - A1));
+            if (u >= 0) {
+                const double lc = s_lnc[i];
+                const double p0 = R0 + lc, p1 = R1 + lc;
+                Rp[(size_t)w * ncolpad + 2 * u] = p0;
+                Rp[(size_t)w * ncolpad + 2 * u + 1] = p1;
+                const double q0 = rint(p0 * inv_abs_kappa), q1 = rint(p1 * inv_abs_kappa);
+                akey[(size_t)w * ncolpad + 2 * u] = (int32_t)q0;
+                akey[(size_t)w * ncolpad + 2 * u + 1] = (int32_t)q1;
+                Fp[(size_t)w * ncolpad + 2 * u] = p0 == -INFINITY ? 0.0 : exp(fma(q0, kappa, p0));
+                Fp[(size_t)w * ncolpad + 2 * u + 1] = p1 == -INFINITY ? 0.0 : exp(fma(q1, kappa, p1));
+                Qp[(size_t)w * nU + u] = (((c0 + R0) + R1) + kappa * (double)M) + lc;
+            }
+            for (int k = k0; k < k1; k++) {
+                const int t = slot_target(k);
+                Rt[((size_t)w * T + t) * 2] = R0;
+                Rt[((size_t)w * T + t) * 2 + 1] = R1;
+                wll[((size_t)t * outW + w) * 3 + 2] = ((c0 + R0) + R1) + kappa * (double)M;
+            }
+        }
     }
 }
 
@@ -900,7 +893,6 @@
     dev_free(e, c->d_nr, c->b_nr);
     dev_free(e, c->d_l0, c->b_l0);
     dev_free(e, c->d_C0, c->b_C0);
-    dev_free(e, c->d_tbits, c->b_tbits);
     delete c;
     e->ld = nullptr;
 }
@@ -926,10 +918,9 @@
         c->H = 2 * e->N;
         const size_t slots = (size_t)c->nW * c->Wpad;
         c->b_infsite = slots * 4; c->b_nk = slots; c->b_nr = slots; c->b_l0 = slots * 8; c->b_C0 = (size_t)c->nW * 8;
-        c->b_tbits = (size_t)c->nW * c->H * c->WP32 * 4;
         if (dev_alloc(e, (void **)&c->d_infsite, c->b_infsite) || dev_alloc(e, (void **)&c->d_nk, c->b_nk) ||
             dev_alloc(e, (void **)&c->d_nr, c->b_nr) || dev_alloc(e, (void **)&c->d_l0, c->b_l0) ||
-            dev_alloc(e, (void **)&c->d_C0, c->b_C0) || dev_alloc(e, (void **)&c->d_tbits, c->b_tbits))
+            dev_alloc(e, (void **)&c->d_C0, c->b_C0))
             return 1;
     }
     c->K = e->K_shared;
@@ -949,7 +940,6 @@
     }
     IBD_CUDA(cudaGetLastError());
     c->valid = true;
-    c->tw_upto = 0;
     return 0;
 }
 
@@ -963,25 +953,9 @@
     return 0;
 }
 
-static int cache_windows(ibdgem_engine *e, int w_hi) {
-    LdCache *c = e->ld;
-    if (e->shard_count > 1 && c->tw_upto == 0) {
-        int32_t wb = 0;
-        window_shard_bounds(e, &wb, nullptr, nullptr, nullptr);
-        c->tw_upto = wb;
-    }
-    if (c->tw_upto >= w_hi) return 0;
-    if (ld_transpose_launch(e, c->tw_upto, w_hi, c->d_infsite, c->Wpad, c->WP32, c->H, c->d_tbits)) return 1;
-    c->tw_upto = w_hi;
-    return 0;
-}
-
-int ld_tensor_prepare(ibdgem_engine *e) {
-    if (build_cache(e) || ensure_table(e, e->S)) return 1;
-    return cache_windows(e, e->ld->nW);
-}
-
-int ld_tensor_score(ibdgem_engine *e, int32_t T, const int32_t *h_targets, const int32_t *d_targets, int32_t n_bg,
+int ld_tensor_prepare(ibdgem_engine *e) { return build_cache(e) || ensure_table(e, e->S); }
+
+int ld_tensor_score(ibdgem_engine *e, int32_t T, const int32_t *h_targets, int32_t n_bg,
                     const int32_t *h_bg, int32_t pu_idx, int32_t outW, double *d_wll, int32_t *d_wn, uint64_t *d_ws,
                     uint64_t *d_we, int32_t *d_nwout) {
     if (build_cache(e)) return 1;
@@ -990,17 +964,14 @@
     int64_t total_bg = 0;
     for (int n = 0; n < n_bg; n++)
         if (h_bg[n] != pu_idx) { mult[h_bg[n]]++; total_bg++; }
-    std::vector<int32_t> bgU;
     std::vector<double> lnc;
-    bgU.reserve((size_t)c->N);
     lnc.reserve((size_t)c->N);
     for (int32_t b = 0; b < c->N; b++)
         if (mult[b]) {
-            where[b] = (int32_t)bgU.size();
-            bgU.push_back(b);
+            where[b] = (int32_t)lnc.size();
             lnc.push_back(mult[b] == 1 ? 0.0 : log((double)mult[b]));
         }
-    const int nU = (int)bgU.size();
+    const int nU = (int)lnc.size();
     const double nan = (double)NAN;
     std::vector<int32_t> ownU(T), row_own(2 * (size_t)T);
     std::vector<double> lognb(T), lognb4(T);
@@ -1012,11 +983,18 @@
         lognb4[t] = nb > 0 ? log(4.0 * (double)nb) : nan;
         row_own[2 * t] = row_own[2 * t + 1] = own >= 0 ? 2 * own : -1;
     }
+    std::vector<int32_t> tptr((size_t)c->N + 1, 0), tlist(T);
+    for (int t = 0; t < T; t++) tptr[h_targets[t] + 1]++;
+    for (int n = 0; n < c->N; n++) tptr[n + 1] += tptr[n];
+    {
+        std::vector<int32_t> fill(tptr.begin(), tptr.end() - 1);
+        for (int t = 0; t < T; t++) tlist[fill[h_targets[t]]++] = t;
+    }
     const int nW = c->nW;
     std::vector<int> range_end;
     const bool in_flight = e->chunks_waited < (int)e->chunk_end.size() && e->chunk_end.size() > 1 &&
                            cudaEventQuery(e->chunk_ev[e->chunk_end.size() - 1]) == cudaErrorNotReady;
-    if (in_flight && c->tw_upto == 0) {
+    if (in_flight) {
         int w = 0;
         for (size_t k = 0; k < e->chunk_end.size(); k++) {
             while (w < nW && e->h_wlast[(size_t)w] < e->chunk_end[k]) w++;
@@ -1027,7 +1005,7 @@
         if (e->h_wll_out && tail_div > 1 && nW >= 8 * tail_div) range_end.push_back(nW - nW / tail_div);
         range_end.push_back(nW);
     }
-    bool by_chunk = in_flight && c->tw_upto == 0;
+    bool by_chunk = in_flight;
     int32_t shard_wb = 0, shard_we = nW;
     int64_t shard_se = e->S;
     const bool sharded = e->shard_count > 1;
@@ -1051,9 +1029,52 @@
     }
     auto range_sites = [&](size_t k) { return by_chunk ? e->chunk_end[k] : shard_se; };
     const int nrows = 2 * T;
+    const int N = c->N;
+    double *d_lnc, *d_lognb, *d_lognb4;
+    int32_t *d_where, *d_tptr, *d_tlist, *d_ownU, *d_rowown;
+    {
+        const size_t misc_d = (size_t)nU + 2 * (size_t)T;
+        const size_t misc_i = 2 * (size_t)N + 1 + T + T + 2 * (size_t)T;
+        void *h_misc;
+        if (scratch(e, SC_MMA_MISC, misc_i * 4 + misc_d * 8 + 64, (void **)&d_lnc) ||
+            pinned_stage(e, misc_d * 8 + misc_i * 4, &h_misc))
+            return 1;
+        d_lognb = d_lnc + nU;
+        d_lognb4 = d_lognb + T;
+        d_where = reinterpret_cast<int32_t *>(d_lognb4 + T);
+        d_tptr = d_where + N;
+        d_tlist = d_tptr + N + 1;
+        d_ownU = d_tlist + T;
+        d_rowown = d_ownU + T;
+        double *hd = static_cast<double *>(h_misc);
+        memcpy(hd, lnc.data(), (size_t)nU * 8);
+        memcpy(hd + nU, lognb.data(), (size_t)T * 8);
+        memcpy(hd + nU + T, lognb4.data(), (size_t)T * 8);
+        int32_t *hi = reinterpret_cast<int32_t *>(hd + misc_d);
+        memcpy(hi, where.data(), (size_t)N * 4);
+        memcpy(hi + N, tptr.data(), ((size_t)N + 1) * 4);
+        memcpy(hi + 2 * N + 1, tlist.data(), (size_t)T * 4);
+        memcpy(hi + 2 * N + 1 + T, ownU.data(), (size_t)T * 4);
+        memcpy(hi + 2 * N + 1 + 2 * T, row_own.data(), (size_t)T * 8);
+        LaunchScope ls(e, K_LD_STAGE);
+        const int n = (int)((misc_d * 8 + misc_i * 4) / 4);
+        ld_stage_kernel<<<(n + 255) / 256, 256, 0, e->stream>>>(reinterpret_cast<uint32_t *>(d_lnc),
+                                                               static_cast<const uint32_t *>(h_misc), n);
+    }
+    auto launch_build = [&](int wb, int nw, int ncols, int ncolpad, unsigned char *A, unsigned char *B, int32_t *akey,
+                            double *Rp, double *Qp, double *Fp, double *Rt) {
+        LaunchScope ls(e, K_LD_BUILD);
+        const int groups = ((c->H + 31) / 32 + 7) / 8;
+        for (int w0 = wb; w0 < wb + nw; w0 += MAX_GRID_Y)
+            ld_build_kernel<<<dim3((unsigned)groups, (unsigned)std::min(MAX_GRID_Y, wb + nw - w0)), BUILD_THREADS, 0, e->stream>>>(
+                w0, N, T, ncols, ncolpad, nU, c->Wpad, c->WP32, outW, e->d_bits, e->Wh, c->d_infsite, c->d_nr, c->d_nk,
+                c->d_C0, d_where, d_tptr, d_tlist, d_lnc, e->alpha, e->beta, e->kappa, 1.0 / -e->kappa,
+                A ? A + (size_t)(w0 - wb) * nrows * c->Wpad : nullptr, B ? B + (size_t)(w0 - wb) * ncols * c->Wpad : nullptr,
+                akey, Rp, Qp, Fp, Rt, d_wll);
+    };
     if (nU == 0) {
         double *d_Rt;
-        if (ensure_table(e, e->S) || cache_windows(e, nW) || scratch(e, SC_MMA_ROWLSE, (size_t)nW * nrows * 8, (void **)&d_Rt))
+        if (ensure_table(e, e->S) || scratch(e, SC_MMA_ROWLSE, (size_t)nW * nrows * 8, (void **)&d_Rt))
             return 1;
         {
             LaunchScope ls(e, K_LD_WINDOWS);
@@ -1061,13 +1082,7 @@
             ld_windows_kernel<<<(unsigned)((n + 255) / 256), 256, 0, e->stream>>>(
                 0, nW, T, nW, outW, c->W, c->K, e->d_wfirst, e->d_wlast, e->d_pos, d_wn, d_ws, d_we, d_nwout);
         }
-        {
-            LaunchScope ls(e, K_LD_EXPAND_TGT);
-            for (int w0 = 0; w0 < nW; w0 += MAX_GRID_Y)
-                ld_expand_tgt_kernel<<<dim3((unsigned)((T + 7) / 8), (unsigned)std::min(MAX_GRID_Y, nW - w0)), 256, 0, e->stream>>>(
-                    w0, T, c->H, c->Wpad, c->WP32, outW, d_targets, c->d_tbits, c->d_nr, c->d_nk, c->d_C0, e->alpha, e->beta,
-                    e->kappa, nullptr, d_Rt, d_wll);
-        }
+        launch_build(0, nW, 0, 0, nullptr, nullptr, nullptr, nullptr, nullptr, nullptr, d_Rt);
         IBD_CUDA(cudaGetLastError());
         return 0;
     }
@@ -1084,41 +1099,17 @@
         return sb && atol(sb) > 0 ? (size_t)atol(sb) << 20 : LD_OPERAND_BUDGET;
     }();
     const int nWb = (int)std::max<size_t>(1, std::min<size_t>({(size_t)nW, budget / per_window, (size_t)MAX_GRID_Y}));
-    int32_t *d_bgU, *d_ownU, *d_rowown, *d_akey;
-    double *d_lnc, *d_lognb, *d_lognb4, *d_Rp, *d_Qp, *d_Rt, *d_Fp;
+    int32_t *d_akey;
+    double *d_Rp, *d_Qp, *d_Rt, *d_Fp;
     unsigned char *d_A, *d_B;
-    const size_t misc_i = (size_t)nU + T + 2 * (size_t)T;
-    const size_t misc_d = (size_t)nU + 2 * (size_t)T;
-    if (scratch(e, SC_MMA_MISC, misc_i * 4 + misc_d * 8 + 64, (void **)&d_lnc) ||
-        scratch(e, SC_MMA_BGIDX, (size_t)nW * ncolpad * 4, (void **)&d_akey) ||
+    if (scratch(e, SC_MMA_BGIDX, (size_t)nW * ncolpad * 4, (void **)&d_akey) ||
         scratch(e, SC_MMA_ROWLSE, (2 * (size_t)nW * ncolpad + (size_t)nW * nU + (size_t)nW * nrows) * 8, (void **)&d_Rp) ||
         scratch(e, SC_MMA_TGT, (size_t)nWb * nrows * c->Wpad, (void **)&d_A) ||
         scratch(e, SC_MMA_BG, (size_t)nWb * ncols * c->Wpad, (void **)&d_B))
         return 1;
-    d_lognb = d_lnc + nU;
-    d_lognb4 = d_lognb + T;
-    d_bgU = reinterpret_cast<int32_t *>(d_lognb4 + T);
-    d_ownU = d_bgU + nU;
-    d_rowown = d_ownU + T;
     d_Fp = d_Rp + (size_t)nW * ncolpad;
     d_Qp = d_Fp + (size_t)nW * ncolpad;
     d_Rt = d_Qp + (size_t)nW * nU;
-    {
-        void *h_misc;
-        if (pinned_stage(e, misc_d * 8 + misc_i * 4, &h_misc)) return 1;
-        double *hd = static_cast<double *>(h_misc);
-        memcpy(hd, lnc.data(), (size_t)nU * 8);
-        memcpy(hd + nU, lognb.data(), (size_t)T * 8);
-        memcpy(hd + nU + T, lognb4.data(), (size_t)T * 8);
-        int32_t *hi = reinterpret_cast<int32_t *>(hd + misc_d);
-        memcpy(hi, bgU.data(), (size_t)nU * 4);
-        memcpy(hi + nU, ownU.data(), (size_t)T * 4);
-        memcpy(hi + nU + T, row_own.data(), (size_t)T * 8);
-        LaunchScope ls(e, K_LD_STAGE);
-        const int n = (int)((misc_d * 8 + misc_i * 4) / 4);
-        ld_stage_kernel<<<(n + 255) / 256, 256, 0, e->stream>>>(reinterpret_cast<uint32_t *>(d_lnc),
-                                                               static_cast<const uint32_t *>(h_misc), n);
-    }
 
     const bool stream_out = (range_end.size() > 1 || sharded) && e->h_wll_out != nullptr;
     const bool stream_dev = e->d_wll_out_device != nullptr;
@@ -1149,7 +1140,6 @@
     const int w_hi = range_end[rk];
     if (ensure_table(e, range_sites(rk))) return 1;
     if (w_hi == w_lo && !(sharded && rk == 0)) continue;
-    if (w_hi > w_lo && cache_windows(e, w_hi)) return 1;
     if (!sharded || rk == 0) {
         LaunchScope ls(e, K_LD_WINDOWS);
         const int b_lo = sharded ? 0 : w_lo, b_hi = sharded ? nW : w_hi;
@@ -1165,19 +1155,7 @@
     if (w_hi == w_lo) continue;
     for (int w0 = w_lo; w0 < w_hi; w0 += nWb) {
         const int nw = std::min(nWb, w_hi - w0);
-        {
-            LaunchScope ls(e, K_LD_EXPAND_BG);
-            const int npadU = ncolpad / 2;
-            ld_expand_bg_kernel<<<dim3((unsigned)((npadU + 7) / 8), (unsigned)nw), 256, 0, e->stream>>>(
-                w0, nU, npadU, ncols, ncolpad, c->H, c->Wpad, c->WP32, d_bgU, d_lnc, c->d_tbits, c->d_nr, c->d_nk, c->d_C0,
-                e->alpha, e->beta, e->kappa, 1.0 / -e->kappa, d_B, d_akey, d_Rp, d_Qp, d_Fp);
-        }
-        {
-            LaunchScope ls(e, K_LD_EXPAND_TGT);
-            ld_expand_tgt_kernel<<<dim3((unsigned)((T + 7) / 8), (unsigned)nw), 256, 0, e->stream>>>(
-                w0, T, c->H, c->Wpad, c->WP32, outW, d_targets, c->d_tbits, c->d_nr, c->d_nk, c->d_C0, e->alpha, e->beta,
-                e->kappa, d_A, d_Rt, d_wll);
-        }
+        launch_build(w0, nw, ncols, ncolpad, d_A, d_B, d_akey, d_Rp, d_Qp, d_Fp, d_Rt);
         IBD_CUDA(cudaGetLastError());
         CUtensorMap mapA, mapB;
         if (make_operand_map(&mapA, d_A, c->Wpad, nrows, nw)) return 1;
```

New measurement: 1359000 billion, median of 6. 8.6% higher.
